# lostinc0de/sparsemat

Measured on AMD Instinct MI355X. Metric: csr_spmv_effective_hbm_GBps, higher is better.
Workload: dtype f32

## Files before the change

include/sparsemat_hip.h:

```cpp
#ifndef SPARSEMAT_HIP_H
#define SPARSEMAT_HIP_H

#include <stddef.h>
#include <stdint.h>

#ifdef __cplusplus
extern "C" {
#endif

#define SMH_ABI_VERSION 3

enum {
    SMH_OK = 0,
    SMH_ERR_DIM_MISMATCH = 1,
    SMH_ERR_NOT_SQUARE = 2,
    SMH_ERR_INDEX_RANGE = 3,
    SMH_ERR_INVALID = 4,
    SMH_ERR_HIP = 5,
    SMH_ERR_OOM = 6,
    SMH_ERR_NO_DEVICE = 7,
    SMH_ERR_CAPACITY = 8,
    SMH_ERR_COMM = 9
};

// ... 22 lines not shown
const char *smh_last_error(void);
const char *smh_status_string(int status);
int smh_device_count(int *count_out);
int smh_set_device(int device);
int smh_device_synchronize(void);

int smh_crs_create(smh_dtype dtype, size_t n_rows, size_t n_cols, size_t nnz,
                   const uint32_t *offset_rows, const uint32_t *columns, const void *values,
                   int validate, smh_crs **out);
int smh_crs_create_dev(smh_dtype dtype, size_t n_rows, size_t n_cols, size_t nnz,
                       const uint32_t *offset_rows_dev, const uint32_t *columns_dev,
                       const void *values_dev, int validate, smh_crs **out);
int smh_crs_assemble(smh_dtype dtype, size_t n_ops, const uint32_t *rows, const uint32_t *cols,
                     const void *values, const uint8_t *ops, smh_crs **out);
int smh_crs_assemble_dev(smh_dtype dtype, size_t n_ops, const uint32_t *rows_dev,
                         const uint32_t *cols_dev, const void *values_dev, const uint8_t *ops_dev,
                         smh_crs **out);
int smh_crs_replay(smh_dtype dtype, size_t n_ops, const uint32_t *rows, const uint32_t *cols,
                   const void *values, const uint8_t *ops, smh_crs **out);
int smh_crs_replay_dev(smh_dtype dtype, size_t n_ops, const uint32_t *rows_dev,
                       const uint32_t *cols_dev, const void *values_dev, const uint8_t *ops_dev,
                       smh_crs **out);
int smh_crs_transpose(const smh_crs *a, smh_crs **out);
int smh_last_transpose_route(void);
int smh_crs_column_info(const smh_crs *m, uint32_t *rows, uint32_t *col_ptr, uint32_t *entries);
int smh_crs_column_info_dev(const smh_crs *m, uint32_t *rows_dev, uint32_t *col_ptr_dev,
                            uint32_t *entries_dev);
int smh_crs_prod(const smh_crs *a, const smh_crs *b, smh_crs **out);
int smh_crs_permute(const smh_crs *a, const uint32_t *row_perm, size_t n_row_perm, const uint32_t *col_perm, size_t n_col_perm, smh_crs **out);
int smh_crs_permute_dev(const smh_crs *a, const uint32_t *row_perm_dev, size_t n_row_perm, const uint32_t *col_perm_dev, size_t n_col_perm,
                        smh_crs **out);
int smh_crs_permute_symmetric(const smh_crs *a, const uint32_t *perm, size_t n_perm, smh_crs **out);
int smh_crs_permute_symmetric_dev(const smh_crs *a, const uint32_t *perm_dev, size_t n_perm, smh_crs **out);
int smh_crs_bandwidth(const smh_crs *m, uint32_t *lower_out, uint32_t *upper_out);
int smh_crs_span_fraction(smh_crs *m, double *out);
int smh_crs_rcm(const smh_crs *m, uint32_t *perm_out, size_t *n_components_out, size_t *n_levels_out);
int smh_crs_rcm_dev(const smh_crs *m, uint32_t *perm_out_dev, size_t *n_components_out, size_t *n_levels_out);
int smh_crs_color(const smh_crs *m, uint32_t seed, uint32_t *colors_out, uint32_t *perm_out, size_t *n_colors_out, size_t *n_rounds_out);
int smh_crs_color_dev(const smh_crs *m, uint32_t seed, uint32_t *colors_out_dev, uint32_t *perm_out_dev, size_t *n_colors_out, size_t *n_rounds_out);
int smh_crs_clone(const smh_crs *a, smh_crs **out);
int smh_crs_add(const smh_crs *a, const smh_crs *b, smh_crs **out);
int smh_crs_sub(const smh_crs *a, const smh_crs *b, smh_crs **out);
int smh_crs_add_assign(smh_crs *a, const smh_crs *b);
int smh_crs_sub_assign(smh_crs *a, const smh_crs *b);
int smh_last_add_route(void);
int smh_crs_get(const smh_crs *m, size_t i, size_t j, void *value_out);
int smh_crs_get_many(const smh_crs *m, size_t n, const uint32_t *rows, const uint32_t *cols, void *values_out);
int smh_crs_get_many_dev(const smh_crs *m, size_t n, const uint32_t *rows_dev, const uint32_t *cols_dev, void *values_out_dev);
int smh_crs_apply(smh_crs *m, size_t n_ops, const uint32_t *rows, const uint32_t *cols, const void *values, const uint8_t *ops);
int smh_crs_apply_dev(smh_crs *m, size_t n_ops, const uint32_t *rows_dev, const uint32_t *cols_dev, const void *values_dev,
                      const uint8_t *ops_dev);
int smh_last_apply_route(void);
typedef struct smh_update_plan smh_update_plan;
int smh_update_plan_create(const smh_crs *m, size_t n_ops, const uint32_t *rows, const uint32_t *cols, const uint8_t *ops,
                           smh_update_plan **out);
int smh_update_plan_create_dev(const smh_crs *m, size_t n_ops, const uint32_t *rows_dev, const uint32_t *cols_dev,
                               const uint8_t *ops_dev, smh_update_plan **out);
int smh_update_plan_execute(smh_update_plan *p, smh_crs *m, const void *values, int from_zero);
int smh_update_plan_execute_dev(smh_update_plan *p, smh_crs *m, const void *values_dev, int from_zero);
int smh_update_plan_stats(const smh_update_plan *p, size_t *n_ops, size_t *n_targets, size_t *n_live_ops, size_t *longest_run,
                          size_t *long_run_threshold, size_t *device_bytes);
int smh_update_plan_destroy(smh_update_plan *p);
int smh_crs_eye(smh_dtype dtype, size_t dim, smh_crs **out);
int smh_crs_is_symmetric(const smh_crs *m, int *out);
int smh_crs_is_sorted(const smh_crs *m, int *out);
int smh_crs_sort_rows(smh_crs *m);
int smh_crs_destroy(smh_crs *m);
int smh_crs_update_values(smh_crs *m, const void *values_host);
int smh_crs_download(const smh_crs *m, uint32_t *offset_rows, uint32_t *columns, void *values);
size_t smh_crs_n_rows(const smh_crs *m);
size_t smh_crs_n_cols(const smh_crs *m);
size_t smh_crs_nnz(const smh_crs *m);
size_t smh_crs_orphans(const smh_crs *m);
int smh_crs_dtype(const smh_crs *m);
int smh_crs_max_row_len(const smh_crs *m, uint32_t *out);
int smh_crs_col_range(const smh_crs *m, uint32_t *min_out, uint32_t *max_out);
int smh_crs_scale(smh_crs *m, double a);
int smh_crs_resolved_variant(const smh_crs *m, int *variant_out, int *lanes_out);
int smh_crs_set_vector_lanes(smh_crs *m, int lanes);
int smh_crs_set_stream_xs(smh_crs *m, int mode);
int smh_crs_stream_layout(smh_crs *m, int *coded_out, int *byte_lengths_out, int *small_tiles_out, int *xs_chunks_out);
int smh_crs_stream_value_dict(smh_crs *m, int *n_values_out, void *values_out);
int smh_crs_set_stream_value_dict(smh_crs *m, int mode);
int smh_crs_set_stream_direct(smh_crs *m, int mode);
int smh_crs_stream_direct(smh_crs *m, int *direct_out);
int smh_crs_set_vector_chunks(smh_crs *m, int chunks);
int smh_crs_set_ring(smh_crs *m, int mode);
int smh_crs_ring_entries(smh_crs *m, uint32_t *out);
int smh_crs_ring_column_form(smh_crs *m, int *form_out);
int smh_crs_ring_bands(smh_crs *m, uint32_t *bands_out, uint32_t *intervals_out);
int smh_crs_ring_plan(smh_crs *m, uint32_t *n_blocks_out, size_t *n_phases_out,
                      double *ring_fraction_out, int *active_out, uint32_t *phase_ptr_out,
                      uint32_t *phases_out);
int smh_crs_ring_regular(smh_crs *m, uint32_t *len_out);

int smh_crs_set_colblock_shift(smh_crs *m, uint32_t shift);
int smh_crs_colblock(smh_crs *m, uint32_t *shift_out, size_t *n_blocks_out, int *rows_per_thread_out,
                     double *span_fraction_out, uint32_t *offsets_out, uint32_t *columns_out,
                     void *values_out);

int smh_crs_colfused(smh_crs *m, int *fits_out, uint32_t *shift_out, size_t *n_blocks_out, uint32_t *rows_per_lane_out,
                     size_t *n_tiles_out, uint32_t *tile_rows_out, uint32_t *segments_out, uint8_t *counts_out,
                     uint32_t *columns_out, void *values_out);

int smh_crs_tiled_layout(smh_crs *m, uint32_t *n_slices_out, uint32_t *slice_columns_out, uint32_t *rows_per_block_out,
                         uint32_t *n_row_blocks_out, size_t *copy_entries_out);
int smh_crs_tiled_products(smh_crs *m, size_t *n_products_out);

int smh_crs_tiled_array(smh_crs *m, int which, void *out, size_t capacity_bytes, size_t *bytes_out);

int smh_crs_colsplit(smh_crs *m, int *split_out, uint32_t *min_long_out, size_t *n_long_out, uint32_t *long_rows_out,
                     smh_crs **long_out, smh_crs **short_out);

int smh_crs_spmv(smh_crs *m, const void *x_host, size_t x_len, void *y_host, int variant);
int smh_crs_prepare(smh_crs *m, int variant);
int smh_crs_prepare_stats(smh_crs *m, int variant, double *prepare_ms_out, size_t *derived_bytes_out);
int smh_crs_spmv_dev(smh_crs *m, const void *x_dev, size_t x_len, void *y_dev, int variant,
                     void *stream);
int smh_crs_inner_prod(smh_crs *m, const void *lhs_host, size_t lhs_len, const void *rhs_host,
                       size_t rhs_len, int variant, double *out);
size_t smh_crs_merge_tiles(const smh_crs *m);
size_t smh_crs_merge_tile_items(const smh_crs *m);
int smh_crs_merge_table(smh_crs *m, uint32_t *row_out, uint32_t *nnz_out);

int smh_vec_create(smh_dtype dtype, size_t n, smh_vec **out);
int smh_vec_from_host(smh_dtype dtype, size_t n, const void *host, smh_vec **out);
int smh_vec_wrap_dev(smh_dtype dtype, size_t n, void *dev_ptr, smh_vec **out);
int smh_vec_destroy(smh_vec *v);
int smh_vec_upload(smh_vec *v, const void *host);
int smh_vec_download(const smh_vec *v, void *host);
size_t smh_vec_dim(const smh_vec *v);
int smh_vec_dtype(const smh_vec *v);
void *smh_vec_data(const smh_vec *v);
int smh_vec_copy(smh_vec *dst, const smh_vec *src);
int smh_vec_permute(smh_vec *dst, const smh_vec *src, const uint32_t *perm, size_t n_perm, int inverse);
int smh_vec_permute_dev(smh_vec *dst, const smh_vec *src, const uint32_t *perm_dev, size_t n_perm, int inverse);
int smh_vec_add(smh_vec *x, const smh_vec *y);
int smh_vec_sub(smh_vec *x, const smh_vec *y);
int smh_vec_scale(smh_vec *x, double a);
int smh_vec_axpy(smh_vec *y, double a, const smh_vec *x);
int smh_vec_xpby(smh_vec *p, double b, const smh_vec *r);
int smh_vec_dot(const smh_vec *x, const smh_vec *y, double *out);
int smh_vec_norm_squared(const smh_vec *x, double *out);
int smh_vec_norm(const smh_vec *x, double *out);
int smh_blas_dot_dev(smh_dtype dtype, const void *x_dev, const void *y_dev, size_t n, void *result_dev,
                     void *scratch_dev, void *stream);
size_t smh_blas_dot_scratch_bytes(void);
int smh_blas_axpy_dev(smh_dtype dtype, void *y_dev, const void *a_dev, const void *x_dev, size_t n, void *stream);
int smh_blas_xpby_dev(smh_dtype dtype, void *p_dev, const void *b_dev, const void *r_dev, size_t n, void *stream);
int smh_crs_spmv_vec(smh_crs *m, const smh_vec *x, smh_vec *y, int variant);
int smh_crs_inner_prod_vec(smh_crs *m, const smh_vec *lhs, const smh_vec *rhs, int variant, double *out);

int smh_mvec_create(smh_dtype dtype, size_t n, size_t k, smh_mvec **out);
int smh_mvec_from_host(smh_dtype dtype, size_t n, size_t k, const void *host, smh_mvec **out);
int smh_mvec_upload(smh_mvec *mv, const void *host);
int smh_mvec_download(const smh_mvec *mv, void *host);
int smh_mvec_destroy(smh_mvec *mv);
size_t smh_mvec_dim(const smh_mvec *mv);
size_t smh_mvec_count(const smh_mvec *mv);
size_t smh_mvec_ld(const smh_mvec *mv);
int smh_mvec_dtype(const smh_mvec *mv);
void *smh_mvec_data(const smh_mvec *mv);
int smh_mvec_set_column(smh_mvec *mv, size_t c, const smh_vec *v);
int smh_mvec_get_column(const smh_mvec *mv, size_t c, smh_vec *v);
int smh_mvec_copy(smh_mvec *dst, const smh_mvec *src);
int smh_mvec_add(smh_mvec *x, const smh_mvec *y);
// ... 153 lines not shown
```

rust/src/ffi.rs:

```rust
#![allow(non_camel_case_types)]
use std::os::raw::{c_char, c_double, c_int, c_void};

#[repr(C)] pub struct smh_crs { _private: [u8; 0] }
#[repr(C)] pub struct smh_vec { _private: [u8; 0] }
#[repr(C)] pub struct smh_update_plan { _private: [u8; 0] }
#[repr(C)] pub struct smh_par { _private: [u8; 0] }
#[repr(C)] pub struct smh_par_vec { _private: [u8; 0] }
#[repr(C)] pub struct smh_comm { _private: [u8; 0] }

pub const SMH_OK: c_int = 0;
pub const SMH_ERR_DIM_MISMATCH: c_int = 1;
pub const SMH_F32: c_int = 0;
pub const SMH_F64: c_int = 1;
pub const SMH_SPMV_AUTO: c_int = 0;
pub const SMH_TRI_LOWER: c_int = 0;
pub const SMH_TRI_UPPER: c_int = 1;
pub const SMH_DIAG_NON_UNIT: c_int = 0;
pub const SMH_DIAG_UNIT: c_int = 1;
pub const SMH_EXCHANGE_NONE: c_int = 0;
pub const SMH_EXCHANGE_ALLGATHER: c_int = 1;
pub const SMH_EXCHANGE_WINDOW: c_int = 2;
pub const SMH_EXCHANGE_AUTO: c_int = 3;
pub const SMH_COMM_ID_BYTES: usize = 128;
pub const SMH_SPLIT_ROWS: c_int = 0;
pub const SMH_SPLIT_NNZ: c_int = 1;

extern "C" {
    pub fn smh_abi_version() -> c_int;
    pub fn smh_last_error() -> *const c_char;
    pub fn smh_device_count(count_out: *mut c_int) -> c_int;
    pub fn smh_pool_trim() -> c_int;
    pub fn smh_pool_stats(kept_bytes_out: *mut usize, live_bytes_out: *mut usize) -> c_int;
    pub fn smh_crs_create(dtype: c_int, n_rows: usize, n_cols: usize, nnz: usize,
                          offset_rows: *const u32, columns: *const u32, values: *const c_void,
                          validate: c_int, out: *mut *mut smh_crs) -> c_int;
    pub fn smh_crs_destroy(m: *mut smh_crs) -> c_int;
    pub fn smh_crs_update_values(m: *mut smh_crs, values_host: *const c_void) -> c_int;
    pub fn smh_crs_spmv(m: *mut smh_crs, x_host: *const c_void, x_len: usize, y_host: *mut c_void,
                        variant: c_int) -> c_int;
    pub fn smh_cg_solve(m: *mut smh_crs, b_host: *const c_void, b_len: usize, x_host_inout: *mut c_void,
                        x_len: usize, tol: c_double, iter_max: usize, variant: c_int,
                        iters_out: *mut usize, rr_out: *mut c_double) -> c_int;
    pub fn smh_pcg_jacobi_solve(m: *mut smh_crs, b_host: *const c_void, b_len: usize, x_host_inout: *mut c_void,
                                x_len: usize, tol: c_double, iter_max: usize, variant: c_int,
                                iters_out: *mut usize, rr_out: *mut c_double) -> c_int;
    pub fn smh_bicgstab_solve(m: *mut smh_crs, b_host: *const c_void, b_len: usize, x_host_inout: *mut c_void,
                              x_len: usize, tol: c_double, iter_max: usize, variant: c_int,
                              iters_out: *mut usize, rr_out: *mut c_double, breakdown_out: *mut c_int) -> c_int;
    pub fn smh_bicgstab_solve_vec(m: *mut smh_crs, b: *const smh_vec, x: *mut smh_vec, tol: c_double, iter_max: usize,
                                  variant: c_int, check_every: usize,
                                  iters_out: *mut usize, rr_out: *mut c_double, breakdown_out: *mut c_int) -> c_int;
    pub fn smh_crs_trisolve_levels(m: *mut smh_crs, uplo: c_int, n_levels_out: *mut usize, level_of_row_out: *mut u32,
                                   n_launches_out: *mut usize, small_level_rows_out: *mut usize) -> c_int;
    pub fn smh_crs_trisolve(m: *mut smh_crs, uplo: c_int, diag: c_int, b_host: *const c_void, b_len: usize, x_host: *mut c_void,
                            x_len: usize) -> c_int;
    pub fn smh_crs_trisolve_vec(m: *mut smh_crs, uplo: c_int, diag: c_int, b: *const smh_vec, x: *mut smh_vec) -> c_int;
    pub fn smh_crs_sgs_apply_vec(m: *mut smh_crs, r: *const smh_vec, z: *mut smh_vec) -> c_int;
    pub fn smh_pcg_sgs_solve(m: *mut smh_crs, b_host: *const c_void, b_len: usize, x_host_inout: *mut c_void,
                             x_len: usize, tol: c_double, iter_max: usize, variant: c_int,
                             iters_out: *mut usize, rr_out: *mut c_double) -> c_int;
    pub fn smh_pcg_sgs_solve_vec(m: *mut smh_crs, b: *const smh_vec, x: *mut smh_vec, tol: c_double, iter_max: usize,
                                 variant: c_int, check_every: usize, iters_out: *mut usize, rr_out: *mut c_double) -> c_int;
    pub fn smh_crs_ilu0(a: *const smh_crs, f_out: *mut *mut smh_crs, zero_pivot_out: *mut usize) -> c_int;
    pub fn smh_crs_ilu0_refactor(f: *mut smh_crs, a: *const smh_crs, zero_pivot_out: *mut usize) -> c_int;
    pub fn smh_crs_ilu_apply_vec(f: *mut smh_crs, r: *const smh_vec, z: *mut smh_vec) -> c_int;
    pub fn smh_pcg_ilu_solve(a: *mut smh_crs, f: *mut smh_crs, b_host: *const c_void, b_len: usize, x_host_inout: *mut c_void,
                             x_len: usize, tol: c_double, iter_max: usize, variant: c_int,
                             iters_out: *mut usize, rr_out: *mut c_double) -> c_int;
    pub fn smh_pcg_ilu_solve_vec(a: *mut smh_crs, f: *mut smh_crs, b: *const smh_vec, x: *mut smh_vec, tol: c_double, iter_max: usize,
                                 variant: c_int, check_every: usize, iters_out: *mut usize, rr_out: *mut c_double) -> c_int;
    pub fn smh_crs_inner_prod(m: *mut smh_crs, lhs_host: *const c_void, lhs_len: usize, rhs_host: *const c_void,
                              rhs_len: usize, variant: c_int, out: *mut c_double) -> c_int;
    pub fn smh_crs_assemble(dtype: c_int, n_ops: usize, rows: *const u32, cols: *const u32, values: *const c_void,
                            ops: *const u8, out: *mut *mut smh_crs) -> c_int;
    pub fn smh_crs_replay(dtype: c_int, n_ops: usize, rows: *const u32, cols: *const u32, values: *const c_void,
                          ops: *const u8, out: *mut *mut smh_crs) -> c_int;
    pub fn smh_crs_transpose(a: *const smh_crs, out: *mut *mut smh_crs) -> c_int;
    pub fn smh_crs_set_stream_xs(m: *mut smh_crs, mode: c_int) -> c_int;
    pub fn smh_crs_set_stream_direct(m: *mut smh_crs, mode: c_int) -> c_int;
    pub fn smh_crs_stream_direct(m: *mut smh_crs, direct_out: *mut c_int) -> c_int;
    pub fn smh_crs_stream_layout(m: *mut smh_crs, coded_out: *mut c_int, byte_lengths_out: *mut c_int, small_tiles_out: *mut c_int, xs_chunks_out: *mut c_int) -> c_int;
    pub fn smh_last_transpose_route() -> c_int;
    pub fn smh_crs_orphans(m: *const smh_crs) -> usize;
    pub fn smh_crs_prod(a: *const smh_crs, b: *const smh_crs, out: *mut *mut smh_crs) -> c_int;
    pub fn smh_crs_clone(a: *const smh_crs, out: *mut *mut smh_crs) -> c_int;
    pub fn smh_crs_permute(a: *const smh_crs, row_perm: *const u32, n_row_perm: usize, col_perm: *const u32, n_col_perm: usize,
                           out: *mut *mut smh_crs) -> c_int;
    pub fn smh_crs_permute_dev(a: *const smh_crs, row_perm_dev: *const u32, n_row_perm: usize, col_perm_dev: *const u32,
                               n_col_perm: usize, out: *mut *mut smh_crs) -> c_int;
    pub fn smh_crs_permute_symmetric(a: *const smh_crs, perm: *const u32, n_perm: usize, out: *mut *mut smh_crs) -> c_int;
    pub fn smh_crs_permute_symmetric_dev(a: *const smh_crs, perm_dev: *const u32, n_perm: usize, out: *mut *mut smh_crs) -> c_int;
    pub fn smh_crs_bandwidth(m: *const smh_crs, lower_out: *mut u32, upper_out: *mut u32) -> c_int;
    pub fn smh_crs_span_fraction(m: *mut smh_crs, out: *mut f64) -> c_int;
    pub fn smh_crs_ring_regular(m: *mut smh_crs, len_out: *mut u32) -> c_int;
    pub fn smh_crs_rcm(m: *const smh_crs, perm_out: *mut u32, n_components_out: *mut usize, n_levels_out: *mut usize) -> c_int;
    pub fn smh_crs_rcm_dev(m: *const smh_crs, perm_out_dev: *mut u32, n_components_out: *mut usize, n_levels_out: *mut usize) -> c_int;
    pub fn smh_crs_color(m: *const smh_crs, seed: u32, colors_out: *mut u32, perm_out: *mut u32, n_colors_out: *mut usize, n_rounds_out: *mut usize) -> c_int;
    pub fn smh_crs_color_dev(m: *const smh_crs, seed: u32, colors_out_dev: *mut u32, perm_out_dev: *mut u32, n_colors_out: *mut usize, n_rounds_out: *mut usize) -> c_int;
    pub fn smh_vec_permute(dst: *mut smh_vec, src: *const smh_vec, perm: *const u32, n_perm: usize, inverse: c_int) -> c_int;
    pub fn smh_vec_permute_dev(dst: *mut smh_vec, src: *const smh_vec, perm_dev: *const u32, n_perm: usize, inverse: c_int) -> c_int;
    pub fn smh_crs_add(a: *const smh_crs, b: *const smh_crs, out: *mut *mut smh_crs) -> c_int;
    pub fn smh_crs_sub(a: *const smh_crs, b: *const smh_crs, out: *mut *mut smh_crs) -> c_int;
    pub fn smh_crs_add_assign(a: *mut smh_crs, b: *const smh_crs) -> c_int;
    pub fn smh_crs_sub_assign(a: *mut smh_crs, b: *const smh_crs) -> c_int;
    pub fn smh_last_add_route() -> c_int;
    pub fn smh_crs_get(m: *const smh_crs, i: usize, j: usize, value_out: *mut c_void) -> c_int;
    pub fn smh_crs_get_many(m: *const smh_crs, n: usize, rows: *const u32, cols: *const u32, values_out: *mut c_void) -> c_int;
    pub fn smh_crs_get_many_dev(m: *const smh_crs, n: usize, rows_dev: *const u32, cols_dev: *const u32,
                                values_out_dev: *mut c_void) -> c_int;
    pub fn smh_crs_apply(m: *mut smh_crs, n_ops: usize, rows: *const u32, cols: *const u32, values: *const c_void,
                         ops: *const u8) -> c_int;
    pub fn smh_crs_apply_dev(m: *mut smh_crs, n_ops: usize, rows_dev: *const u32, cols_dev: *const u32,
                             values_dev: *const c_void, ops_dev: *const u8) -> c_int;
    pub fn smh_last_apply_route() -> c_int;
    pub fn smh_update_plan_create(m: *const smh_crs, n_ops: usize, rows: *const u32, cols: *const u32, ops: *const u8,
                                  out: *mut *mut smh_update_plan) -> c_int;
    pub fn smh_update_plan_create_dev(m: *const smh_crs, n_ops: usize, rows_dev: *const u32, cols_dev: *const u32,
                                      ops_dev: *const u8, out: *mut *mut smh_update_plan) -> c_int;
    pub fn smh_update_plan_execute(p: *mut smh_update_plan, m: *mut smh_crs, values: *const c_void, from_zero: c_int) -> c_int;
    pub fn smh_update_plan_execute_dev(p: *mut smh_update_plan, m: *mut smh_crs, values_dev: *const c_void, from_zero: c_int) -> c_int;
    pub fn smh_update_plan_stats(p: *const smh_update_plan, n_ops: *mut usize, n_targets: *mut usize, n_live_ops: *mut usize,
                                 longest_run: *mut usize, long_run_threshold: *mut usize, device_bytes: *mut usize) -> c_int;
    pub fn smh_update_plan_destroy(p: *mut smh_update_plan) -> c_int;
    pub fn smh_crs_eye(dtype: c_int, dim: usize, out: *mut *mut smh_crs) -> c_int;
    pub fn smh_crs_is_symmetric(m: *const smh_crs, out: *mut c_int) -> c_int;
    pub fn smh_crs_is_sorted(m: *const smh_crs, out: *mut c_int) -> c_int;
    pub fn smh_crs_column_info(m: *const smh_crs, rows: *mut u32, col_ptr: *mut u32, entries: *mut u32) -> c_int;
    pub fn smh_crs_sort_rows(m: *mut smh_crs) -> c_int;
    pub fn smh_par_create(dtype: c_int, n_blocks: usize, device_ids: *const c_int, n_rows: usize, n_cols: usize,
                          offset_rows: *const u32, columns: *const u32, values: *const c_void, validate: c_int,
                          out: *mut *mut smh_par) -> c_int;
    pub fn smh_par_create_split(dtype: c_int, n_blocks: usize, device_ids: *const c_int, n_rows: usize, n_cols: usize,
                                offset_rows: *const u32, columns: *const u32, values: *const c_void, validate: c_int,
                                split_mode: c_int, out: *mut *mut smh_par) -> c_int;
    pub fn smh_par_split(p: *const smh_par, rows_out: *mut usize) -> c_int;
    pub fn smh_par_set_overlap(p: *mut smh_par, on: c_int) -> c_int;
    pub fn smh_par_interior(p: *const smh_par, local_block: usize, variant: c_int, row_begin: *mut usize, row_end: *mut usize) -> c_int;
    pub fn smh_par_destroy(p: *mut smh_par) -> c_int;
    pub fn smh_par_spmv(p: *mut smh_par, x_host: *const c_void, x_len: usize, y_host: *mut c_void, variant: c_int) -> c_int;
    pub fn smh_par_cg_solve(p: *mut smh_par, b_host: *const c_void, b_len: usize, x_host_inout: *mut c_void, x_len: usize,
                            tol: c_double, iter_max: usize, variant: c_int, iters_out: *mut usize,
                            rr_out: *mut c_double) -> c_int;
    pub fn smh_par_vec_create(p: *mut smh_par, n: usize, out: *mut *mut smh_par_vec) -> c_int;
    pub fn smh_par_vec_destroy(v: *mut smh_par_vec) -> c_int;
    pub fn smh_par_vec_upload(v: *mut smh_par_vec, host: *const c_void) -> c_int;
    pub fn smh_par_vec_download(v: *const smh_par_vec, host: *mut c_void) -> c_int;
    pub fn smh_par_spmv_dev(p: *mut smh_par, x: *const smh_par_vec, y: *mut smh_par_vec, variant: c_int, exchange: c_int) -> c_int;
    pub fn smh_par_exchange(p: *mut smh_par, v: *mut smh_par_vec, mode: c_int) -> c_int;
    pub fn smh_par_synchronize(p: *mut smh_par) -> c_int;
    pub fn smh_par_cg_solve_vec(p: *mut smh_par, b: *const smh_par_vec, x: *mut smh_par_vec, tol: c_double, iter_max: usize,
                                variant: c_int, check_every: usize, iters_out: *mut usize, rr_out: *mut c_double) -> c_int;
    pub fn smh_comm_unique_id(id_out: *mut c_void) -> c_int;
    pub fn smh_comm_create(id: *const c_void, n_ranks: c_int, rank: c_int, out: *mut *mut smh_comm) -> c_int;
    pub fn smh_comm_destroy(c: *mut smh_comm) -> c_int;
    pub fn smh_par_create_rank(comm: *mut smh_comm, n_rows: usize, block: *mut smh_crs, out: *mut *mut smh_par) -> c_int;
    pub fn smh_par_create_rank_split(comm: *mut smh_comm, n_rows: usize, block: *mut smh_crs, row_begin: usize, out: *mut *mut smh_par) -> c_int;
    pub fn smh_crs_n_rows(m: *const smh_crs) -> usize;
    pub fn smh_crs_n_cols(m: *const smh_crs) -> usize;
    pub fn smh_crs_dtype(m: *const smh_crs) -> c_int;
    pub fn smh_crs_nnz(m: *const smh_crs) -> usize;
    pub fn smh_crs_download(m: *const smh_crs, offset_rows: *mut u32, columns: *mut u32, values: *mut c_void) -> c_int;
}
```

sparsemat_amd/_lib.py:

```python
import ctypes as C
import os

_HERE = os.path.dirname(os.path.abspath(__file__))
LIB_PATH = os.environ.get("SPARSEMAT_HIP_LIB") or os.path.join(_HERE, "libsparsemat_hip.so")

SMH_OK = 0
SMH_ERR_DIM_MISMATCH, SMH_ERR_NOT_SQUARE, SMH_ERR_INDEX_RANGE, SMH_ERR_INVALID = 1, 2, 3, 4
SMH_ERR_HIP, SMH_ERR_OOM, SMH_ERR_NO_DEVICE, SMH_ERR_CAPACITY, SMH_ERR_COMM = 5, 6, 7, 8, 9
SMH_F32, SMH_F64 = 0, 1
SMH_TRI_LOWER, SMH_TRI_UPPER = 0, 1
SMH_DIAG_NON_UNIT, SMH_DIAG_UNIT = 0, 1
UPLO = {"lower": SMH_TRI_LOWER, "upper": SMH_TRI_UPPER}
EXCHANGE_NONE, EXCHANGE_ALLGATHER, EXCHANGE_WINDOW, EXCHANGE_AUTO = 0, 1, 2, 3
EXCHANGES = {"none": EXCHANGE_NONE, "allgather": EXCHANGE_ALLGATHER, "window": EXCHANGE_WINDOW, "halo": EXCHANGE_WINDOW, "auto": EXCHANGE_AUTO}
EXCHANGE_NAMES = {EXCHANGE_NONE: "none", EXCHANGE_ALLGATHER: "allgather", EXCHANGE_WINDOW: "window", EXCHANGE_AUTO: "auto"}
PAR_BACKEND_AUTO, PAR_BACKEND_PEER, PAR_BACKEND_RCCL = 0, 1, 2
PAR_BACKENDS = {"auto": PAR_BACKEND_AUTO, "peer": PAR_BACKEND_PEER, "rccl": PAR_BACKEND_RCCL}
COMM_ID_BYTES = 128
SPMV_AUTO, SPMV_VECTOR, SPMV_MERGE, SPMV_SEQ, SPMV_STREAM, SPMV_COLBLOCK, SPMV_COLFUSED, SPMV_COLSPLIT, SPMV_TILED = 0, 1, 2, 3, 4, 5, 6, 7, 8
VARIANTS = {"auto": SPMV_AUTO, "vector": SPMV_VECTOR, "merge": SPMV_MERGE, "seq": SPMV_SEQ, "stream": SPMV_STREAM,
            "colblock": SPMV_COLBLOCK, "colfused": SPMV_COLFUSED, "colsplit": SPMV_COLSPLIT, "tiled": SPMV_TILED}

_sz = C.c_size_t
_vp = C.c_void_p
# ... 139 lines not shown
    "smh_cg_solve_many_host": (_int, [_vp, _vp, _sz, _sz, _vp, C.c_double, _sz, C.POINTER(_sz), C.POINTER(C.c_double)]),
    "smh_pcg_jacobi_solve": (_int, [_vp, _vp, _sz, _vp, _sz, C.c_double, _sz, _int, C.POINTER(_sz),
                                    C.POINTER(C.c_double)]),
    "smh_crs_trisolve_levels": (_int, [_vp, _int, C.POINTER(_sz), _vp, C.POINTER(_sz), C.POINTER(_sz)]),
    "smh_crs_trisolve": (_int, [_vp, _int, _int, _vp, _sz, _vp, _sz]),
    "smh_crs_trisolve_vec": (_int, [_vp, _int, _int, _vp, _vp]),
    "smh_crs_sgs_apply_vec": (_int, [_vp, _vp, _vp]),
    "smh_pcg_sgs_solve": (_int, [_vp, _vp, _sz, _vp, _sz, C.c_double, _sz, _int, C.POINTER(_sz),
                                 C.POINTER(C.c_double)]),
    "smh_pcg_sgs_solve_vec": (_int, [_vp, _vp, _vp, C.c_double, _sz, _int, _sz, C.POINTER(_sz),
                                     C.POINTER(C.c_double)]),
    "smh_crs_ilu0": (_int, [_vp, C.POINTER(_vp), C.POINTER(_sz)]),
    "smh_crs_ilu0_refactor": (_int, [_vp, _vp, C.POINTER(_sz)]),
    "smh_crs_ilu_apply_vec": (_int, [_vp, _vp, _vp]),
    "smh_pcg_ilu_solve": (_int, [_vp, _vp, _vp, _sz, _vp, _sz, C.c_double, _sz, _int, C.POINTER(_sz),
                                 C.POINTER(C.c_double)]),
    "smh_pcg_ilu_solve_vec": (_int, [_vp, _vp, _vp, _vp, C.c_double, _sz, _int, _sz, C.POINTER(_sz),
                                     C.POINTER(C.c_double)]),
    "smh_bicgstab_solve": (_int, [_vp, _vp, _sz, _vp, _sz, C.c_double, _sz, _int, C.POINTER(_sz),
                                  C.POINTER(C.c_double), C.POINTER(_int)]),
    "smh_bicgstab_solve_vec": (_int, [_vp, _vp, _vp, C.c_double, _sz, _int, _sz, C.POINTER(_sz),
                                      C.POINTER(C.c_double), C.POINTER(_int)]),
    "smh_comm_unique_id": (_int, [_vp]),
    "smh_comm_create": (_int, [_vp, _int, _int, C.POINTER(_vp)]),
    "smh_comm_destroy": (_int, [_vp]),
    "smh_comm_size": (_int, [_vp]),
    "smh_comm_rank": (_int, [_vp]),
    "smh_comm_ranks_seen": (_int, [_vp, C.POINTER(C.c_int), C.POINTER(C.c_int)]),
    "smh_rccl_version": (_int, [C.POINTER(C.c_int)]),
    "smh_comm_barrier": (_int, [_vp]),
    "smh_comm_max_f64": (_int, [_vp, C.POINTER(C.c_double)]),
    "smh_par_create": (_int, [_int, _sz, _vp, _sz, _sz, _vp, _vp, _vp, _int, C.POINTER(_vp)]),
    "smh_par_create_split": (_int, [_int, _sz, _vp, _sz, _sz, _vp, _vp, _vp, _int, _int, C.POINTER(_vp)]),
    "smh_par_adopt_split": (_int, [_sz, C.POINTER(_vp), _sz, _vp, C.POINTER(_vp)]),
    "smh_par_create_rank_split": (_int, [_vp, _sz, _vp, _sz, C.POINTER(_vp)]),
    "smh_par_split": (_int, [_vp, _vp]),
    "smh_par_plan_split": (_int, [_sz, _sz, _vp, _vp, _vp, _vp, _sz, _vp, _vp, _vp, _vp, C.POINTER(_int), C.POINTER(_sz)]),
    "smh_par_adopt": (_int, [_sz, C.POINTER(_vp), _sz, C.POINTER(_vp)]),
    "smh_par_create_rank": (_int, [_vp, _sz, _vp, C.POINTER(_vp)]),
    "smh_par_n_local_blocks": (_sz, [_vp]),
    "smh_par_set_backend": (_int, [_vp, _int]),
    "smh_par_backend": (_int, [_vp]),
    "smh_par_set_overlap": (_int, [_vp, _int]),
    "smh_par_set_threads": (_int, [_vp, _int]),
    "smh_par_interior": (_int, [_vp, _sz, _int, C.POINTER(_sz), C.POINTER(_sz)]),
    "smh_par_exchange_mode": (_int, [_vp, _int, C.POINTER(_int), C.POINTER(_sz)]),
    "smh_par_plan": (_int, [_sz, _sz, _vp, _vp, _vp, _sz, _vp, _vp, _vp, _vp, C.POINTER(_int), C.POINTER(_sz)]),
    "smh_par_vec_create": (_int, [_vp, _sz, C.POINTER(_vp)]),
    "smh_par_vec_destroy": (_int, [_vp]),
    "smh_par_vec_dim": (_sz, [_vp]),
    "smh_par_vec_upload": (_int, [_vp, _vp]),
    "smh_par_vec_download": (_int, [_vp, _vp]),
    "smh_par_vec_download_block": (_int, [_vp, _sz, _vp]),
    "smh_par_vec_ptr": (_int, [_vp, _sz, C.POINTER(_vp)]),
    "smh_par_spmv_dev": (_int, [_vp, _vp, _vp, _int, _int]),
    "smh_par_exchange": (_int, [_vp, _vp, _int]),
    "smh_par_synchronize": (_int, [_vp]),
    "smh_par_cg_solve_vec": (_int, [_vp, _vp, _vp, C.c_double, _sz, _int, _sz, C.POINTER(_sz), C.POINTER(C.c_double)]),
    "smh_par_destroy": (_int, [_vp]),
    "smh_par_n_blocks": (_sz, [_vp]),
    "smh_par_n_rows": (_sz, [_vp]),
    "smh_par_n_cols": (_sz, [_vp]),
    "smh_par_nnz": (_sz, [_vp]),
    "smh_par_rows_per_block": (_sz, [_vp]),
    "smh_par_block": (_int, [_vp, _sz, C.POINTER(_vp), C.POINTER(_sz), C.POINTER(_sz), C.POINTER(_int)]),
    "smh_par_block_stream": (_int, [_vp, _sz, C.POINTER(_vp)]),
    "smh_par_get_block_and_row_id": (_int, [_vp, _sz, C.POINTER(_sz), C.POINTER(_sz)]),
    "smh_par_scale": (_int, [_vp, C.c_double]),
    "smh_par_spmv": (_int, [_vp, _vp, _sz, _vp, _int]),
    "smh_par_cg_solve": (_int, [_vp, _vp, _sz, _vp, _sz, C.c_double, _sz, _int, C.POINTER(_sz),
                                C.POINTER(C.c_double)]),
    "smh_synth_x": (_int, [_int, C.c_uint64, _sz, _sz, _vp, _vp]),
    "smh_synth_fixed": (_int, [_int, C.c_uint64, _int, _sz, C.c_uint32, _sz, _sz, _vp, _vp, _vp, _vp]),
    "smh_synth_powerlaw_cdf": (_int, [C.c_uint32, C.c_double, _vp]),
    "smh_synth_powerlaw_lengths": (_int, [C.c_uint64, _sz, _sz, C.c_uint32, _vp, _vp]),
    "smh_synth_fill": (_int, [_int, C.c_uint64, _sz, _sz, _sz, _vp, _vp, _vp, _vp]),
    "smh_synth_laplace3d": (_int, [_int, _sz, _sz, _sz, _sz, _sz, _vp, _vp, _vp, C.POINTER(_sz), _vp]),
    "smh_crs_set_stream_xs": (_int, [_vp, _int]),
    "smh_crs_set_stream_direct": (_int, [_vp, _int]),
    "smh_crs_stream_direct": (_int, [_vp, C.POINTER(_int)]),
    "smh_crs_stream_layout": (_int, [_vp, C.POINTER(_int), C.POINTER(_int), C.POINTER(_int), C.POINTER(_int)]),
    "smh_crs_stream_value_dict": (_int, [_vp, C.POINTER(C.c_int), _vp]),
    "smh_crs_set_stream_value_dict": (_int, [_vp, _int]),
    "smh_last_transpose_route": (_int, []),
    "smh_pool_trim": (_int, []),
    "smh_pool_stats": (_int, [C.POINTER(_sz), C.POINTER(_sz)]),
    "smh_dev_alloc": (_int, [_sz, C.POINTER(_vp)]),
    "smh_dev_free": (_int, [_vp]),
    "smh_dev_upload": (_int, [_vp, _vp, _sz]),
    "smh_dev_download": (_int, [_vp, _vp, _sz]),
    "smh_dev_memset": (_int, [_vp, _int, _sz, _vp]),
    "smh_stream_create": (_int, [C.POINTER(_vp)]),
    "smh_stream_destroy": (_int, [_vp]),
    "smh_stream_synchronize": (_int, [_vp]),
    "smh_event_create": (_int, [C.POINTER(_vp)]),
    "smh_event_destroy": (_int, [_vp]),
    "smh_event_record": (_int, [_vp, _vp]),
    "smh_event_elapsed_ms": (_int, [_vp, _vp, C.POINTER(C.c_float)]),
}

_LIB = None


class SparseMatPanic(RuntimeError):

    def __init__(self, status, message):
        super().__init__(message)
        self.status = status


def lib():
    global _LIB
    if _LIB is None:
        if not os.path.exists(LIB_PATH):
            raise ImportError(
                "%s is missing: build it with `python -m sparsemat_amd.build` (hipcc, gfx950). "
                "sparsemat_amd has no CPU fallback." % LIB_PATH)
        import sys
        if "torch" in sys.modules:
            try:
                if sys.modules["torch"].cuda.is_available():
                    sys.modules["torch"].cuda.init()
            except Exception:
                pass
        os.environ.setdefault("HSA_ENABLE_IPC_MODE_LEGACY", "0")
        L = C.CDLL(LIB_PATH)
        for name, (res, args) in SIGNATURES.items():
            fn = getattr(L, name)
            fn.restype = res
            fn.argtypes = args
        _LIB = L
    return _LIB


def check(status):
    if status != SMH_OK:
        L = lib()
        msg = L.smh_last_error().decode(errors="replace") or L.smh_status_string(status).decode()
        raise SparseMatPanic(status, msg)


def dtype_code(np_dtype):
    import numpy as np
    dt = np.dtype(np_dtype)
    if dt == np.float32:
        return SMH_F32
    if dt == np.float64:
        return SMH_F64
    raise TypeError("the HIP path handles f32/f64 values only (got %s)" % dt)


def np_dtype(code):
    import numpy as np
    return np.float64 if code == SMH_F64 else np.float32
```

sparsemat_amd/csrc/capi.hip:

```cpp
#include <atomic>
#include <chrono>
#include <cmath>
#include <cstdarg>
#include <cstdlib>
#include <cstring>
#include <new>
#include <vector>

#include "crs_forms.hpp"

namespace smh {

static thread_local char g_err[512] = "";

void set_error(const char *fmt, ...) {
    va_list ap;
    va_start(ap, fmt);
    vsnprintf(g_err, sizeof g_err, fmt, ap);
    va_end(ap);
}

void clear_error() { g_err[0] = 0; }

int fail(int status, const char *fmt, ...) {
// ... 933 lines not shown
    SMH_TRY(build_eye(dtype, dim, arrays.off, arrays.col, arrays.val, nullptr));
    return wrap_arrays(dtype, nullptr, dim, dim, dim, arrays, 0, out);
}

int smh_crs_is_symmetric(const smh_crs *m, int *out) {
    if (!m || !out) return fail(SMH_ERR_INVALID, "NULL argument");
    return crs_is_symmetric(m->dtype, m->d_off, m->d_col, m->d_val, m->n_rows, out, m->stream);
}

int smh_crs_is_sorted(const smh_crs *m, int *out) {
    if (!m || !out) return fail(SMH_ERR_INVALID, "NULL argument");
    return crs_is_sorted(m->d_off, m->d_col, m->n_rows, out, m->stream);
}

int smh_crs_sort_rows(smh_crs *m) {
    if (!m) return fail(SMH_ERR_INVALID, "NULL handle");
    SMH_TRY(sort_rows(m->dtype, m->d_off, m->d_col, m->d_val, m->n_rows, m->nnz, m->max_col, m->stream));
    invalidate(m, Changed::Order);
    ++m->epoch;
    return SMH_OK;
}

int smh_crs_destroy(smh_crs *m) {
    if (!m) return SMH_OK;
    if (m->stream) { (void)hipStreamSynchronize(m->stream); (void)hipStreamDestroy(m->stream); }
    if (m->owns) { (void)hipFree(m->d_off); (void)hipFree(m->d_col); (void)hipFree(m->d_val); }
    (void)hipGetLastError();
    delete m;
    return SMH_OK;
}

int smh_crs_update_values(smh_crs *m, const void *values_host) {
    if (!m) return fail(SMH_ERR_INVALID, "NULL argument");
    if (m->nnz && values_host) SMH_HIP(hipMemcpy(m->d_val, values_host, m->nnz * dtype_size(m->dtype), hipMemcpyHostToDevice));
    invalidate(m, Changed::Values);
    if (m->codes.state != Form::NotTried && m->codes.direct) {
        StreamCfg c;
        SMH_TRY(stream_cfg(m, &c, true));
    }
    return SMH_OK;
}

int smh_crs_download(const smh_crs *m, uint32_t *offset_rows, uint32_t *columns, void *values) {
    if (!m) return fail(SMH_ERR_INVALID, "NULL handle");
    SMH_HIP(hipStreamSynchronize(m->stream));
    if (offset_rows) SMH_HIP(hipMemcpy(offset_rows, m->d_off, (m->n_rows + 1) * sizeof(uint32_t), hipMemcpyDeviceToHost));
    if (columns && m->nnz) SMH_HIP(hipMemcpy(columns, m->d_col, m->nnz * sizeof(uint32_t), hipMemcpyDeviceToHost));
    if (values && m->nnz) SMH_HIP(hipMemcpy(values, m->d_val, m->nnz * dtype_size(m->dtype), hipMemcpyDeviceToHost));
    return SMH_OK;
}

size_t smh_crs_n_rows(const smh_crs *m) { return m ? m->n_rows : 0; }
size_t smh_crs_n_cols(const smh_crs *m) { return m ? m->n_cols : 0; }
size_t smh_crs_nnz(const smh_crs *m) { return m ? m->nnz : 0; }
size_t smh_crs_orphans(const smh_crs *m) { return m ? m->orphans : 0; }
int smh_crs_dtype(const smh_crs *m) { return m ? m->dtype : -1; }

int smh_crs_max_row_len(const smh_crs *m, uint32_t *out) {
    if (!m || !out) return fail(SMH_ERR_INVALID, "NULL argument");
    *out = m->max_row_len;
    return SMH_OK;
}

int smh_crs_col_range(const smh_crs *m, uint32_t *min_out, uint32_t *max_out) {
    if (!m) return fail(SMH_ERR_INVALID, "NULL handle");
    if (min_out) *min_out = m->min_col;
    if (max_out) *max_out = m->max_col;
    return SMH_OK;
}

int smh_crs_scale(smh_crs *m, double a) {
    if (!m) return fail(SMH_ERR_INVALID, "NULL handle");
    SMH_TRY(launch_scale_values(m->dtype, m->d_val, m->nnz, a, m->stream));
    if (m->has_first_op) {
        Scratch scr;
        char *d = nullptr;
        SMH_TRY(scr.alloc(&d, 16));
        SMH_HIP(hipMemcpyAsync(d, &m->first_val_bits, 8, hipMemcpyHostToDevice, m->stream));
        SMH_TRY(launch_scale_values(m->dtype, d, 1, a, m->stream));
        SMH_HIP(hipMemcpyAsync(&m->first_val_bits, d, 8, hipMemcpyDeviceToHost, m->stream));
        SMH_HIP(hipStreamSynchronize(m->stream));
    }
    if (m->dict.state == Form::Ready) SMH_TRY(launch_scale_values(m->dtype, m->dict.values.get(), 32, a, m->stream));
    if (m->cb.state == Form::Ready) SMH_TRY(launch_scale_values(m->dtype, m->cb.val.get(), m->nnz, a, m->stream));
    if (m->cf.state == Form::Ready) SMH_TRY(launch_scale_values(m->dtype, m->cf.val.get(), m->nnz, a, m->stream));
    if (m->tiled.state == Form::Ready) SMH_TRY(launch_scale_values(m->dtype, m->tiled.val.get(), (size_t)m->tiled.tot, a, m->stream));
    if (m->split.state == Form::Ready) {
        SMH_TRY(smh_crs_scale(m->split.long_part, a));
        SMH_TRY(smh_crs_scale(m->split.short_part, a));
    }
    SMH_HIP(hipStreamSynchronize(m->stream));
    return SMH_OK;
}

int smh_crs_tiled_layout(smh_crs *m, uint32_t *n_slices_out, uint32_t *slice_columns_out, uint32_t *rows_per_block_out, uint32_t *n_row_blocks_out,
                         size_t *copy_entries_out) {
    if (!m) return fail(SMH_ERR_INVALID, "NULL handle");
    SMH_TRY(tiled_build(m));
    if (n_slices_out) *n_slices_out = m->tiled.n_cb;
    if (slice_columns_out) *slice_columns_out = tiled_slice_columns(m->dtype);
    if (rows_per_block_out) *rows_per_block_out = m->tiled.R;
    if (n_row_blocks_out) *n_row_blocks_out = m->tiled.n_rb;
    if (copy_entries_out) *copy_entries_out = (size_t)m->tiled.tot;
    return SMH_OK;
}

int smh_crs_tiled_products(smh_crs *m, size_t *n_products_out) {
    if (!m) return fail(SMH_ERR_INVALID, "NULL handle");
    SMH_TRY(tiled_build(m));
    if (n_products_out) *n_products_out = (size_t)m->tiled.n_prod;
    return SMH_OK;
}

int smh_crs_tiled_array(smh_crs *m, int which, void *out, size_t capacity_bytes, size_t *bytes_out) {
    if (!m) return fail(SMH_ERR_INVALID, "NULL handle");
    SMH_TRY(tiled_build(m));
    return tiled_array(m, which, out, capacity_bytes, bytes_out);
}

int smh_crs_set_colblock_shift(smh_crs *m, uint32_t shift) {
    if (!m) return fail(SMH_ERR_INVALID, "NULL handle");
    if (shift > 31) return fail(SMH_ERR_INVALID, "column block shift must be 0 (automatic) or 1..31");
    if (shift != m->knobs.cb_forced_shift) invalidate(m, Changed::BlockWidth);
    m->knobs.cb_forced_shift = shift;
    return SMH_OK;
}

int smh_crs_colblock(smh_crs *m, uint32_t *shift_out, size_t *n_blocks_out, int *rows_per_thread_out,
                     double *span_fraction_out, uint32_t *offsets_out, uint32_t *columns_out, void *values_out) {
    if (!m) return fail(SMH_ERR_INVALID, "NULL handle");
    SMH_TRY(ensure_ring_plan(m, false));
    SMH_TRY(ensure_colblock(m));
    if (shift_out) *shift_out = m->cb.shift;
    if (n_blocks_out) *n_blocks_out = m->cb.blocks;
    if (rows_per_thread_out) *rows_per_thread_out = m->cb.rpt;
    if (span_fraction_out) *span_fraction_out = m->span_fraction;
    if (offsets_out)
        SMH_HIP(hipMemcpy(offsets_out, m->cb.off.get(), m->cb.blocks * (m->n_rows + 1) * sizeof(uint32_t), hipMemcpyDeviceToHost));
    if (columns_out && m->nnz) SMH_HIP(hipMemcpy(columns_out, m->cb.col.get(), m->nnz * sizeof(uint32_t), hipMemcpyDeviceToHost));
    if (values_out && m->nnz) SMH_HIP(hipMemcpy(values_out, m->cb.val.get(), m->nnz * dtype_size(m->dtype), hipMemcpyDeviceToHost));
    return SMH_OK;
}

int smh_crs_colfused(smh_crs *m, int *fits_out, uint32_t *shift_out, size_t *n_blocks_out, uint32_t *rows_per_lane_out,
                     size_t *n_tiles_out, uint32_t *tile_rows_out, uint32_t *segments_out, uint8_t *counts_out, uint32_t *columns_out,
                     void *values_out) {
    if (!m) return fail(SMH_ERR_INVALID, "NULL handle");
    SMH_TRY(ensure_colfused(m));
    const size_t tile_rows = (size_t)64 * m->cf.rt, n_tiles = (m->cf.state == Form::Ready) ? m->cf.tiles : 0;
    if (fits_out) *fits_out = (m->cf.state == Form::Ready) ? 1 : 0;
    if (shift_out) *shift_out = m->cf.shift;
    if (n_blocks_out) *n_blocks_out = m->cf.blocks;
    if (rows_per_lane_out) *rows_per_lane_out = m->cf.rt;
    if (n_tiles_out) *n_tiles_out = n_tiles;
    if (m->cf.state != Form::Ready) return SMH_OK;
    SMH_HIP(hipStreamSynchronize(m->stream));
    if (tile_rows_out) SMH_HIP(hipMemcpy(tile_rows_out, m->cf.tile_row.get(), (n_tiles + 1) * sizeof(uint32_t), hipMemcpyDeviceToHost));
    if (segments_out) SMH_HIP(hipMemcpy(segments_out, m->cf.seg.get(), (n_tiles * m->cf.blocks + 1) * sizeof(uint32_t), hipMemcpyDeviceToHost));
    if (counts_out && n_tiles) SMH_HIP(hipMemcpy(counts_out, m->cf.cnt.get(), n_tiles * m->cf.blocks * tile_rows, hipMemcpyDeviceToHost));
    if (columns_out && m->nnz) SMH_HIP(hipMemcpy(columns_out, m->cf.col.get(), m->nnz * sizeof(uint32_t), hipMemcpyDeviceToHost));
    if (values_out && m->nnz) SMH_HIP(hipMemcpy(values_out, m->cf.val.get(), m->nnz * dtype_size(m->dtype), hipMemcpyDeviceToHost));
    return SMH_OK;
}

int smh_crs_colsplit(smh_crs *m, int *split_out, uint32_t *min_long_out, size_t *n_long_out, uint32_t *long_rows_out, smh_crs **long_out,
                     smh_crs **short_out) {
    if (!m) return fail(SMH_ERR_INVALID, "NULL handle");
    SMH_TRY(ensure_split(m));
    const bool split = m->split.state == Form::Ready;
    if (split_out) *split_out = split ? 1 : 0;
    if (min_long_out) *min_long_out = kSplitMinLong;
    if (n_long_out) *n_long_out = split ? m->split.n_long : 0;
    if (long_out) *long_out = split ? m->split.long_part : nullptr;
    if (short_out) *short_out = split ? m->split.short_part : nullptr;
    if (long_rows_out && split && m->split.n_long)
        SMH_HIP(hipMemcpy(long_rows_out, m->split.rows.get(), m->split.n_long * sizeof(uint32_t), hipMemcpyDeviceToHost));
    return SMH_OK;
}

int smh_crs_resolved_variant(const smh_crs *m, int *variant_out, int *lanes_out) {
    if (!m) return fail(SMH_ERR_INVALID, "NULL handle");
    if (variant_out) *variant_out = resolve_variant(m, SMH_SPMV_AUTO);
    if (lanes_out) *lanes_out = auto_lanes(m);
    return SMH_OK;
}

int smh_crs_set_stream_xs(smh_crs *m, int mode) {
    if (!m) return fail(SMH_ERR_INVALID, "NULL handle");
    if (mode < -1 || mode > 1) return fail(SMH_ERR_INVALID, "mode must be -1 (automatic), 0 (never) or 1 (whenever the tiles allow)");
    m->knobs.use_stream_xs = mode;
    return recode_stream(m);
}

int smh_crs_set_stream_direct(smh_crs *m, int mode) {
    if (!m) return fail(SMH_ERR_INVALID, "NULL handle");
    if (mode < -1 || mode > 1) return fail(SMH_ERR_INVALID, "mode must be -1 (automatic), 0 (never) or 1 (whenever x is staged)");
    m->knobs.use_stream_direct = mode;
    return recode_stream(m);
}

int smh_crs_stream_direct(smh_crs *m, int *direct_out) {
    if (!m || !direct_out) return fail(SMH_ERR_INVALID, "NULL argument");
    StreamCfg c;
    SMH_TRY(stream_cfg(m, &c));
    *direct_out = c.direct && c.xs != 0;
    return SMH_OK;
}

int smh_crs_stream_value_dict(smh_crs *m, int *n_values_out, void *values_out) {
    if (!m || !n_values_out) return fail(SMH_ERR_INVALID, "NULL argument");
    StreamCfg c;
    SMH_TRY(stream_cfg(m, &c));
    *n_values_out = c.dict ? (int)m->dict.n : 0;
    if (c.dict && values_out) {
        SMH_HIP(hipMemcpyAsync(values_out, m->dict.values.get(), (size_t)m->dict.n * dtype_size(m->dtype), hipMemcpyDeviceToHost, m->stream));
        SMH_HIP(hipStreamSynchronize(m->stream));
    }
    return SMH_OK;
}

int smh_crs_set_stream_value_dict(smh_crs *m, int mode) {
    if (!m) return fail(SMH_ERR_INVALID, "NULL handle");
    if (mode < -1 || mode > 0) return fail(SMH_ERR_INVALID, "mode must be -1 (automatic: whenever the values allow) or 0 (never)");
    m->knobs.use_stream_vdict = mode;
    return recode_stream(m);
}

int smh_crs_stream_layout(smh_crs *m, int *coded_out, int *byte_lengths_out, int *small_tiles_out, int *xs_chunks_out) {
    if (!m) return fail(SMH_ERR_INVALID, "NULL handle");
    StreamCfg c;
    SMH_TRY(stream_cfg(m, &c));
    if (coded_out) *coded_out = c.code && c.cwin;
    if (byte_lengths_out) *byte_lengths_out = c.len8 && c.tbase;
    if (small_tiles_out) *small_tiles_out = c.small;
    if (xs_chunks_out) *xs_chunks_out = c.xs;
    return SMH_OK;
}

int smh_crs_set_vector_chunks(smh_crs *m, int chunks) {
    if (!m) return fail(SMH_ERR_INVALID, "NULL handle");
    if (chunks < 0 || chunks > 3) return fail(SMH_ERR_INVALID, "chunks per lane must be 0 (automatic), 1, 2 or 3");
    m->knobs.forced_chunks = chunks;
    return SMH_OK;
}

int smh_crs_set_ring(smh_crs *m, int mode) {
    if (!m) return fail(SMH_ERR_INVALID, "NULL handle");
    if (mode < -1 || mode > 1) return fail(SMH_ERR_INVALID, "ring mode must be -1 (auto), 0 (plain K1) or 1 (K1r)");
    m->knobs.use_ring = mode;
    return SMH_OK;
}

int smh_crs_ring_plan(smh_crs *m, uint32_t *n_blocks_out, size_t *n_phases_out, double *ring_fraction_out,
                      int *active_out, uint32_t *phase_ptr_out, uint32_t *phases_out) {
    if (!m) return fail(SMH_ERR_INVALID, "NULL handle");
    SMH_TRY(ensure_ring_plan(m));
    bool ring = false;
    SMH_TRY(vector_uses_ring(m, &ring));
    if (n_blocks_out) *n_blocks_out = m->ring.blocks;
    if (n_phases_out) *n_phases_out = m->ring.n_phases;
    if (ring_fraction_out) *ring_fraction_out = m->ring.fraction;
    if (active_out) *active_out = ring ? 1 : 0;
    if (phase_ptr_out)
        SMH_HIP(hipMemcpy(phase_ptr_out, m->ring.phase_ptr.get(), (m->ring.blocks + 1) * sizeof(uint32_t), hipMemcpyDeviceToHost));
    if (phases_out && m->ring.n_phases)
        SMH_HIP(hipMemcpy(phases_out, m->ring.phases.get(), m->ring.n_phases * sizeof(RingPhase), hipMemcpyDeviceToHost));
    return SMH_OK;
}

int smh_crs_ring_regular(smh_crs *m, uint32_t *len_out) {
    if (!m || !len_out) return fail(SMH_ERR_INVALID, "NULL argument");
    SMH_TRY(ensure_ring_plan(m));
    if (m->ring.n_phases)
        SMH_HIP(hipMemcpy(len_out, m->ring.reg_len.get(), m->ring.n_phases * sizeof(uint32_t), hipMemcpyDeviceToHost));
    return SMH_OK;
}

int smh_crs_ring_column_form(smh_crs *m, int *form_out) {
    if (!m || !form_out) return fail(SMH_ERR_INVALID, "NULL argument");
    bool ring = false;
    SMH_TRY(vector_uses_ring(m, &ring));
    *form_out = !ring ? 0 : m->ring.lo8.get() ? 2 : m->ring.col16.get() ? 1 : 0;
    return SMH_OK;
}

int smh_crs_ring_entries(smh_crs *m, uint32_t *out) {
    if (!m || !out) return fail(SMH_ERR_INVALID, "NULL argument");
    SMH_TRY(ensure_ring_plan(m));
    *out = m->ring.entries;
    return SMH_OK;
}

int smh_crs_ring_bands(smh_crs *m, uint32_t *bands_out, uint32_t *intervals_out) {
    if (!m || !bands_out) return fail(SMH_ERR_INVALID, "NULL argument");
    SMH_TRY(ensure_ring_plan(m));
    *bands_out = m->ring.bands;
    if (intervals_out && m->ring.bands == 4 && m->ring.win.get())
        SMH_HIP(hipMemcpy(intervals_out, m->ring.win.get(), ((m->n_rows + 63) / 64) * 8 * sizeof(uint32_t), hipMemcpyDeviceToHost));
    return SMH_OK;
}

int smh_crs_set_vector_lanes(smh_crs *m, int lanes) {
    if (!m) return fail(SMH_ERR_INVALID, "NULL handle");
    if (lanes != 0 && (lanes < 1 || lanes > 64 || (lanes & (lanes - 1))))
        return fail(SMH_ERR_INVALID, "lanes per row must be 0 or a power of two in 1..64");
    m->knobs.forced_lanes = lanes;
    return SMH_OK;
// ... 433 lines not shown
```

sparsemat_amd/csrc/crs_forms.hip:

```cpp
#include <cstdlib>
#include <cstring>
#include <vector>

#include "crs_forms.hpp"

namespace smh {

void build_ring_plan(size_t n_rows, size_t ring_entries, const uint32_t *cmin, const uint32_t *cmax, size_t n_blocks,
                     uint32_t noring_mode, std::vector<uint32_t> &phase_ptr, std::vector<RingPhase> &phases,
                     double *ring_row_fraction);
void build_ring_plan_banded(size_t n_rows, size_t ring_entries, const uint32_t *win, size_t n_blocks, uint32_t noring_mode,
                            std::vector<uint32_t> &phase_ptr, std::vector<RingPhase> &phases, double *ring_row_fraction);

int ensure_merge_ws(smh_crs *m) {
    if (m->merge.state == Form::Ready) return SMH_OK;
    MergeTable t;
    const uint64_t items = (uint64_t)m->n_rows + (uint64_t)m->nnz;
    t.n_tiles = (size_t)((items + kMergeTile - 1) / kMergeTile);
    if (t.n_tiles) {
        SMH_TRY(t.tile_row.alloc(t.n_tiles + 1));
        SMH_TRY(t.tile_nz.alloc(t.n_tiles + 1));
        SMH_TRY(t.carry_row.alloc(t.n_tiles));
        SMH_TRY(t.carry_val.alloc(t.n_tiles * dtype_size(m->dtype)));
        SMH_TRY(launch_merge_table(m->d_off, m->n_rows, m->nnz, t.n_tiles, t.tile_row.get(), t.tile_nz.get(), m->stream));
// ... 153 lines not shown
                return launch_stream_max_tile(c.off.get() + b * (m->n_rows + 1), m->n_rows, (size_t)kStreamRows * rpt, d, m->stream);
            }));
            worst = h > worst ? h : worst;
        }
        if (worst <= (uint32_t)kStreamCap || rpt == 1) break;
    }
    c.rpt = rpt < 1 ? 1 : rpt;
    c.single_pass = worst <= (uint32_t)kStreamCap;
    c.state = Form::Ready;
    m->cb = std::move(c);
    return SMH_OK;
}

int ensure_colfused(smh_crs *m) {
    if (m->cf.state != Form::NotTried) return SMH_OK;
    SMH_TRY(columns_within_n_cols(m, "fused column-blocked variant"));
    const size_t blocks = blocks_for(m->n_cols, cf_shift_for(m));
    if (blocks > 255) return fail(SMH_ERR_INVALID, "fused column-blocked variant: %zu column blocks (supported: 1..255)", blocks);
    uint32_t rt = 16;
    if (const char *e = getenv("SMH_COLFUSED_RT")) {
        if (atoi(e) == 8) rt = 8;
    }
    ColFused c;
    bool fits = false;
    uint32_t *tile_row = nullptr, *seg = nullptr, *col2 = nullptr;
    uint8_t *cnt = nullptr;
    void *val2 = nullptr;
    SMH_TRY(build_colfused(m->dtype, m->d_off, m->d_col, m->d_val, m->n_rows, m->nnz, cf_shift_for(m), blocks, rt, &c.tiles,
                           &tile_row, &seg, &cnt, &col2, &val2, &fits, m->stream));
    c.tile_row.reset(tile_row);
    c.seg.reset(seg);
    c.cnt.reset(cnt);
    c.col.reset(col2);
    c.val.reset((char *)val2);
    c.shift = cf_shift_for(m);
    c.blocks = blocks;
    c.rt = rt;
    c.state = fits ? Form::Ready : Form::Refused;
    m->cf = std::move(c);
    return SMH_OK;
}

const uint32_t kSplitMinLong = 64;
int ensure_split(smh_crs *m) {
    if (m->split.state != Form::NotTried) return SMH_OK;
    SMH_TRY(columns_within_n_cols(m, "row-length split"));
    m->split.state = Form::Refused;
    if (m->no_split || m->n_rows == 0 || m->nnz == 0) return SMH_OK;
    RowSplit sp;
    size_t nnz_long = 0;
    uint32_t *rows = nullptr;
    CrsArrays long_part, short_part;
    SMH_TRY(build_colsplit(m->dtype, m->d_off, m->d_col, m->d_val, m->n_rows, m->nnz, kSplitMinLong, &sp.n_long, &nnz_long, &rows, &long_part.off,
                           &long_part.col, &long_part.val, &short_part.off, &short_part.col, &short_part.val, m->stream));
    sp.rows.reset(rows);
    const bool worth = sp.n_long > 0 && sp.n_long * 4 <= m->n_rows && nnz_long * 4 >= m->nnz;
    if (!worth) return SMH_OK;
    auto part = [&](size_t n_rows, size_t nnz, CrsArrays &arrays, uint32_t shift, smh_crs **out) -> int {
        SMH_TRY(wrap_arrays(m->dtype, nullptr, n_rows, m->n_cols, nnz, arrays, 0, out));
        (*out)->no_split = true;
        (*out)->knobs.cb_forced_shift = shift;
        return SMH_OK;
    };
    SMH_TRY(part(sp.n_long, nnz_long, long_part, 18u, &sp.long_part));
    SMH_TRY(part(m->n_rows, m->nnz - nnz_long, short_part, 19u, &sp.short_part));
    SMH_TRY(sp.y.alloc(sp.n_long * dtype_size(m->dtype)));
    SMH_HIP(hipStreamCreateWithFlags(&sp.side, hipStreamNonBlocking));
    SMH_HIP(hipEventCreateWithFlags(&sp.fork, hipEventDisableTiming));
    SMH_HIP(hipEventCreateWithFlags(&sp.join, hipEventDisableTiming));
    sp.state = Form::Ready;
    m->split = std::move(sp);
    return SMH_OK;
}
RowSplit::~RowSplit() {
    (void)smh_crs_destroy(long_part);
    (void)smh_crs_destroy(short_part);
    rows.reset();
    y.reset();
    if (side) { (void)hipStreamSynchronize(side); (void)hipStreamDestroy(side); }
    if (fork) (void)hipEventDestroy(fork);
    if (join) (void)hipEventDestroy(join);
}

static int ensure_stream_codes(smh_crs *m) {
    if (m->codes.state != Form::NotTried) return SMH_OK;
    StreamCodes c;
    c.state = Form::Refused;
    const size_t n_tiles = (m->n_rows + kStreamRows - 1) / kStreamRows;
    if (n_tiles && m->nnz) {
        uint32_t h_count = 0;
        SMH_TRY(c.cwin.alloc(n_tiles * 8));
        SMH_TRY(read_back(&h_count, 1, m->stream, [&](uint32_t *d_count) {
            return launch_stream_windows(m->d_off, m->d_col, m->n_rows, c.cwin.get(), d_count, m->stream);
        }));
        if ((size_t)h_count == n_tiles) c.state = Form::Ready;
        else c.cwin.reset();
    }
    if (c.state == Form::Ready) {
        const size_t n_out = ((m->nnz + 3) & ~size_t(3)) + 4;
        SMH_TRY(c.code.alloc(n_out));
        SMH_HIP(hipMemsetAsync(c.code.get(), 0, n_out * sizeof(uint16_t), m->stream));
        SMH_TRY(launch_stream_codes(m->d_off, m->d_col, c.cwin.get(), m->n_rows, c.code.get(), m->stream));
        if (m->max_row_len <= 255u) {
            SMH_TRY(c.len8.alloc(n_tiles * kStreamRows));
            SMH_TRY(c.tbase.alloc(n_tiles + 1));
            SMH_TRY(launch_stream_len8(m->d_off, m->n_rows, c.len8.get(), c.tbase.get(), m->stream));
            uint32_t h_xs[2] = {0xFFFFFFFFu, 0};
            SMH_TRY(read_back(h_xs, 2, m->stream, [&](uint32_t *d_xs) { return launch_stream_xs_stats(c.cwin.get(), n_tiles, d_xs, m->stream); }));
            c.xs_chunks = h_xs[0];
            c.xs_end = h_xs[1];
            unsigned long long h_odd = 0;
            SMH_TRY(read_back(&h_odd, 1, m->stream, [&](unsigned long long *d_odd) {
                return launch_stream_odd_rows(c.len8.get(), n_tiles * kStreamRows, d_odd, m->stream);
            }));
            c.odd_rows = (uint64_t)h_odd;
        }
        SMH_HIP(hipStreamSynchronize(m->stream));
    }
    m->codes = std::move(c);
    return SMH_OK;
}

static void drop_ring_col12(smh_crs *m) {
    m->ring.lo8.reset();
    m->ring.hdr.reset();
    m->ring.escapes.reset();
}
static int ensure_ring_col12(smh_crs *m, bool forced, bool *use) {
    RingPlan &r = m->ring;
    *use = forced || r.c12 == Form::Ready;
    if (r.c12 != Form::NotTried && (!*use || r.lo8.get())) return SMH_OK;
    Scratch scr;
    uint32_t *jobs = nullptr;
    unsigned long long *d_counts = nullptr, h_counts[2] = {0, 0};
    SMH_TRY(scr.alloc(&jobs, 2 * r.n_phases));
    SMH_TRY(scr.alloc(&d_counts, 2));
    SMH_TRY(read_back(d_counts, h_counts, 2, m->stream, [&](unsigned long long *d) {
        return launch_col12_count(m->d_off, m->d_col, m->nnz, r.phases.get(), r.n_phases, jobs, d, m->stream);
    }));
    r.c12_chunks = h_counts[0];
    r.c12_escapes = h_counts[1];
    r.c12 = r.c12_escapes * 1024ull <= r.c12_chunks ? Form::Ready : Form::Refused;
    *use = forced || r.c12 == Form::Ready;
    if (!*use) return SMH_OK;
    const size_t n_chunks_out = ((m->nnz + 3) >> 2) + 1;
    DevArray<uint8_t> lo8;
    DevArray<uint16_t> hdr;
    DevArray<uint32_t> escapes;
    SMH_TRY(lo8.alloc(n_chunks_out * 4));
    SMH_TRY(hdr.alloc(n_chunks_out));
    SMH_TRY(escapes.alloc(2 * (size_t)(r.c12_escapes ? r.c12_escapes : 1)));
    SMH_TRY(launch_col12_encode(m->d_col, m->nnz, jobs, r.n_phases, n_chunks_out, lo8.get(), hdr.get(), escapes.get(), d_counts, m->stream));
    SMH_HIP(hipStreamSynchronize(m->stream));
    r.lo8 = std::move(lo8);
    r.hdr = std::move(hdr);
    r.escapes = std::move(escapes);
    return SMH_OK;
}

int vector_uses_ring(smh_crs *m, bool *out) {
    *out = false;
    if (m->knobs.use_ring == 0 || m->n_rows == 0) return SMH_OK;
    SMH_TRY(ensure_ring_plan(m));
    *out = true;
    int want = m->knobs.use_col16;
    if (const char *e = getenv("SMH_RING_COL16")) want = atoi(e) ? 1 : 0;
    int want12 = m->knobs.use_col12;
    if (const char *e = getenv("SMH_RING_COL12")) want12 = strcmp(e, "auto") == 0 ? -1 : (atoi(e) ? 1 : 0);
    const bool can12 = m->dtype == SMH_F32 && m->ring.bands == 1 && m->ring.entries == (unsigned)kRingEntries && m->nnz > 0;
    bool use12 = can12 && (want12 == 1 || (want12 < 0 && want < 0 && m->ring.fraction >= 0.25));
    if (use12) SMH_TRY(ensure_ring_col12(m, want12 == 1, &use12));
    if (!use12) drop_ring_col12(m);
    const bool use16 = m->ring.bands == 4 || want == 1 || (want < 0 && m->ring.fraction >= 0.25);
    if (use16 && !m->ring.col16.get() && m->nnz) {
        const size_t n_out = ((m->nnz + 3) & ~size_t(3)) + 4;
        DevArray<uint16_t> col16;
        SMH_TRY(col16.alloc(n_out));
        if (m->ring.bands == 4) {
            SMH_HIP(hipMemsetAsync(col16.get(), 0, n_out * sizeof(uint16_t), m->stream));
            SMH_TRY(launch_ring_band_codes(m->d_off, m->d_col, m->ring.win.get(), m->n_rows, m->ring.entries / 4, col16.get(), m->stream));
        } else {
            SMH_TRY(launch_narrow_columns(m->d_col, m->nnz, col16.get(), n_out, m->stream));
        }
        SMH_HIP(hipStreamSynchronize(m->stream));
        m->ring.col16 = std::move(col16);
    } else if (!use16) {
        m->ring.col16.reset();
    }
    return SMH_OK;
}

void invalidate(smh_crs *m, Changed what) {
    m->cb = ColBlock();
    m->cf = ColFused();
    m->split = RowSplit();
    m->tiled = Tiled();
    if (what == Changed::Values) m->dict.state = Form::NotTried;
    if (what == Changed::Order) {
        m->codes = StreamCodes();
        m->ring.col16.reset();
        drop_ring_col12(m);
        m->ring.c12 = Form::NotTried;
        m->tri[0] = TriSchedule();
        m->tri[1] = TriSchedule();
    }
}

static int stream_rpt(const smh_crs *m) {
    int want = m->knobs.stream_rows_per_thread;
    if (const char *e = getenv("SMH_STREAM_RPT")) want = atoi(e);
    return want == 2 && m->max_tile512_entries <= (uint32_t)kStreamCap ? 2 : 1;
}

int stream_cfg(smh_crs *m, StreamCfg *c, bool recode) {
    *c = StreamCfg();
    c->rpt = stream_rpt(m);
    c->single_pass = m->have_stats && (c->rpt == 2 || m->max_tile_entries <= (uint32_t)kStreamCap);
    const char *c16_env = getenv("SMH_STREAM_C16");
    if (!(c16_env && atoi(c16_env) == 0) && c->rpt == 1 && c->single_pass) {
        const bool first = m->codes.state == Form::NotTried;
        SMH_TRY(ensure_stream_codes(m));
        if (first) recode = true;
        c->code = m->codes.code.get();
        c->cwin = m->codes.code.get() ? m->codes.cwin.get() : nullptr;
        static const bool l8_off = getenv("SMH_STREAM_L8") && atoi(getenv("SMH_STREAM_L8")) == 0;
        if (c->cwin && !l8_off) { c->len8 = m->codes.len8.get(); c->tbase = m->codes.tbase.get(); }
        static const bool small_off = getenv("SMH_STREAM_SMALL") && atoi(getenv("SMH_STREAM_SMALL")) == 0;
        c->small = !small_off && m->have_stats && m->max_tile_entries <= (uint32_t)kStreamCapSmall;
        static const bool xs_off = getenv("SMH_STREAM_XS") && atoi(getenv("SMH_STREAM_XS")) == 0;
        const bool forced = m->knobs.use_stream_xs == 1;
        const size_t x_bytes = m->n_cols * dtype_size(m->dtype);
        const bool on2 = forced || x_bytes >= ((size_t)1 << 20), on4 = forced || (x_bytes >= ((size_t)8 << 20) && m->dtype == SMH_F32);
        c->xs = (xs_off || m->knobs.use_stream_xs == 0 || !c->small || !c->len8) ? 0
                : (m->codes.xs_chunks <= 2u * kBlock && on2) ? 2
                : (m->codes.xs_chunks <= 4u * kBlock && on4) ? 4 : 0;
        static const bool xd_off = getenv("SMH_STREAM_XD") && atoi(getenv("SMH_STREAM_XD")) == 0;
        const bool want_direct = c->code && c->xs != 0 && !xd_off && m->knobs.use_stream_direct != 0 &&
                                 (m->knobs.use_stream_direct == 1 || 2 * m->codes.odd_rows >= (uint64_t)m->n_rows);
        static const bool vd_off = getenv("SMH_STREAM_VDICT") && atoi(getenv("SMH_STREAM_VDICT")) == 0;
        bool want_vdict = want_direct && !vd_off && m->knobs.use_stream_vdict != 0 && m->dict.state != Form::Refused;
        bool dict_rebuilt = false;
        if (recode && want_vdict && m->dict.state == Form::NotTried) {
            if (!m->dict.values.get()) SMH_TRY(m->dict.values.alloc(32 * dtype_size(m->dtype)));
            SMH_HIP(hipDeviceSynchronize());
            uint32_t n_vals = 0;
            SMH_TRY(stream_value_dict(m->dtype, m->d_val, m->nnz, m->dict.values.get(), &n_vals, m->stream));
            m->dict.n = n_vals;
            m->dict.state = n_vals ? Form::Ready : Form::Refused;
            dict_rebuilt = true;
        }
        want_vdict = want_vdict && m->dict.state == Form::Ready && m->dict.n <= stream_value_dict_capacity(c->xs);
        const bool form_ok = want_direct == m->codes.direct && want_vdict == m->codes.vdict && (!want_vdict || m->codes.vdict_xs == c->xs) &&
                             !(dict_rebuilt && (want_vdict || m->codes.vdict));
        if (recode && c->code && !form_ok) {
            SMH_HIP(hipDeviceSynchronize());
            if (want_direct)
                SMH_TRY(launch_stream_stage_codes(m->d_off, m->d_col, m->codes.cwin.get(), m->n_rows, (uint32_t)dtype_size(m->dtype), m->codes.code.get(), m->stream));
            else
                SMH_TRY(launch_stream_codes(m->d_off, m->d_col, m->codes.cwin.get(), m->n_rows, m->codes.code.get(), m->stream));
            if (want_vdict)
                SMH_TRY(launch_stream_value_codes(m->dtype, m->d_val, m->nnz, m->dict.values.get(), m->dict.n, c->xs, m->codes.code.get(), m->stream));
            SMH_HIP(hipStreamSynchronize(m->stream));
            m->codes.direct = want_direct;
            m->codes.vdict = want_vdict;
            m->codes.vdict_xs = want_vdict ? c->xs : 0;
        }
        c->direct = c->code && m->codes.direct;
        c->dict = c->direct && m->codes.vdict ? m->dict.values.get() : nullptr;
        c->dict_high = c->dict && stream_value_dict_high(m->dtype, m->dict.n, m->codes.vdict_xs);
    }
    return SMH_OK;
}

int recode_stream(smh_crs *m) {
    if (m->codes.state == Form::NotTried) return SMH_OK;
    StreamCfg c;
    return stream_cfg(m, &c, true);
}

}
```

sparsemat_amd/csrc/crs_forms.hpp:

```cpp
#pragma once
#include "internal.hpp"

namespace smh {

void clear_error();
int wrap_arrays(int dtype, const ::smh_crs *like, size_t n_rows, size_t n_cols, size_t nnz, CrsArrays &arrays, int validate, ::smh_crs **out);

template <typename U, typename F> int read_back(U *d, U *host, size_t count, hipStream_t s, F &&launch) {
    SMH_TRY(launch(d));
    SMH_HIP(hipMemcpyAsync(host, d, count * sizeof(U), hipMemcpyDeviceToHost, s));
    SMH_HIP(hipStreamSynchronize(s));
    return SMH_OK;
}
template <typename U, typename F> int read_back(U *host, size_t count, hipStream_t s, F &&launch) {
    Scratch scr;
    U *d = nullptr;
    SMH_TRY(scr.alloc(&d, count));
    return read_back(d, host, count, s, launch);
}

extern const uint32_t kSplitMinLong;
int ensure_merge_ws(::smh_crs *m);
int ensure_ring_plan(::smh_crs *m, bool with_bands = true);
int ensure_colblock(::smh_crs *m);
int ensure_colfused(::smh_crs *m);
int ensure_split(::smh_crs *m);
int vector_uses_ring(::smh_crs *m, bool *out);
enum class Changed { Values, Order, BlockWidth };
void invalidate(::smh_crs *m, Changed what);
struct StreamCfg {
    int rpt = 1;
    bool single_pass = false;
    const uint16_t *code = nullptr;
    const uint32_t *cwin = nullptr;
    const uint8_t *len8 = nullptr;
    const uint32_t *tbase = nullptr;
    bool small = false;
    int xs = 0;
    bool direct = false;
    const void *dict = nullptr;
    bool dict_high = false;
};
int stream_cfg(::smh_crs *m, StreamCfg *c, bool recode = false);
int recode_stream(::smh_crs *m);

extern const size_t kColblockMinXBytes;
uint32_t cb_shift_for(const ::smh_crs *m);
uint32_t cf_shift_for(const ::smh_crs *m);
size_t blocks_for(size_t n_cols, uint32_t shift);
int auto_lanes(const ::smh_crs *m);
int resolve_variant(const ::smh_crs *m, int variant);
int prepare_forms(::smh_crs *m, int variant);
int spmv_inner_prod(::smh_crs *m, const void *d_lhs, const void *d_rhs, size_t rhs_len, int variant, void *scratch, void *res);

}
```

sparsemat_amd/csrc/internal.hpp:

```cpp
#pragma once
#include <hip/hip_runtime.h>

#include <cstddef>
#include <cstdint>
#include <cstdio>
#include <cstring>
#include <string>
#include <utility>
#include <vector>

#include "../../include/sparsemat_hip.h"

namespace smh {

void set_error(const char *fmt, ...);
int fail(int status, const char *fmt, ...);
int hip_fail(hipError_t e, const char *what, const char *file, int line);

#define SMH_HIP(call)                                                     \
    do {                                                                  \
        hipError_t e__ = (call);                                          \
        if (e__ != hipSuccess) return ::smh::hip_fail(e__, #call, __FILE__, __LINE__); \
    } while (0)

// ... 230 lines not shown
    return v + __int_as_float(__builtin_amdgcn_update_dpp(0, __float_as_int(v), CTRL, ROWS, 0xF, false));
}
template <int CTRL, int ROWS> __device__ __forceinline__ double wave_dpp_add(double v) {
    const long long b = __double_as_longlong(v);
    const uint32_t lo = (uint32_t)__builtin_amdgcn_update_dpp(0, (int)(uint32_t)b, CTRL, ROWS, 0xF, false);
    const uint32_t hi = (uint32_t)__builtin_amdgcn_update_dpp(0, (int)(uint32_t)((unsigned long long)b >> 32), CTRL, ROWS, 0xF, false);
    return v + __longlong_as_double((long long)(((unsigned long long)hi << 32) | lo));
}
template <typename T> __device__ __forceinline__ T wave_sum_to_lane63(T v) {
    v = wave_dpp_add<0x111, 0xF>(v);
    v = wave_dpp_add<0x112, 0xF>(v);
    v = wave_dpp_add<0x114, 0xF>(v);
    v = wave_dpp_add<0x118, 0xF>(v);
    v = wave_dpp_add<0x142, 0xA>(v);
    v = wave_dpp_add<0x143, 0xC>(v);
    return v;
}
__device__ __forceinline__ uint32_t wave_max_u32(uint32_t v) {
#pragma unroll
    for (int o = 32; o > 0; o >>= 1) {
        const uint32_t w = (uint32_t)__shfl_xor((int)v, o, kWave);
        v = w > v ? w : v;
    }
    return v;
}
constexpr uint64_t kBuildGrid = 16384;
inline unsigned grid_for(uint64_t n, uint64_t cap) {
    const uint64_t b = (n + kBlock - 1) / kBlock;
    return (unsigned)(b == 0 ? 1 : b > cap ? cap : b);
}
inline unsigned bits_for(uint64_t v) {
    unsigned b = 1;
    while (b < 64 && (v >> b)) ++b;
    return b;
}
constexpr int kMergeItemsPerThread = 8;
constexpr int kMergeTile = kBlock * kMergeItemsPerThread;
constexpr int kReducePartials = 1024;
constexpr int kRingEntries = 16384;
constexpr int kRingEntriesWide = 32768;
constexpr int kStreamRows = kBlock;
constexpr int kStreamCap = 4096;
constexpr int kStreamCapSmall = 2045;
constexpr int kStreamCodeWidth = 16384;
constexpr int kManyCap = 2048;

int device_exclusive_scan_u32(uint32_t *data, uint64_t n, hipStream_t s, uint64_t *total_out);
int launch_spmv_vector(int dtype, int lanes, const uint32_t *off, const uint32_t *col, const void *val,
                       const void *x, void *y, size_t n_rows, size_t nnz, hipStream_t s);
int launch_spmv_seq(int dtype, const uint32_t *off, const uint32_t *col, const void *val, const void *x,
                    void *y, size_t n_rows, hipStream_t s);
int launch_merge_table(const uint32_t *off, size_t n_rows, size_t nnz, size_t n_tiles, uint32_t *tile_row,
                       uint32_t *tile_nz, hipStream_t s);
int launch_spmv_merge(int dtype, const uint32_t *off, const uint32_t *col, const void *val, const void *x,
                      void *y, size_t n_rows, size_t nnz, size_t n_tiles, const uint32_t *tile_row,
                      const uint32_t *tile_nz, uint32_t *carry_row, void *carry_val, hipStream_t s);
int launch_spmv_stream(int dtype, const uint32_t *off, const uint32_t *col, const void *val, const void *x, void *y,
                       size_t n_rows, size_t nnz, bool padded, int rows_per_thread,
                       bool single_pass ,
                       void *dot_partials ,
                       const uint16_t *code, const uint32_t *cwin ,
                       const uint8_t *len8, const uint32_t *tbase ,
                       const void *dot_lhs ,
                       hipStream_t s, bool small_tiles = false ,
                       int xs = 0 ,
                       uint64_t tile_begin = 0, uint64_t tile_end = ~uint64_t(0) );
int launch_stream_xs_stats(const uint32_t *win, size_t n_tiles, uint32_t *d_out2, hipStream_t s);
int launch_stream_len8(const uint32_t *off, size_t n_rows, uint8_t *len8, uint32_t *tbase, hipStream_t s);
size_t stream_tiles(size_t n_rows, int rows_per_thread);
int launch_stream_windows(const uint32_t *off, const uint32_t *col, size_t n_rows, uint32_t *win,
                          uint32_t *d_count, hipStream_t s);
int launch_stream_codes(const uint32_t *off, const uint32_t *col, const uint32_t *win, size_t n_rows, uint16_t *code,
                        hipStream_t s);
int launch_spmv_many(int dtype, const uint32_t *off, const uint32_t *col, const void *val, const void *x, void *y, size_t n_rows, size_t nnz,
                     bool padded, size_t k, size_t ld, hipStream_t s);
int launch_spmv_stream_xd(int dtype, const void *val, const void *x, void *y, size_t n_rows, void *dot_partials, const uint16_t *scode,
                          const uint32_t *cwin, const uint8_t *len8, const uint32_t *tbase, const void *dot_lhs, hipStream_t s, int xs,
                          uint64_t tile_begin = 0, uint64_t tile_end = ~uint64_t(0), const void *dict = nullptr ,
                          bool dict_high = false );
bool stream_value_dict_high(int dtype, uint32_t n, int xs);
int stream_value_dict(int dtype, const void *val, size_t nnz, void *dict_out, uint32_t *count_out, hipStream_t s);
int launch_stream_value_codes(int dtype, const void *val, size_t nnz, const void *dict, uint32_t n, int xs, uint16_t *code, hipStream_t s);
uint32_t stream_value_dict_capacity(int xs);
int launch_stream_stage_codes(const uint32_t *off, const uint32_t *col, const uint32_t *win, size_t n_rows, uint32_t elem_bytes,
                              uint16_t *code, hipStream_t s);
int launch_stream_odd_rows(const uint8_t *len8, size_t n_padded, unsigned long long *d_out, hipStream_t s);
int launch_stream_max_tile(const uint32_t *off, size_t n_rows, size_t tile_rows, uint32_t *d_out, hipStream_t s);
int launch_spmv_stream_block(int dtype, const uint32_t *off, const uint32_t *col, const void *val, const void *x, void *y,
                             size_t n_rows, size_t nnz_total, int rows_per_thread, bool single_pass, bool accumulate,
                             hipStream_t s);
int build_colblock(int dtype, const uint32_t *off, const uint32_t *col, const void *val, size_t n_rows, size_t nnz,
                   uint32_t shift, size_t n_blocks, uint32_t **off2_out, uint32_t **col2_out, void **val2_out,
                   hipStream_t s);
int build_colfused(int dtype, const uint32_t *off, const uint32_t *col, const void *val, size_t n_rows, size_t nnz, uint32_t shift,
                   size_t n_blocks, uint32_t rt, size_t *n_tiles_out, uint32_t **tile_row_out, uint32_t **seg_out, uint8_t **cnt_out,
                   uint32_t **col2_out, void **val2_out, bool *fits_out, hipStream_t s);
int launch_spmv_colfused(int dtype, uint32_t rt, const uint32_t *tile_row, size_t n_tiles, const uint32_t *seg, const uint8_t *cnt,
                         const uint32_t *col, const void *val, const void *x, void *y, size_t n_rows, size_t nnz, uint32_t n_blocks,
                         int device, hipStream_t s);
int build_colsplit(int dtype, const uint32_t *off, const uint32_t *col, const void *val, size_t n_rows, size_t nnz, uint32_t min_long,
                   size_t *n_long_out, size_t *nnz_long_out, uint32_t **long_rows_out, uint32_t **off_l_out, uint32_t **col_l_out, void **val_l_out,
                   uint32_t **off_s_out, uint32_t **col_s_out, void **val_s_out, hipStream_t s);
int launch_split_scatter(int dtype, const uint32_t *long_rows, const void *y_long, size_t n_long, void *y, hipStream_t s);
int assemble_triplets(int dtype, size_t n, const uint32_t *rows, const uint32_t *cols, const void *vals, const uint8_t *ops,
                      bool reverse_rows, bool all_set, bool repeats_adjacent, size_t *n_rows_out, size_t *n_cols_out, size_t *nnz_out,
                      uint32_t **off_out, uint32_t **col_out, void **val_out, hipStream_t s);
int expand_rows(const uint32_t *off, size_t n_rows, uint32_t *rows_out, hipStream_t s);
int column_lists_bucketed(const uint32_t *off, const uint32_t *col, size_t n_rows, size_t n_cols, size_t nnz, uint32_t max_col, uint32_t *col_ptr,
                          uint32_t *entries, bool *done, hipStream_t s);
int transpose_bucketed(int dtype, const uint32_t *off, const uint32_t *col, const void *val, size_t n_rows, size_t nnz, uint32_t max_col,
                       uint32_t **off_out, uint32_t **col_out, void **val_out, size_t *n_rows_out, size_t *n_cols_out, bool *done, hipStream_t s);
int append_to_row(int dtype, uint32_t *off, uint32_t **col, void **val, size_t n_rows, size_t *nnz, size_t row, uint32_t column,
                  const void *value_host, hipStream_t s);
int column_info(const uint32_t *off, const uint32_t *col, size_t n_rows, size_t n_cols, size_t nnz, uint32_t max_col, uint32_t *rows,
                uint32_t *col_ptr, uint32_t *entries, hipStream_t s);
int sort_rows(int dtype, const uint32_t *off, uint32_t *col, void *val, size_t n_rows, size_t nnz, uint32_t max_col,
              hipStream_t s);
int crs_is_sorted(const uint32_t *off, const uint32_t *col, size_t n_rows, int *out, hipStream_t s);
int crs_is_symmetric(int dtype, const uint32_t *off, const uint32_t *col, const void *val, size_t n_rows, int *out, hipStream_t s);
int prod_crs(int dtype, const uint32_t *a_off, const uint32_t *a_col, const void *a_val, size_t a_rows, size_t a_nnz, uint32_t a_max_col,
             const uint32_t *b_off, const uint32_t *b_col, const void *b_val, size_t b_rows, size_t *n_rows_out, size_t *n_cols_out,
             size_t *nnz_out, uint32_t **off_out, uint32_t **col_out, void **val_out, hipStream_t s);
struct AddOperand {
    const uint32_t *off = nullptr, *col = nullptr;
    const void *val = nullptr;
    size_t n_rows = 0, n_cols = 0, nnz = 0, orphans = 0;
    uint32_t max_row_len = 0, max_col = 0;
};
struct AddResult {
    size_t n_rows = 0, n_cols = 0, nnz = 0;
    CrsArrays arrays;
    int route = 0;
    bool values_only = false;
};
int add_crs(int dtype, bool subtract, const AddOperand &a, const AddOperand &b, bool in_place, bool alias, bool force_general, AddResult *res,
            hipStream_t s);
struct UpdMatrix {
    const uint32_t *off = nullptr, *col = nullptr;
    void *val = nullptr;
    size_t n_rows = 0, n_cols = 0, nnz = 0, orphans = 0;
    uint32_t max_row_len = 0;
};
struct UpdResult {
    size_t n_rows = 0, n_cols = 0, nnz = 0;
    CrsArrays arrays;
    int route = 0;
    bool values_only = false;
};
int crs_get_many(int dtype, const UpdMatrix &m, size_t n, const uint32_t *rows, const uint32_t *cols, void *values_out, hipStream_t s);
int crs_apply(int dtype, const UpdMatrix &m, size_t n, const uint32_t *rows, const uint32_t *cols, const void *vals, const uint8_t *ops,
              bool force_general, UpdResult *res, hipStream_t s);
int build_eye(int dtype, size_t dim, uint32_t *off, uint32_t *col, void *val, hipStream_t s);
int validate_permutation(const uint32_t *perm, size_t n, uint32_t *first, const char *what, hipStream_t s);
int permute_crs(int dtype, const uint32_t *a_off, const uint32_t *a_col, const void *a_val, size_t n_rows, size_t nnz, const uint32_t *row_perm,
                const uint32_t *col_inv, CrsArrays *out, hipStream_t s);
int launch_vec_permute(int dtype, void *dst, const void *src, const uint32_t *perm, size_t n, bool inverse, hipStream_t s);
int launch_bandwidth(const uint32_t *off, const uint32_t *col, size_t n_rows, uint32_t *d_out2, hipStream_t s);
int rcm_order(const uint32_t *off, const uint32_t *col, size_t n, size_t nnz, uint32_t *perm_out, size_t *n_components, size_t *n_levels, hipStream_t s);
int symmetrised_pattern(const uint32_t *off, const uint32_t *col, size_t n, size_t nnz, Scratch &scr, uint32_t **adj_off_out, uint32_t **adj_col_out,
                        hipStream_t s);
int color_order(const uint32_t *off, const uint32_t *col, size_t n, size_t nnz, uint32_t seed, uint32_t *colors_out, uint32_t *perm_out, size_t *n_colors,
                size_t *n_rounds, hipStream_t s);
constexpr uint32_t kPlanLongRun = 64;
struct UpdPlan {
    size_t n_ops = 0, n_targets = 0, n_live = 0, longest_run = 0, n_short = 0, device_bytes = 0;
    DevArray<uint32_t> pos;
// ... 92 lines not shown
        if (crc != SMH_OK || ce != hipSuccess || !graph.get() || exec.instantiate(graph.get()) != hipSuccess)
            (void)hipGetLastError();
    } else {
        (void)hipGetLastError();
    }
    auto poll = [&]() -> int {
        SMH_HIP(hipMemcpyAsync(h_sc, d_sc, cg_scalars_bytes(dtype), hipMemcpyDeviceToHost, s));
        SMH_HIP(hipStreamSynchronize(s));
        uint64_t it64 = 0;
        cg_read_scalars(dtype, h_sc, converged, &it64, rr);
        *iters = (size_t)it64;
        return SMH_OK;
    };
    auto run = [&]() -> int {
        size_t launched = 0;
        while (launched < iter_max) {
            size_t batch = iter_max - launched < check_every ? iter_max - launched : check_every;
            if (exec.get()) {
                SMH_HIP(hipGraphLaunch(exec.get(), s));
                batch = check_every;
            } else {
                for (size_t i = 0; i < batch; ++i) SMH_TRY(body());
            }
            launched += batch;
            SMH_TRY(poll());
            if (*converged) break;
        }
        if (iter_max == 0) SMH_TRY(poll());
        return SMH_OK;
    };
    const int rc = run();
    if (rc != SMH_OK) (void)hipStreamSynchronize(s);
    return rc;
}

enum class Form {
    NotTried,
    Ready,
    Refused,
};
struct MergeTable {
    Form state = Form::NotTried;
    size_t n_tiles = 0;
    DevArray<uint32_t> tile_row, tile_nz, carry_row;
    DevArray<char> carry_val;
};
struct RingPlan {
    Form state = Form::NotTried;
    bool bands_tried = false;
    unsigned blocks = 0;
    double fraction = 0.0;
    unsigned entries = kRingEntries;
    unsigned bands = 1;
    size_t n_phases = 0;
    DevArray<uint32_t> phase_ptr;
    DevArray<RingPhase> phases;
    DevArray<uint32_t> reg_len;
    bool reg_applies = false;
    DevArray<uint32_t> win;
    DevArray<uint16_t> col16;
    Form c12 = Form::NotTried;
    uint64_t c12_chunks = 0, c12_escapes = 0;
    DevArray<uint8_t> lo8;
    DevArray<uint16_t> hdr;
    DevArray<uint32_t> escapes;
};
struct StreamCodes {
    Form state = Form::NotTried;
    DevArray<uint32_t> cwin;
    DevArray<uint16_t> code;
    DevArray<uint8_t> len8;
    DevArray<uint32_t> tbase;
    uint32_t xs_chunks = 0xFFFFFFFFu, xs_end = 0;
    uint64_t odd_rows = 0;
    bool direct = false;
    bool vdict = false;
    int vdict_xs = 0;
};
struct StreamDict {
    Form state = Form::NotTried;
    uint32_t n = 0;
    DevArray<char> values;
};
struct ColBlock {
    Form state = Form::NotTried;
    uint32_t shift = 0;
    size_t blocks = 0;
    int rpt = 1;
    bool single_pass = false;
    DevArray<uint32_t> off, col;
    DevArray<char> val;
};
struct ColFused {
    Form state = Form::NotTried;
    uint32_t shift = 0, rt = 0;
    size_t blocks = 0, tiles = 0;
    DevArray<uint32_t> seg, col, tile_row;
    DevArray<uint8_t> cnt;
    DevArray<char> val;
};
struct RowSplit {
    Form state = Form::NotTried;
    ::smh_crs *long_part = nullptr, *short_part = nullptr;
    DevArray<uint32_t> rows;
    DevArray<char> y;
    size_t n_long = 0;
    hipStream_t side = nullptr;
    hipEvent_t fork = nullptr, join = nullptr;
    RowSplit() = default;
    RowSplit(RowSplit &&o) noexcept { swap(o); }
    RowSplit &operator=(RowSplit &&o) noexcept {
        RowSplit old(std::move(*this));
        swap(o);
        return *this;
    }
    ~RowSplit();
    void swap(RowSplit &o) noexcept {
        std::swap(state, o.state); std::swap(long_part, o.long_part); std::swap(short_part, o.short_part);
        std::swap(rows, o.rows); std::swap(y, o.y); std::swap(n_long, o.n_long);
        std::swap(side, o.side); std::swap(fork, o.fork); std::swap(join, o.join);
    }
};
struct Tiled {
    Form state = Form::NotTried;
    uint32_t n_cb = 0, n_rb = 0, R = 0;
    uint64_t tot = 0;
    DevArray<char> val, prod;
    DevArray<uint16_t> code, row;
    DevArray<uint32_t> tstart;
    DevArray<uint32_t> rbstart;
    DevArray<uint32_t> cptr;
    DevArray<char> chunk;
    uint32_t n_chunks = 0, max_slice_chunks = 0;
    bool dups = false;
    uint64_t n_prod = 0;
};
struct TriSchedule {
    Form state = Form::NotTried;
    size_t n_levels = 0;
    uint64_t first_no_diag = ~0ull;
    DevArray<uint32_t> rows;
    DevArray<uint32_t> level_ptr;
    DevArray<uint32_t> level;
    DevArray<uint32_t> diagpos;
    struct Launch { uint32_t level_begin, level_end, row_begin, row_end; bool small; };
    std::vector<Launch> launches;
};
constexpr uint32_t kTriSmallRows = 128;
constexpr uint32_t kTriSmallBlock = 1024;
struct StageBuf {
    DevArray<char> d;
    size_t cap = 0;
    int ensure_cap(size_t bytes) {
        if (cap >= bytes && d.get()) return SMH_OK;
        cap = 0;
        const size_t want = bytes < 256 ? 256 : bytes;
        SMH_TRY(d.alloc(want));
        cap = want;
        return SMH_OK;
    }
};
struct Knobs {
    int forced_lanes = 0;
    int forced_chunks = 0;
    int stream_rows_per_thread = 0;
    uint32_t cb_forced_shift = 0;
    int use_ring = -1;
    int use_stream_xs = -1;
    int use_stream_direct = -1;
    int use_stream_vdict = -1;
    int use_col16 = -1;
    int use_col12 = -1;
};

}

namespace smh {
uint64_t next_crs_id();
}
struct smh_crs {
    uint64_t id = smh::next_crs_id();
    uint64_t epoch = 0;
    int dtype = SMH_F32;
    int device = 0;
    size_t n_rows = 0, n_cols = 0, nnz = 0;
    size_t orphans = 0;
    bool has_first_op = false;
    uint32_t first_row = 0, first_col = 0;
    uint64_t first_val_bits = 0;
    uint32_t *d_off = nullptr;
    uint32_t *d_col = nullptr;
    void *d_val = nullptr;
    bool owns = true;
    bool no_split = false;
    hipStream_t stream = nullptr;
    uint32_t max_row_len = 0;
    uint32_t max_col = 0;
    uint32_t min_col = 0;
    uint32_t max_tile_entries = 0;
    uint32_t max_tile512_entries = 0;
    bool have_stats = false;
    double span_fraction = 0.0;
    smh::Knobs knobs;
    smh::MergeTable merge;
    smh::RingPlan ring;
    smh::StreamCodes codes;
    smh::StreamDict dict;
    smh::ColBlock cb;
    smh::ColFused cf;
    smh::RowSplit split;
    smh::Tiled tiled;
    smh::TriSchedule tri[2];
    smh::StageBuf stage_x, stage_y;
    double create_ms = 0.0, prepare_ms = 0.0;
    long long create_bytes = 0, prepare_bytes = 0;
};

struct smh_vec {
    int dtype = SMH_F32;
    int device = 0;
    size_t n = 0;
    void *d = nullptr;
    bool owns = true;
};

struct smh_mvec {
    int dtype = SMH_F32;
    int device = 0;
    size_t n = 0, k = 0, ld = 0;
    smh::DevArray<char> d;
};

namespace smh {
int cg_solve_many(::smh_crs *m, const ::smh_mvec *b, ::smh_mvec *x, double tol, size_t iter_max, size_t check_every, size_t *iters_out,
                  double *rr_out);
}

#ifndef SMH_POOL_IMPL
#define hipMalloc(p, n) ::smh::pool_malloc((void **)(p), (n))
#define hipFree(p) ::smh::pool_free((void *)(p))
#endif
```

sparsemat_amd/csrc/spmv_dispatch.hip:

```cpp
#include <cstdlib>
#include <cstring>

#include "crs_forms.hpp"

namespace smh {

static double mean_row(const smh_crs *m) { return m->n_rows ? (double)m->nnz / (double)m->n_rows : 0.0; }

static int mean_lanes(const smh_crs *m) {
    const double mean = mean_row(m);
    const double need = mean < 16.0 ? mean + 3.0 : mean;
    int lanes = 1;
    while (lanes < 64 && 4.0 * lanes < need) lanes <<= 1;
    return lanes;
}

int auto_lanes(const smh_crs *m) {
    if (m->knobs.forced_lanes) return m->knobs.forced_lanes;
    const double mean = mean_row(m);
    int lanes = mean_lanes(m);
    if (m->knobs.use_ring != 0) {
        if (mean >= 128.0) lanes = 16;
        else if (lanes > 32) lanes = 32;
        if (mean > 32.0 && m->ring.state == Form::Ready && m->ring.fraction < 0.5) lanes = 8;
    }
    return lanes;
}

static int auto_chunks(const smh_crs *m) {
    const int lanes = auto_lanes(m);
    if (m->knobs.forced_chunks) {
        if (lanes == 1) return m->knobs.forced_chunks;
        if (lanes == 2) return m->knobs.forced_chunks > 2 ? 2 : m->knobs.forced_chunks;
        return 1;
    }
    return 1;
}

uint32_t cb_shift_for(const smh_crs *m) { return m->knobs.cb_forced_shift ? m->knobs.cb_forced_shift : 19u; }
uint32_t cf_shift_for(const smh_crs *m) { return m->knobs.cb_forced_shift ? m->knobs.cb_forced_shift : 18u; }
size_t blocks_for(size_t n_cols, uint32_t shift) {
    const uint64_t w = 1ull << shift;
    const uint64_t b = ((uint64_t)n_cols + w - 1) / w;
    return (size_t)(b ? b : 1);
}
const size_t kColblockMinXBytes = 4u << 20;
static bool wants_colblock(const smh_crs *m) {
    const size_t b = blocks_for(m->n_cols, cb_shift_for(m));
    return m->n_cols * dtype_size(m->dtype) >= kColblockMinXBytes && m->span_fraction > 0.25 && b >= 2 && b <= 128;
}

static bool tiled_fits(const smh_crs *m, double min_tile = 32.0) {
    static const bool tiled_off = getenv("SMH_TILED") && atoi(getenv("SMH_TILED")) == 0;
    if (tiled_off || m->tiled.state == Form::Refused) return false;
    uint32_t n_cb = 0, R = 0, n_rb = 0;
    tiled_geometry(m->n_rows, m->n_cols, m->nnz, m->dtype, &n_cb, &R, &n_rb);
    const double tile = (double)m->nnz / (double)n_cb / (double)n_rb;
    return tile >= min_tile && (double)(n_rb + 1) * (double)n_cb * 4.0 <= (double)(1u << 30);
}

int resolve_variant(const smh_crs *m, int variant) {
    if (variant != SMH_SPMV_AUTO) return variant;
    if (wants_colblock(m)) {
        static const bool fused_off = getenv("SMH_COLBLOCK_FUSED") && atoi(getenv("SMH_COLBLOCK_FUSED")) == 0;
        if (fused_off || m->cf.state == Form::Refused || blocks_for(m->n_cols, cf_shift_for(m)) > 255) return SMH_SPMV_COLBLOCK;
        const double mean = mean_row(m);
        const double similar = 2.0 * mean + 8.0 > 128.0 ? 2.0 * mean + 8.0 : 128.0;
        if ((double)m->max_row_len <= similar) {
            const size_t blocks = blocks_for(m->n_cols, cf_shift_for(m));
            const bool pays = m->dtype == SMH_F32 ? tiled_fits(m)
                              : m->no_split       ? false
                                                  : tiled_fits(m, blocks >= 24 ? 12.0 : 32.0);
            if (pays) return SMH_SPMV_TILED;
            return SMH_SPMV_COLFUSED;
        }
        if (!m->no_split && tiled_fits(m, m->dtype == SMH_F64 && blocks_for(m->n_cols, cf_shift_for(m)) >= 24 ? 12.0 : 32.0)) return SMH_SPMV_TILED;
        static const bool split_off = getenv("SMH_COLBLOCK_SPLIT") && atoi(getenv("SMH_COLBLOCK_SPLIT")) == 0;
        const double vs = (double)dtype_size(m->dtype);
        const double sweeps = (double)blocks_for(m->n_cols, cb_shift_for(m)) * (double)m->n_rows * (4.0 + 2.0 * vs), entries = (double)m->nnz * (4.0 + vs);
        if (!split_off && !m->no_split && m->split.state != Form::Refused && sweeps >= 0.6 * entries) return SMH_SPMV_COLSPLIT;
        return SMH_SPMV_COLBLOCK;
    }
    const int lanes = mean_lanes(m);
    const double mean = mean_row(m);
    const bool short_ring_rows = mean > 8.0 && m->ring.state == Form::Ready && m->ring.fraction >= 0.5 && m->knobs.use_ring != 0;
    if (mean <= 12.0 && m->max_row_len <= 64 && !short_ring_rows) return SMH_SPMV_STREAM;
    if ((uint64_t)m->max_row_len >= 8ull * 4ull * (uint64_t)lanes && m->max_row_len > 64) return SMH_SPMV_MERGE;
    if (mean > 32.0 && mean <= 128.0 && m->ring.state == Form::Ready && m->ring.fraction < 0.5) return SMH_SPMV_STREAM;
    return SMH_SPMV_VECTOR;
}

static int launch_colblock(const smh_crs *m, const void *x, void *y, hipStream_t s) {
    for (size_t b = 0; b < m->cb.blocks; ++b)
        SMH_TRY(launch_spmv_stream_block(m->dtype, m->cb.off.get() + b * (m->n_rows + 1), m->cb.col.get(), m->cb.val.get(), x, y,
                                         m->n_rows, m->nnz, m->cb.rpt, m->cb.single_pass, b > 0, s));
    return SMH_OK;
}

static int stream_launch(smh_crs *m, const StreamCfg &c, const void *x, size_t x_len, void *y, hipStream_t s, void *dot_partials,
                         const void *dot_lhs, uint64_t t0, uint64_t t1) {
    const bool xs_ok = ((m->dtype == SMH_F64 ? x_len + 1 : ((x_len + 3) & ~(size_t)3)) >= (size_t)m->codes.xs_end) &&
                       (reinterpret_cast<uintptr_t>(x) & 15u) == 0;
    if (c.direct) {
        if (xs_ok && c.xs)
            return launch_spmv_stream_xd(m->dtype, m->d_val, x, y, m->n_rows, dot_partials, c.code, c.cwin, c.len8, c.tbase, dot_lhs, s,
                                         c.xs, t0, t1, c.dict, c.dict_high);
        return launch_spmv_stream(m->dtype, m->d_off, m->d_col, m->d_val, x, y, m->n_rows, m->nnz, m->owns, c.rpt, c.single_pass,
                                  dot_partials, nullptr, nullptr, nullptr, nullptr, dot_lhs, s, false, 0, t0, t1);
    }
    return launch_spmv_stream(m->dtype, m->d_off, m->d_col, m->d_val, x, y, m->n_rows, m->nnz, m->owns, c.rpt, c.single_pass,
                              dot_partials, c.code, c.cwin, c.len8, c.tbase, dot_lhs, s, c.small, xs_ok ? c.xs : 0, t0, t1);
}

static int launch_ring(smh_crs *m, const void *x, void *y, hipStream_t s, void *dot_partials = nullptr, unsigned b0 = 0, unsigned b1 = ~0u) {
    const char *reg_env = getenv("SMH_RING_REGULAR");
    const bool reg_off = reg_env && strcmp(reg_env, "auto") != 0 && atoi(reg_env) == 0;
    const uint32_t *reg_len = m->ring.reg_applies && !reg_off && (m->ring.lo8.get() || m->ring.col16.get()) ? m->ring.reg_len.get() : nullptr;
    return launch_spmv_ring2(m->dtype, auto_lanes(m), auto_chunks(m), m->d_off, m->d_col, m->ring.col16.get(),
                             RingCol12{m->ring.lo8.get(), m->ring.hdr.get(), m->ring.escapes.get()}, m->d_val, x, y, m->n_rows, m->nnz,
                             m->owns || m->nnz % 4 == 0, m->ring.blocks, m->ring.phase_ptr.get(), m->ring.phases.get(), m->ring.entries,
                             m->ring.bands, s, dot_partials, b0, b1, reg_len);
}

size_t spmv_fused_dot_partials(smh_crs *m, size_t x_len, int variant, bool any_lhs) {
    if (const char *e = getenv("SMH_CG_FUSED_DOT")) {
        if (atoi(e) == 0) return 0;
    }
    if (resolve_variant(m, variant) != SMH_SPMV_STREAM) return 0;
    if (!any_lhs && (m->n_rows != m->n_cols || x_len < m->n_rows)) return 0;
    StreamCfg c;
    if (stream_cfg(m, &c) != SMH_OK) return 0;
    return stream_tiles(m->n_rows, c.rpt);
}

static int x_covers_columns(const smh_crs *m, size_t x_len) {
    if (m->nnz > 0 && (size_t)m->max_col >= x_len)
        return fail(SMH_ERR_INDEX_RANGE, "index out of bounds: the len is %zu but the index is %u", x_len, m->max_col);
    return SMH_OK;
}

struct Resolved {
    int v = SMH_SPMV_AUTO;
    bool ring = false;
    StreamCfg stream;
};

static int build_forms(smh_crs *m, Resolved *r, bool eager) {
    switch (r->v) {
        case SMH_SPMV_VECTOR: return vector_uses_ring(m, &r->ring);
        case SMH_SPMV_SEQ: return SMH_OK;
        case SMH_SPMV_STREAM: return stream_cfg(m, &r->stream, eager);
        case SMH_SPMV_COLSPLIT:
            SMH_TRY(ensure_split(m));
            if (m->split.state != Form::Ready) return ensure_colblock(m);
            if (eager) {
                SMH_TRY(smh_crs_prepare(m->split.short_part, SMH_SPMV_AUTO));
                return smh_crs_prepare(m->split.long_part, SMH_SPMV_AUTO);
            }
            return SMH_OK;
        case SMH_SPMV_COLFUSED:
            SMH_TRY(ensure_colfused(m));
            return (m->cf.state == Form::Ready) ? SMH_OK : ensure_colblock(m);
        case SMH_SPMV_COLBLOCK: return ensure_colblock(m);
        case SMH_SPMV_TILED: return tiled_build(m);
        case SMH_SPMV_MERGE: return ensure_merge_ws(m);
        default: return fail(SMH_ERR_INVALID, "unknown SpMV variant %d", r->v);
    }
}

static int resolve_and_build(smh_crs *m, int variant, bool eager, Resolved *r) {
    for (;;) {
        r->v = resolve_variant(m, variant);
        const int rc = build_forms(m, r, eager);
        if (rc == SMH_OK || variant != SMH_SPMV_AUTO || rc == SMH_ERR_INDEX_RANGE || resolve_variant(m, variant) == r->v) return rc;
        clear_error();
    }
}

int prepare_forms(smh_crs *m, int variant) {
    Resolved r;
    return resolve_and_build(m, variant, true, &r);
}

int spmv_enqueue(smh_crs *m, const void *x, size_t x_len, void *y, int variant, hipStream_t s, void *dot_partials, const void *dot_lhs) {
    SMH_TRY(x_covers_columns(m, x_len));
    Resolved r;
// ... 118 lines not shown
```

sparsemat_amd/csrc/spmv_stream_xd.hip:

```cpp
#include "internal.hpp"

namespace smh {

namespace {

typedef uint32_t xd_u4 __attribute__((ext_vector_type(4)));
typedef uint32_t xd_u2 __attribute__((ext_vector_type(2)));
typedef float xd_f4 __attribute__((ext_vector_type(4)));
typedef double xd_d2 __attribute__((ext_vector_type(2)));
constexpr int kXdRsrc = 0x00020000;

__device__ __forceinline__ float xd_mul(float a, float b) { return __fmul_rn(a, b); }
__device__ __forceinline__ double xd_mul(double a, double b) { return __dmul_rn(a, b); }
__device__ __forceinline__ float xd_add(float a, float b) { return __fadd_rn(a, b); }
__device__ __forceinline__ double xd_add(double a, double b) { return __dadd_rn(a, b); }

template <int CTRL, int ROWS> __device__ __forceinline__ uint32_t xd_dpp(uint32_t v) {
    return (uint32_t)__builtin_amdgcn_update_dpp(0, (int)v, CTRL, ROWS, 0xF, false);
}
__device__ __forceinline__ uint32_t xd_wave_scan(uint32_t v) {
    v += xd_dpp<0x111, 0xF>(v);
    v += xd_dpp<0x112, 0xF>(v);
    v += xd_dpp<0x114, 0xF>(v);
    v += xd_dpp<0x118, 0xF>(v);
    v += xd_dpp<0x142, 0xA>(v);
    v += xd_dpp<0x143, 0xC>(v);
    return v;
}

constexpr int kXdSlots = 2 * 4 * kBlock;
static_assert(kStreamCapSmall + 3 <= kXdSlots, "a tile's entries from an aligned start fit two chunks per thread");

template <typename T, int XS> struct XdBits {
    static constexpr uint32_t kLow = sizeof(T) == 8 ? 3u : 2u;
    static constexpr uint32_t kIdx = XS == 4 ? 12u : 11u;
    static constexpr uint32_t kOfsMask = ((1u << (kLow + kIdx)) - 1u) & ~((1u << kLow) - 1u);
    static constexpr uint32_t kValues = 1u << (16u - kIdx);
    static constexpr uint32_t kHigh = 16u - (kLow + kIdx);
    __device__ static __forceinline__ uint32_t ofs(uint32_t c) { return c & kOfsMask; }
    __device__ static __forceinline__ uint32_t vidx(uint32_t c) { return (c & ((1u << kLow) - 1u)) | ((c >> (kLow + kIdx)) << kLow); }
    __device__ static __forceinline__ uint32_t vidx_high(uint32_t c) { return c >> (kLow + kIdx); }
};

template <typename T, bool DOT, int XS, int VD = 0>
__global__ void __launch_bounds__(kBlock)
k_spmv_stream_xd(const T *__restrict__ val, const T *__restrict__ x, T *__restrict__ y, uint64_t n_rows, uint64_t n_tiles,
                 T *__restrict__ dot_partials, const uint16_t *__restrict__ scode, const uint32_t *__restrict__ cwin,
                 const uint8_t *__restrict__ len8, const uint32_t *__restrict__ tbase, const T *__restrict__ dot_lhs, uint64_t tile0,
                 const T *__restrict__ dict = nullptr) {
    constexpr int kXsCap = XS * kBlock * 4;
    __shared__ T s_dict[VD ? 32 : 1];
    T dict_v = T(0);
    if constexpr (VD) dict_v = dict[threadIdx.x & 31u];
    __shared__ __attribute__((aligned(16))) T s_xs[kXsCap];
    __shared__ __attribute__((aligned(16))) T s_prod[kXdSlots + 8];
    __shared__ uint32_t s_wtot[kBlock / kWave];
    const uint64_t q8 = n_tiles >> 3, rm = n_tiles & 7, xcd = blockIdx.x & 7, idx = blockIdx.x >> 3;
    const uint64_t tile = tile0 + (xcd < rm ? xcd * (q8 + 1) : rm * (q8 + 1) + (xcd - rm) * q8) + idx;
    const uint64_t r0 = tile * (uint64_t)kStreamRows;
    const uint32_t tid = threadIdx.x, lane = tid & (kWave - 1);
    const uint32_t wave = (uint32_t)__builtin_amdgcn_readfirstlane((int)(tid / kWave));
    const uint32_t k0 = tbase[tile], k1 = tbase[tile + 1];
    const uint32_t my_len = len8[r0 + tid];
    T dl = T(0);
    if constexpr (DOT) dl = r0 + tid < n_rows ? dot_lhs[r0 + tid] : T(0);
    const uint32_t *w = cwin + 8 * tile;
    const uint32_t cb0 = w[0], e0 = w[1], cb1 = w[2], e1 = w[3], cb2 = w[4], e2 = w[5], cb3 = w[6], e3 = w[7];
    const uint32_t al0 = cb0 & ~3u, al1 = cb1 & ~3u, al2 = cb2 & ~3u, al3 = cb3 & ~3u;
    const uint32_t n0 = e0 > cb0 ? (e0 - al0 + 3u) >> 2 : 0u, n1 = e1 > cb1 ? (e1 - al1 + 3u) >> 2 : 0u;
    const uint32_t n2 = e2 > cb2 ? (e2 - al2 + 3u) >> 2 : 0u, n3 = e3 > cb3 ? (e3 - al3 + 3u) >> 2 : 0u;
    const uint32_t p1 = n0, p2 = p1 + n1, p3 = p2 + n2, xs_tot = p3 + n3;
    const uint32_t d0 = al0 >> 2, d1 = (al1 >> 2) - p1, d2 = (al2 >> 2) - p2, d3 = (al3 >> 2) - p3;
    const uint32_t wbase = tid & ~(uint32_t)(kWave - 1);
    T xr[XS][4];
    uint32_t xpiece[XS][2];
#pragma unroll
    for (int u = 0; u < XS; ++u) {
        xr[u][0] = xr[u][1] = xr[u][2] = xr[u][3] = T(0);
        if constexpr (sizeof(T) == 4) {
            const uint32_t j = tid + (uint32_t)u * kBlock;
            xpiece[u][0] = xpiece[u][1] = 0;
            if (j < xs_tot) {
                uint32_t d = d0;
                d = j >= p1 ? d1 : d;
                d = j >= p2 ? d2 : d;
                d = j >= p3 ? d3 : d;
                const T *g = x + 4ull * (uint64_t)(j + d);
                const xd_f4 a = *reinterpret_cast<const xd_f4 *>(g);
                xr[u][0] = a.x; xr[u][1] = a.y; xr[u][2] = a.z; xr[u][3] = a.w;
            }
        } else {
#pragma unroll
            for (int h = 0; h < 2; ++h) {
                const uint32_t pi = 2u * ((uint32_t)u * kBlock + wbase) + (uint32_t)h * kWave + lane;
                const uint32_t j = pi >> 1;
                xpiece[u][h] = pi;
                if (j < xs_tot) {
                    uint32_t d = d0;
                    d = j >= p1 ? d1 : d;
                    d = j >= p2 ? d2 : d;
                    d = j >= p3 ? d3 : d;
                    const xd_d2 a = *reinterpret_cast<const xd_d2 *>(x + 4ull * (uint64_t)(j + d) + 2u * (pi & 1u));
                    xr[u][2 * h] = a.x; xr[u][2 * h + 1] = a.y;
                }
            }
        }
    }
    const uint32_t pa = k0 & ~3u, hi = k1 - pa;
    const __amdgpu_buffer_rsrc_t rc = __builtin_amdgcn_make_buffer_rsrc((void *)(scode + pa), 0, (int)(((hi + 3u) & ~3u) * 2u), kXdRsrc);
    const __amdgpu_buffer_rsrc_t rv = __builtin_amdgcn_make_buffer_rsrc((void *)(val + pa), 0, (int)(hi * (uint32_t)sizeof(T)), kXdRsrc);
    xd_u2 cw[2];
    T v[2][4];
    uint32_t epos[2][2];
#pragma unroll
    for (int it = 0; it < 2; ++it) {
        v[it][0] = v[it][1] = v[it][2] = v[it][3] = T(0);
        if constexpr (sizeof(T) == 4) {
            const uint32_t j = 4u * tid + (uint32_t)it * (4u * kBlock);
            epos[it][0] = epos[it][1] = 0;
            cw[it] = __builtin_bit_cast(xd_u2, __builtin_amdgcn_raw_buffer_load_b64(rc, (int)(j * 2u), 0, 2 ));
            if constexpr (!VD) {
                const xd_f4 a = __builtin_bit_cast(xd_f4, __builtin_amdgcn_raw_buffer_load_b128(rv, (int)(j * 4u), 0, 2));
                v[it][0] = a.x; v[it][1] = a.y; v[it][2] = a.z; v[it][3] = a.w;
            }
        } else {
            const uint32_t e0p = 4u * ((uint32_t)it * kBlock + wbase) + 2u * lane, e1p = e0p + 2u * kWave;
            epos[it][0] = e0p; epos[it][1] = e1p;
            cw[it].x = __builtin_amdgcn_raw_buffer_load_b32(rc, (int)(e0p * 2u), 0, 2 );
            cw[it].y = __builtin_amdgcn_raw_buffer_load_b32(rc, (int)(e1p * 2u), 0, 2);
            if constexpr (!VD) {
                const xd_d2 a = __builtin_bit_cast(xd_d2, __builtin_amdgcn_raw_buffer_load_b128(rv, (int)(e0p * 8u), 0, 2));
                const xd_d2 b = __builtin_bit_cast(xd_d2, __builtin_amdgcn_raw_buffer_load_b128(rv, (int)(e1p * 8u), 0, 2));
                v[it][0] = a.x; v[it][1] = a.y; v[it][2] = b.x; v[it][3] = b.y;
            }
        }
    }
    const uint32_t incl = xd_wave_scan(my_len);
    if (lane == kWave - 1) s_wtot[wave] = incl;
#pragma unroll
    for (int u = 0; u < XS; ++u) {
        if constexpr (sizeof(T) == 4) {
            const uint32_t j = tid + (uint32_t)u * kBlock;
            if (j < xs_tot) {
                xd_f4 a; a.x = xr[u][0]; a.y = xr[u][1]; a.z = xr[u][2]; a.w = xr[u][3];
                *reinterpret_cast<xd_f4 *>(&s_xs[4u * j]) = a;
            }
        } else {
#pragma unroll
            for (int h = 0; h < 2; ++h)
                if ((xpiece[u][h] >> 1) < xs_tot) {
                    xd_d2 a; a.x = xr[u][2 * h]; a.y = xr[u][2 * h + 1];
                    *reinterpret_cast<xd_d2 *>(&s_xs[2u * xpiece[u][h]]) = a;
                }
        }
    }
    if constexpr (VD) {
        if (tid < 32u) s_dict[tid] = dict_v;
    }
    __syncthreads();
    const char *xs_bytes = reinterpret_cast<const char *>(s_xs);
#pragma unroll
    for (int it = 0; it < 2; ++it) {
        T p[4];
#pragma unroll
        for (int e = 0; e < 4; ++e) {
            const uint32_t cword = (e >> 1) ? cw[it].y : cw[it].x;
            const uint32_t code = (e & 1) ? (cword >> 16) : (cword & 0xFFFFu);
            if constexpr (VD) {
                const uint32_t vi = VD == 2 ? XdBits<T, XS>::vidx_high(code) : XdBits<T, XS>::vidx(code);
                p[e] = xd_mul(*reinterpret_cast<const T *>(xs_bytes + XdBits<T, XS>::ofs(code)), s_dict[vi]);
            } else {
                p[e] = xd_mul(*reinterpret_cast<const T *>(xs_bytes + code), v[it][e]);
            }
        }
        if constexpr (sizeof(T) == 4) {
            const uint32_t j = 4u * tid + (uint32_t)it * (4u * kBlock);
            xd_f4 a; a.x = p[0]; a.y = p[1]; a.z = p[2]; a.w = p[3];
            *reinterpret_cast<xd_f4 *>(&s_prod[j]) = a;
        } else {
            xd_d2 a, b; a.x = p[0]; a.y = p[1]; b.x = p[2]; b.y = p[3];
            *reinterpret_cast<xd_d2 *>(&s_prod[epos[it][0]]) = a;
            *reinterpret_cast<xd_d2 *>(&s_prod[epos[it][1]]) = b;
        }
    }
    __syncthreads();
    uint32_t before = 0;
#pragma unroll
    for (int ww = 0; ww < kBlock / kWave - 1; ++ww) before += (uint32_t)ww < wave ? s_wtot[ww] : 0u;
    const T *pp = s_prod + ((k0 - pa) + before + (incl - my_len));
    T q[8];
#pragma unroll
    for (int i = 0; i < 8; ++i) q[i] = pp[i];
    T acc = T(0);
#pragma unroll
    for (int i = 0; i < 8; ++i)
        if ((uint32_t)i < my_len) acc = xd_add(acc, q[i]);
    for (uint32_t i = 8; i < my_len; ++i) acc = xd_add(acc, pp[i]);
    const uint64_t r = r0 + tid;
    if (r < n_rows && (!DOT || y)) __builtin_nontemporal_store(acc, &y[r]);
    if constexpr (DOT) {
        __shared__ T s_red[kBlock / kWave];
        T d = T(0);
        if (r < n_rows) d += dl * acc;
        d = wave_sum_to_lane63(d);
        if (lane == kWave - 1) s_red[wave] = d;
        __syncthreads();
        if (tid == 0) {
            T t = T(0);
#pragma unroll
            for (int ww = 0; ww < kBlock / kWave; ++ww) t += s_red[ww];
            dot_partials[tile] = t;
        }
    }
}

template <typename T, int XS>
struct XdTileRegs {
    uint32_t k0, pa, my_len, xs_tot;
    uint64_t r0, tile;
    T dl;
    T xr[XS][4];
    uint32_t xpiece[XS][2];
    xd_u2 cw[2];
    uint32_t epos[2][2];
};

template <typename T, bool DOT, int XS, int VD>
__global__ void __launch_bounds__(kBlock)
k_spmv_stream_xdp(const T *__restrict__ x, T *__restrict__ y, uint64_t n_rows, uint64_t n_tiles, T *__restrict__ dot_partials,
                  const uint16_t *__restrict__ scode, const uint32_t *__restrict__ cwin, const uint8_t *__restrict__ len8,
                  const uint32_t *__restrict__ tbase, const T *__restrict__ dot_lhs, uint64_t tile0, const T *__restrict__ dict) {
    static_assert(VD == 1 || VD == 2, "the persistent form exists for the value-dictionary kernels");
    constexpr int kXsCap = XS * kBlock * 4;
    __shared__ T s_dict[32];
    __shared__ __attribute__((aligned(16))) T s_xs[kXsCap];
    __shared__ __attribute__((aligned(16))) T s_prod[kXdSlots + 8];
    __shared__ uint32_t s_wtot[2][kBlock / kWave];
    __shared__ T s_red[2][kBlock / kWave];
    const uint32_t tid = threadIdx.x, lane = tid & (kWave - 1);
    const uint32_t wave = (uint32_t)__builtin_amdgcn_readfirstlane((int)(tid / kWave));
    const uint32_t wbase = tid & ~(uint32_t)(kWave - 1);
    if (tid < 32u) s_dict[tid] = dict[tid];
    const uint64_t q8 = n_tiles >> 3, rm = n_tiles & 7, xcd = blockIdx.x & 7, wgx = gridDim.x >> 3, j_wg = blockIdx.x >> 3;
    const uint64_t xcd_first = xcd < rm ? xcd * (q8 + 1) : rm * (q8 + 1) + (xcd - rm) * q8, xcd_count = q8 + (xcd < rm ? 1u : 0u);
    const uint64_t per = (xcd_count + wgx - 1) / wgx;
    const uint64_t t_begin = xcd_first + j_wg * per;
    const uint64_t t_end = t_begin + per < xcd_first + xcd_count ? t_begin + per : xcd_first + xcd_count;
    if (t_begin >= t_end) return;

    auto load = [&](XdTileRegs<T, XS> &R, uint64_t t) {
        R.tile = tile0 + t;
        R.r0 = R.tile * (uint64_t)kStreamRows;
        const uint32_t k0 = tbase[R.tile], k1 = tbase[R.tile + 1];
        R.k0 = k0;
        R.my_len = len8[R.r0 + tid];
        R.dl = T(0);
        if constexpr (DOT) R.dl = R.r0 + tid < n_rows ? dot_lhs[R.r0 + tid] : T(0);
        const uint32_t *w = cwin + 8 * R.tile;
        const uint32_t cb0 = w[0], e0 = w[1], cb1 = w[2], e1 = w[3], cb2 = w[4], e2 = w[5], cb3 = w[6], e3 = w[7];
        const uint32_t al0 = cb0 & ~3u, al1 = cb1 & ~3u, al2 = cb2 & ~3u, al3 = cb3 & ~3u;
        const uint32_t n0 = e0 > cb0 ? (e0 - al0 + 3u) >> 2 : 0u, n1 = e1 > cb1 ? (e1 - al1 + 3u) >> 2 : 0u;
        const uint32_t n2 = e2 > cb2 ? (e2 - al2 + 3u) >> 2 : 0u, n3 = e3 > cb3 ? (e3 - al3 + 3u) >> 2 : 0u;
        const uint32_t p1 = n0, p2 = p1 + n1, p3 = p2 + n2;
        R.xs_tot = p3 + n3;
        const uint32_t d0 = al0 >> 2, d1 = (al1 >> 2) - p1, d2 = (al2 >> 2) - p2, d3 = (al3 >> 2) - p3;
#pragma unroll
        for (int u = 0; u < XS; ++u) {
            R.xr[u][0] = R.xr[u][1] = R.xr[u][2] = R.xr[u][3] = T(0);
            if constexpr (sizeof(T) == 4) {
                const uint32_t j = tid + (uint32_t)u * kBlock;
                R.xpiece[u][0] = R.xpiece[u][1] = 0;
                if (j < R.xs_tot) {
                    uint32_t d = d0;
                    d = j >= p1 ? d1 : d;
                    d = j >= p2 ? d2 : d;
                    d = j >= p3 ? d3 : d;
                    const xd_f4 a = *reinterpret_cast<const xd_f4 *>(x + 4ull * (uint64_t)(j + d));
                    R.xr[u][0] = a.x; R.xr[u][1] = a.y; R.xr[u][2] = a.z; R.xr[u][3] = a.w;
                }
            } else {
#pragma unroll
                for (int h = 0; h < 2; ++h) {
                    const uint32_t pi = 2u * ((uint32_t)u * kBlock + wbase) + (uint32_t)h * kWave + lane;
                    const uint32_t j = pi >> 1;
                    R.xpiece[u][h] = pi;
                    if (j < R.xs_tot) {
                        uint32_t d = d0;
                        d = j >= p1 ? d1 : d;
                        d = j >= p2 ? d2 : d;
                        d = j >= p3 ? d3 : d;
                        const xd_d2 a = *reinterpret_cast<const xd_d2 *>(x + 4ull * (uint64_t)(j + d) + 2u * (pi & 1u));
                        R.xr[u][2 * h] = a.x; R.xr[u][2 * h + 1] = a.y;
                    }
                }
            }
        }
        const uint32_t pa = k0 & ~3u, hi = k1 - pa;
        R.pa = pa;
        const __amdgpu_buffer_rsrc_t rc = __builtin_amdgcn_make_buffer_rsrc((void *)(scode + pa), 0, (int)(((hi + 3u) & ~3u) * 2u), kXdRsrc);
#pragma unroll
        for (int it = 0; it < 2; ++it) {
            if constexpr (sizeof(T) == 4) {
                const uint32_t j = 4u * tid + (uint32_t)it * (4u * kBlock);
                R.epos[it][0] = j; R.epos[it][1] = j;
                R.cw[it] = __builtin_bit_cast(xd_u2, __builtin_amdgcn_raw_buffer_load_b64(rc, (int)(j * 2u), 0, 2 ));
            } else {
                const uint32_t e0p = 4u * ((uint32_t)it * kBlock + wbase) + 2u * lane, e1p = e0p + 2u * kWave;
                R.epos[it][0] = e0p; R.epos[it][1] = e1p;
                R.cw[it].x = __builtin_amdgcn_raw_buffer_load_b32(rc, (int)(e0p * 2u), 0, 2);
                R.cw[it].y = __builtin_amdgcn_raw_buffer_load_b32(rc, (int)(e1p * 2u), 0, 2);
            }
        }
    };
    auto fold_dot = [&](uint32_t par, uint64_t tile) {
        if (tid == 0) {
            T t = T(0);
#pragma unroll
            for (int ww = 0; ww < kBlock / kWave; ++ww) t += s_red[par][ww];
            dot_partials[tile] = t;
        }
    };
    auto tile_body = [&](XdTileRegs<T, XS> &R, XdTileRegs<T, XS> &N, uint64_t t_next, uint32_t par, bool first) {
        const uint32_t incl = xd_wave_scan(R.my_len);
        if (lane == kWave - 1) s_wtot[par][wave] = incl;
#pragma unroll
        for (int u = 0; u < XS; ++u) {
            if constexpr (sizeof(T) == 4) {
                const uint32_t j = tid + (uint32_t)u * kBlock;
                if (j < R.xs_tot) {
                    xd_f4 a; a.x = R.xr[u][0]; a.y = R.xr[u][1]; a.z = R.xr[u][2]; a.w = R.xr[u][3];
                    *reinterpret_cast<xd_f4 *>(&s_xs[4u * j]) = a;
                }
            } else {
#pragma unroll
                for (int h = 0; h < 2; ++h)
                    if ((R.xpiece[u][h] >> 1) < R.xs_tot) {
                        xd_d2 a; a.x = R.xr[u][2 * h]; a.y = R.xr[u][2 * h + 1];
                        *reinterpret_cast<xd_d2 *>(&s_xs[2u * R.xpiece[u][h]]) = a;
                    }
            }
        }
        __syncthreads();
        if constexpr (DOT) {
            if (!first) fold_dot(par ^ 1u, R.tile - 1);
        }
        load(N, t_next);
        const char *xs_bytes = reinterpret_cast<const char *>(s_xs);
#pragma unroll
        for (int it = 0; it < 2; ++it) {
            T p[4];
#pragma unroll
            for (int e = 0; e < 4; ++e) {
                const uint32_t cword = (e >> 1) ? R.cw[it].y : R.cw[it].x;
                const uint32_t code = (e & 1) ? (cword >> 16) : (cword & 0xFFFFu);
                const uint32_t vi = VD == 2 ? XdBits<T, XS>::vidx_high(code) : XdBits<T, XS>::vidx(code);
                p[e] = xd_mul(*reinterpret_cast<const T *>(xs_bytes + XdBits<T, XS>::ofs(code)), s_dict[vi]);
            }
            if constexpr (sizeof(T) == 4) {
                xd_f4 a; a.x = p[0]; a.y = p[1]; a.z = p[2]; a.w = p[3];
                *reinterpret_cast<xd_f4 *>(&s_prod[R.epos[it][0]]) = a;
            } else {
                xd_d2 a, b; a.x = p[0]; a.y = p[1]; b.x = p[2]; b.y = p[3];
                *reinterpret_cast<xd_d2 *>(&s_prod[R.epos[it][0]]) = a;
                *reinterpret_cast<xd_d2 *>(&s_prod[R.epos[it][1]]) = b;
            }
        }
        __syncthreads();
        uint32_t before = 0;
#pragma unroll
        for (int ww = 0; ww < kBlock / kWave - 1; ++ww) before += (uint32_t)ww < wave ? s_wtot[par][ww] : 0u;
        const T *pp = s_prod + ((R.k0 - R.pa) + before + (incl - R.my_len));
        T q[8];
#pragma unroll
        for (int i = 0; i < 8; ++i) q[i] = pp[i];
        T acc = T(0);
#pragma unroll
        for (int i = 0; i < 8; ++i)
            if ((uint32_t)i < R.my_len) acc = xd_add(acc, q[i]);
        for (uint32_t i = 8; i < R.my_len; ++i) acc = xd_add(acc, pp[i]);
        const uint64_t r = R.r0 + tid;
        if (r < n_rows && (!DOT || y)) __builtin_nontemporal_store(acc, &y[r]);
        if constexpr (DOT) {
            T d = T(0);
            if (r < n_rows) d += R.dl * acc;
            d = wave_sum_to_lane63(d);
            if (lane == kWave - 1) s_red[par][wave] = d;
        }
    };
    XdTileRegs<T, XS> A, B;
    const uint64_t t_last = t_end - 1;
    load(A, t_begin);
    uint32_t last_par = 0;
    for (uint64_t t = t_begin;;) {
        tile_body(A, B, t + 1 < t_end ? t + 1 : t_last, 0u, t == t_begin);
        last_par = 0;
        if (++t >= t_end) break;
        tile_body(B, A, t + 1 < t_end ? t + 1 : t_last, 1u, false);
        last_par = 1;
        if (++t >= t_end) break;
    }
    if constexpr (DOT) {
        __syncthreads();
        fold_dot(last_par, tile0 + t_last);
    }
}

__global__ void __launch_bounds__(kBlock)
k_stream_stage_codes(const uint32_t *__restrict__ off, const uint32_t *__restrict__ col, const uint32_t *__restrict__ win,
                     uint64_t n_rows, uint64_t n_tiles, uint32_t elem_bytes, uint16_t *__restrict__ code) {
    for (uint64_t t = blockIdx.x; t < n_tiles; t += gridDim.x) {
        const uint32_t *w = win + 8 * t;
        const uint32_t a0 = w[0], e0 = w[1], a1 = w[2], e1 = w[3], a2 = w[4], e2 = w[5], a3 = w[6], e3 = w[7];
        const uint32_t al0 = a0 & ~3u, al1 = a1 & ~3u, al2 = a2 & ~3u, al3 = a3 & ~3u;
        const uint32_t n0 = e0 > a0 ? (e0 - al0 + 3u) >> 2 : 0u, n1 = e1 > a1 ? (e1 - al1 + 3u) >> 2 : 0u;
        const uint32_t n2 = e2 > a2 ? (e2 - al2 + 3u) >> 2 : 0u;
        const uint32_t p1 = n0, p2 = p1 + n1, p3 = p2 + n2;
        const uint64_t r0 = t * kStreamRows, r1 = r0 + kStreamRows < n_rows ? r0 + kStreamRows : n_rows;
        const uint64_t k0 = off[r0], k1 = off[r1];
        for (uint64_t k = k0 + threadIdx.x; k < k1; k += kBlock) {
            const uint32_t c = col[k];
            const uint32_t q = (uint32_t)(e1 > a1 && c >= a1) + (uint32_t)(e2 > a2 && c >= a2) + (uint32_t)(e3 > a3 && c >= a3);
            const uint32_t al = q == 3u ? al3 : q == 2u ? al2 : q == 1u ? al1 : al0;
            const uint32_t pq = q == 3u ? p3 : q == 2u ? p2 : q == 1u ? p1 : 0u;
            code[k] = (uint16_t)((4u * pq + (c - al)) * elem_bytes);
// ... 16 lines not shown
            if (old == empty || old == pat) return true;
        }
    }
    return false;
}

template <typename T>
__global__ void __launch_bounds__(kBlock)
k_value_dict_collect(const T *__restrict__ val, uint64_t nnz, typename XdPat<T>::U *__restrict__ wg_tables, uint32_t *__restrict__ overflow) {
    typedef typename XdPat<T>::U U;
    __shared__ U tab[kXdDictCap];
    if (threadIdx.x < kXdDictCap) tab[threadIdx.x] = XdPat<T>::kEmpty;
    __syncthreads();
    const U *bits = reinterpret_cast<const U *>(val);
    for (uint64_t i = (uint64_t)blockIdx.x * kBlock + threadIdx.x; i < nnz; i += (uint64_t)gridDim.x * kBlock) {
        if (*(volatile uint32_t *)overflow) break;
        const U pat = bits[i];
        if (pat == XdPat<T>::kEmpty || !xd_dict_insert<U>(tab, pat, XdPat<T>::kEmpty)) { atomicOr(overflow, 1u); break; }
    }
    __syncthreads();
    if (threadIdx.x < kXdDictCap) wg_tables[(uint64_t)blockIdx.x * kXdDictCap + threadIdx.x] = tab[threadIdx.x];
}

template <typename T>
__global__ void __launch_bounds__(kBlock)
k_value_dict_merge(const typename XdPat<T>::U *__restrict__ wg_tables, uint32_t n_tables, T *__restrict__ dict, uint32_t *__restrict__ count,
                   uint32_t *__restrict__ overflow) {
    typedef typename XdPat<T>::U U;
    __shared__ U tab[kXdDictCap];
    __shared__ uint32_t s_over;
    if (threadIdx.x < kXdDictCap) tab[threadIdx.x] = XdPat<T>::kEmpty;
    if (threadIdx.x == 0) s_over = *overflow;
    __syncthreads();
    if (!s_over) {
        for (uint32_t i = threadIdx.x; i < n_tables * kXdDictCap; i += kBlock) {
            const U pat = wg_tables[i];
            if (pat != XdPat<T>::kEmpty && !xd_dict_insert<U>(tab, pat, XdPat<T>::kEmpty)) s_over = 1u;
        }
    }
    __syncthreads();
    if (threadIdx.x == 0) {
        uint32_t n = 0;
        U sorted[kXdDictCap];
        for (uint32_t i = 0; i < kXdDictCap; ++i)
            if (tab[i] != XdPat<T>::kEmpty) sorted[n++] = tab[i];
        for (uint32_t i = 1; i < n; ++i) {
            const U v = sorted[i];
            uint32_t j = i;
            while (j > 0 && sorted[j - 1] > v) { sorted[j] = sorted[j - 1]; --j; }
            sorted[j] = v;
        }
        U *out = reinterpret_cast<U *>(dict);
        for (uint32_t i = 0; i < kXdDictCap; ++i) out[i] = i < n ? sorted[i] : (U)0;
        *count = s_over ? 0u : n;
        *overflow = s_over;
    }
}

template <typename T>
__global__ void __launch_bounds__(kBlock)
k_value_dict_encode(const T *__restrict__ val, uint64_t nnz, const T *__restrict__ dict, uint32_t n, uint32_t low, uint32_t high_shift,
                    uint16_t *__restrict__ code) {
    typedef typename XdPat<T>::U U;
    __shared__ U tab[kXdDictCap];
    if (threadIdx.x < kXdDictCap) tab[threadIdx.x] = reinterpret_cast<const U *>(dict)[threadIdx.x];
    __syncthreads();
    const U *bits = reinterpret_cast<const U *>(val);
    for (uint64_t k = (uint64_t)blockIdx.x * kBlock + threadIdx.x; k < nnz; k += (uint64_t)gridDim.x * kBlock) {
        const U pat = bits[k];
        uint32_t idx = 0;
        for (uint32_t i = 0; i < n; ++i) idx = tab[i] == pat ? i : idx;
        const uint32_t lowmask = (1u << low) - 1u;
        code[k] = (uint16_t)(code[k] | (idx & lowmask) | ((idx >> low) << high_shift));
    }
}

__global__ void __launch_bounds__(kBlock)
k_stream_odd_rows(const uint8_t *__restrict__ len8, uint64_t n, unsigned long long *__restrict__ out) {
    uint32_t c = 0;
    for (uint64_t i = (uint64_t)blockIdx.x * blockDim.x + threadIdx.x; i < n; i += (uint64_t)gridDim.x * blockDim.x) c += len8[i] & 1u;
#pragma unroll
    for (int o = kWave / 2; o > 0; o >>= 1) c += (uint32_t)__shfl_down((int)c, o, kWave);
    if ((threadIdx.x & (kWave - 1)) == 0 && c) atomicAdd(out, (unsigned long long)c);
}

template <typename T, int XS, int VD> int xdp_resident(bool dot) {
    static int res[2] = {0, 0};
    if (res[0] == 0 || res[1] == 0) {
        int a = 0, b = 0;
        if (hipOccupancyMaxActiveBlocksPerMultiprocessor(&a, k_spmv_stream_xdp<T, false, XS, VD>, kBlock, 0) == hipSuccess && a > 0) res[0] = a;
        if (hipOccupancyMaxActiveBlocksPerMultiprocessor(&b, k_spmv_stream_xdp<T, true, XS, VD>, kBlock, 0) == hipSuccess && b > 0) res[1] = b;
        (void)hipGetLastError();
    }
    const int r = res[dot ? 1 : 0];
    return r > 0 ? r : (sizeof(T) == 8 ? 4 : 8);
}

template <typename T>
int launch_xd_t(const T *val, const T *x, T *y, size_t n_rows, T *dot_partials, const uint16_t *scode, const uint32_t *cwin,
                const uint8_t *len8, const uint32_t *tbase, const T *dot_lhs, hipStream_t s, int xs, uint64_t tile_begin, uint64_t tile_end,
                const T *dict, bool dict_high) {
    const uint64_t all_tiles = stream_tiles(n_rows, 1);
    const uint64_t tile0 = tile_begin < all_tiles ? tile_begin : all_tiles, tile1 = tile_end < all_tiles ? tile_end : all_tiles;
    if (tile1 <= tile0) return SMH_OK;
    const uint64_t n_tiles = tile1 - tile0;
    const dim3 grid((unsigned)n_tiles), block(kBlock);
    static const int persist_env = getenv("SMH_STREAM_PERSIST") ? atoi(getenv("SMH_STREAM_PERSIST")) : -1;
    const bool persist = persist_env < 0 ? sizeof(T) == 8 : persist_env != 0;
    if (dict && persist && (xs == 2 || xs == 4)) {
        static int cus_cache[64] = {};
        int dev = 0;
        (void)hipGetDevice(&dev);
        int &cus = cus_cache[dev & 63];
        if (cus == 0) {
            hipDeviceProp_t prop;
            cus = hipGetDeviceProperties(&prop, dev) == hipSuccess && prop.multiProcessorCount > 0 ? prop.multiProcessorCount : 256;
        }
        static const int per_cu_env = getenv("SMH_STREAM_PERSIST_WGS") ? atoi(getenv("SMH_STREAM_PERSIST_WGS")) : 0;
#define SMH_XDP(D, P, V)                                                                                                           \
    do {                                                                                                                           \
        const int resident = xdp_resident<T, P, V>(D);                          \
        uint64_t wgx = (uint64_t)(cus / 8 > 0 ? cus / 8 : 1) * (uint64_t)(per_cu_env > 0 ? per_cu_env : resident);    \
        if (wgx > (n_tiles + 7) / 8) wgx = (n_tiles + 7) / 8;                                                                      \
        if (wgx < 1) wgx = 1;                                                                                                      \
        hipLaunchKernelGGL((k_spmv_stream_xdp<T, D, P, V>), dim3((unsigned)(8 * wgx)), block, 0, s, x, y, (uint64_t)n_rows, n_tiles, \
                           dot_partials, scode, cwin, len8, tbase, dot_lhs, tile0, dict);                                          \
    } while (0)
#define SMH_XDP2(P)                                                                              \
    do {                                                                                         \
        if (dict_high) { if (dot_partials) SMH_XDP(true, P, 2); else SMH_XDP(false, P, 2); }    \
        else { if (dot_partials) SMH_XDP(true, P, 1); else SMH_XDP(false, P, 1); }              \
    } while (0)
        if (xs == 2) SMH_XDP2(2); else SMH_XDP2(4);
#undef SMH_XDP2
#undef SMH_XDP
        SMH_HIP(hipGetLastError());
        return SMH_OK;
    }
#define SMH_XD(D, P, V)                                                                                                              \
    hipLaunchKernelGGL((k_spmv_stream_xd<T, D, P, V>), grid, block, 0, s, val, x, y, (uint64_t)n_rows, n_tiles, dot_partials, scode, \
                       cwin, len8, tbase, dot_lhs, tile0, dict)
#define SMH_XD2(P)                                                                                  \
    do {                                                                                            \
        if (dict && dict_high) { if (dot_partials) SMH_XD(true, P, 2); else SMH_XD(false, P, 2); } \
        else if (dict) { if (dot_partials) SMH_XD(true, P, 1); else SMH_XD(false, P, 1); }         \
        else { if (dot_partials) SMH_XD(true, P, 0); else SMH_XD(false, P, 0); }                   \
    } while (0)
    if (xs == 2) SMH_XD2(2);
    else if (xs == 4) SMH_XD2(4);
    else return fail(SMH_ERR_INVALID, "K1s XD: the stage of x holds 2 or 4 chunks per thread");
#undef SMH_XD2
#undef SMH_XD
    SMH_HIP(hipGetLastError());
    return SMH_OK;
}

}

int launch_spmv_stream_xd(int dtype, const void *val, const void *x, void *y, size_t n_rows, void *dot_partials, const uint16_t *scode,
                          const uint32_t *cwin, const uint8_t *len8, const uint32_t *tbase, const void *dot_lhs, hipStream_t s, int xs,
                          uint64_t tile_begin, uint64_t tile_end, const void *dict, bool dict_high) {
    if (n_rows == 0) return SMH_OK;
    if (dot_partials && !dot_lhs) dot_lhs = x;
    if (!dot_partials && !y) return fail(SMH_ERR_INVALID, "K1s: no output");
    if (dtype == SMH_F64)
        return launch_xd_t<double>((const double *)val, (const double *)x, (double *)y, n_rows, (double *)dot_partials, scode, cwin, len8,
                                   tbase, (const double *)dot_lhs, s, xs, tile_begin, tile_end, (const double *)dict, dict_high);
    return launch_xd_t<float>((const float *)val, (const float *)x, (float *)y, n_rows, (float *)dot_partials, scode, cwin, len8, tbase,
                              (const float *)dot_lhs, s, xs, tile_begin, tile_end, (const float *)dict, dict_high);
}

template <typename T>
static int value_dict_t(const T *val, size_t nnz, T *dict_out, uint32_t *count_out, hipStream_t s) {
    typedef typename XdPat<T>::U U;
    *count_out = 0;
    if (nnz == 0) return SMH_OK;
    uint64_t blocks = (nnz + (uint64_t)kBlock * 64 - 1) / ((uint64_t)kBlock * 64);
    blocks = blocks < 1 ? 1 : (blocks > 1024 ? 1024 : blocks);
    U *tables = nullptr;
    uint32_t *flags = nullptr;
    SMH_HIP(hipMalloc((void **)&tables, blocks * kXdDictCap * sizeof(U)));
    hipError_t e = hipMalloc((void **)&flags, 2 * sizeof(uint32_t));
    uint32_t h[2] = {1u, 0u};
    auto go = [&]() -> int {
        SMH_HIP(e);
        SMH_HIP(hipMemsetAsync(flags, 0, 2 * sizeof(uint32_t), s));
        hipLaunchKernelGGL(k_value_dict_collect<T>, dim3((unsigned)blocks), dim3(kBlock), 0, s, val, (uint64_t)nnz, tables, flags);
        SMH_HIP(hipGetLastError());
        hipLaunchKernelGGL(k_value_dict_merge<T>, dim3(1), dim3(kBlock), 0, s, (const U *)tables, (uint32_t)blocks, dict_out, flags + 1, flags);
        SMH_HIP(hipGetLastError());
        SMH_HIP(hipMemcpyAsync(h, flags, sizeof h, hipMemcpyDeviceToHost, s));
        SMH_HIP(hipStreamSynchronize(s));
        return SMH_OK;
    };
    const int rc = go();
    (void)hipFree(tables);
    (void)hipFree(flags);
    SMH_TRY(rc);
    *count_out = h[0] ? 0u : h[1];
    return SMH_OK;
}

int stream_value_dict(int dtype, const void *val, size_t nnz, void *dict_out, uint32_t *count_out, hipStream_t s) {
    return dtype == SMH_F64 ? value_dict_t<double>((const double *)val, nnz, (double *)dict_out, count_out, s)
                            : value_dict_t<float>((const float *)val, nnz, (float *)dict_out, count_out, s);
}

bool stream_value_dict_high(int dtype, uint32_t n, int xs) {
    const uint32_t low = dtype == SMH_F64 ? 3u : 2u, high_shift = low + (xs == 4 ? 12u : 11u);
    return n <= (1u << (16u - high_shift));
}

int launch_stream_value_codes(int dtype, const void *val, size_t nnz, const void *dict, uint32_t n, int xs, uint16_t *code, hipStream_t s) {
    if (nnz == 0) return SMH_OK;
    const uint32_t high_shift = (dtype == SMH_F64 ? 3u : 2u) + (xs == 4 ? 12u : 11u);
    const uint32_t low = stream_value_dict_high(dtype, n, xs) ? 0u : (dtype == SMH_F64 ? 3u : 2u);
    uint64_t blocks = (nnz + kBlock - 1) / kBlock;
    if (blocks > 16384) blocks = 16384;
    if (dtype == SMH_F64)
        hipLaunchKernelGGL(k_value_dict_encode<double>, dim3((unsigned)blocks), dim3(kBlock), 0, s, (const double *)val, (uint64_t)nnz, (const double *)dict, n, low, high_shift, code);
    else
        hipLaunchKernelGGL(k_value_dict_encode<float>, dim3((unsigned)blocks), dim3(kBlock), 0, s, (const float *)val, (uint64_t)nnz, (const float *)dict, n, low, high_shift, code);
    SMH_HIP(hipGetLastError());
    return SMH_OK;
}

uint32_t stream_value_dict_capacity(int xs) { return xs == 4 ? 16u : 32u; }

int launch_stream_stage_codes(const uint32_t *off, const uint32_t *col, const uint32_t *win, size_t n_rows, uint32_t elem_bytes,
                              uint16_t *code, hipStream_t s) {
    const uint64_t n_tiles = (n_rows + kStreamRows - 1) / kStreamRows;
    if (n_tiles == 0) return SMH_OK;
    const uint64_t blocks = n_tiles < 16384 ? n_tiles : 16384;
    hipLaunchKernelGGL(k_stream_stage_codes, dim3((unsigned)blocks), dim3(kBlock), 0, s, off, col, win, (uint64_t)n_rows, n_tiles, elem_bytes, code);
    SMH_HIP(hipGetLastError());
    return SMH_OK;
}

int launch_stream_odd_rows(const uint8_t *len8, size_t n_padded, unsigned long long *d_out, hipStream_t s) {
// ... 11 lines not shown
```

sparsemat_amd/sparsemat_crs.py:

```python
import ctypes as C
import numbers

import numpy as np

from . import _lib
from ._lib import check, lib
from .densevec import DenseVec
from .multivec import MultiVec, pack_host


def _index(i):
    i = int(i)
    if not 0 <= i <= 0xFFFFFFFF:
        raise _lib.SparseMatPanic(_lib.SMH_ERR_INVALID, "index %d does not fit the u32 index type" % i)
    return i


class SparseMatCRS:
    def __init__(self, handle, dtype, keep=None):
        self._h = handle
        self._dtype = np.dtype(dtype)
        self._keep = keep

    @classmethod
# ... 393 lines not shown
                out[name] = buf
            out["chunks"] = out["chunks"].reshape(-1, 2)
            out["tile_start"] = out["tile_start"].reshape(d.value + 1, a.value)
        return out

    def colsplit_flag(self):
        flag = C.c_int()
        check(lib().smh_crs_colsplit(self._h, C.byref(flag), None, None, None, None, None))
        return bool(flag.value)

    def colsplit(self):
        flag, ml, nl = C.c_int(), C.c_uint32(), C.c_size_t()
        check(lib().smh_crs_colsplit(self._h, C.byref(flag), C.byref(ml), C.byref(nl), None, None, None))
        out = {"split": bool(flag.value), "min_long": ml.value, "n_long": nl.value}
        if out["split"]:
            rows = np.zeros(nl.value, np.uint32)
            hl, hs = C.c_void_p(), C.c_void_p()
            check(lib().smh_crs_colsplit(self._h, None, None, None, rows.ctypes.data, C.byref(hl), C.byref(hs)))
            out["long_rows"] = rows
            for name, h in (("long", hl), ("short", hs)):
                nr, nnz = lib().smh_crs_n_rows(h), lib().smh_crs_nnz(h)
                off, col, val = np.zeros(nr + 1, np.uint32), np.zeros(nnz, np.uint32), np.zeros(nnz, self._dtype)
                check(lib().smh_crs_download(h, off.ctypes.data, col.ctypes.data if nnz else None, val.ctypes.data if nnz else None))
                var, lanes = C.c_int(), C.c_int()
                check(lib().smh_crs_resolved_variant(h, C.byref(var), C.byref(lanes)))
                out[name] = (nr, off, col, val)
                out[name + "_variant"] = {1: "vector", 2: "merge", 3: "seq", 4: "stream", 5: "colblock", 6: "colfused", 7: "colsplit", 8: "tiled"}[var.value]
        return out

    def colfused(self, arrays=True):
        fits, sh, nb, rt, nt = C.c_int(), C.c_uint32(), C.c_size_t(), C.c_uint32(), C.c_size_t()
        check(lib().smh_crs_colfused(self._h, C.byref(fits), C.byref(sh), C.byref(nb), C.byref(rt), C.byref(nt), None, None, None, None, None))
        out = {"fits": bool(fits.value), "shift": sh.value, "n_blocks": nb.value, "rows_per_lane": rt.value, "n_tiles": nt.value}
        if arrays and out["fits"]:
            nnz = self.n_non_zero_entries()
            tiles = np.zeros(nt.value + 1, np.uint32)
            seg = np.zeros(nt.value * nb.value + 1, np.uint32)
            cnt = np.zeros(nt.value * nb.value * 64 * rt.value, np.uint8)
            col = np.zeros(nnz, np.uint32)
            val = np.zeros(nnz, self._dtype)
            check(lib().smh_crs_colfused(self._h, None, None, None, None, None, tiles.ctypes.data, seg.ctypes.data,
                                         cnt.ctypes.data if len(cnt) else None, col.ctypes.data if nnz else None,
                                         val.ctypes.data if nnz else None))
            out.update(tile_rows=tiles, segments=seg, counts=cnt, columns=col, values=val)
        return out

    def colblock(self, arrays=True):
        sh, nb, rpt, span = C.c_uint32(), C.c_size_t(), C.c_int(), C.c_double()
        check(lib().smh_crs_colblock(self._h, C.byref(sh), C.byref(nb), C.byref(rpt), C.byref(span), None, None, None))
        out = dict(shift=sh.value, n_blocks=nb.value, rows_per_thread=rpt.value, span_fraction=span.value)
        if arrays:
            nnz = self.n_non_zero_entries()
            off = np.zeros((nb.value, self.n_rows() + 1), dtype=np.uint32)
            col = np.zeros(nnz, dtype=np.uint32)
            val = np.zeros(nnz, dtype=self._dtype)
            check(lib().smh_crs_colblock(self._h, None, None, None, None, off.ctypes.data,
                                         col.ctypes.data if nnz else None, val.ctypes.data if nnz else None))
            out.update(offsets=off, columns=col, values=val)
        return out

    def set_vector_lanes(self, lanes):
        check(lib().smh_crs_set_vector_lanes(self._h, lanes))

    def set_stream_xs(self, mode):
        check(lib().smh_crs_set_stream_xs(self._h, mode))

    def set_stream_direct(self, mode):
        check(lib().smh_crs_set_stream_direct(self._h, mode))

    def stream_direct(self):
        a = C.c_int()
        check(lib().smh_crs_stream_direct(self._h, C.byref(a)))
        return bool(a.value)

    def stream_value_dict(self):
        n = C.c_int()
        buf = np.zeros(32, dtype=self.dtype)
        check(lib().smh_crs_stream_value_dict(self._h, C.byref(n), buf.ctypes.data))
        return buf[:n.value].copy()

    def set_stream_value_dict(self, mode):
        check(lib().smh_crs_set_stream_value_dict(self._h, int(mode)))

    def stream_layout(self):
        a, b, c, d = C.c_int(), C.c_int(), C.c_int(), C.c_int()
        check(lib().smh_crs_stream_layout(self._h, C.byref(a), C.byref(b), C.byref(c), C.byref(d)))
        return {"coded": bool(a.value), "byte_lengths": bool(b.value), "small_tiles": bool(c.value), "xs_chunks": d.value}

    def set_vector_chunks(self, chunks):
        check(lib().smh_crs_set_vector_chunks(self._h, chunks))

    def set_ring(self, mode):
        check(lib().smh_crs_set_ring(self._h, mode))

    def ring_entries(self):
        out = C.c_uint32()
        check(lib().smh_crs_ring_entries(self._h, C.byref(out)))
        return out.value

    def ring_column_form(self):
        out = C.c_int()
        check(lib().smh_crs_ring_column_form(self._h, C.byref(out)))
        return ("u32", "col16", "col12")[out.value]

    def ring_bands(self, intervals=False):
        bands = C.c_uint32()
        check(lib().smh_crs_ring_bands(self._h, C.byref(bands), None))
        if not intervals:
            return bands.value
        if bands.value != 4:
            return bands.value, None
        table = np.zeros(((self.n_rows() + 63) // 64, 4, 2), dtype=np.uint32)
        check(lib().smh_crs_ring_bands(self._h, C.byref(bands), table.ctypes.data))
        return bands.value, table

    def ring_plan(self):
        nb, nph, frac, act = C.c_uint32(), C.c_size_t(), C.c_double(), C.c_int()
        check(lib().smh_crs_ring_plan(self._h, C.byref(nb), C.byref(nph), C.byref(frac), C.byref(act), None, None))
        ptr = np.zeros(nb.value + 1, dtype=np.uint32)
        ph = np.zeros((nph.value, 11), dtype=np.uint32)
        check(lib().smh_crs_ring_plan(self._h, None, None, None, None, ptr.ctypes.data,
                                      ph.ctypes.data if nph.value else None))
        return nb.value, frac.value, bool(act.value), ptr, ph

    def ring_regular(self):
        nph = C.c_size_t()
        check(lib().smh_crs_ring_plan(self._h, None, C.byref(nph), None, None, None, None))
        out = np.zeros(nph.value, dtype=np.uint32)
        if nph.value:
            check(lib().smh_crs_ring_regular(self._h, out.ctypes.data))
        return out

    def max_row_len(self):
        out = C.c_uint32()
        check(lib().smh_crs_max_row_len(self._h, C.byref(out)))
        return out.value

    def col_range(self):
        lo, hi = C.c_uint32(), C.c_uint32()
        check(lib().smh_crs_col_range(self._h, C.byref(lo), C.byref(hi)))
        return lo.value, hi.value

    def merge_table(self):
        n = lib().smh_crs_merge_tiles(self._h)
        rows = np.zeros(n + 1, dtype=np.uint32)
        nz = np.zeros(n + 1, dtype=np.uint32)
        check(lib().smh_crs_merge_table(self._h, rows.ctypes.data, nz.ctypes.data))
        return rows, nz, lib().smh_crs_merge_tile_items(self._h)

    def mvp(self, rhs, variant="auto"):
        var = _lib.VARIANTS[variant]
        if isinstance(rhs, DenseVec):
            ret = DenseVec.zeros(self.n_rows(), self._dtype)
            check(lib().smh_crs_spmv_vec(self._h, rhs._h, ret._h, var))
            return ret
        x = np.ascontiguousarray(rhs, dtype=self._dtype)
        y = np.zeros(self.n_rows(), dtype=self._dtype)
        check(lib().smh_crs_spmv(self._h, x.ctypes.data if x.size else None, x.size,
                                 y.ctypes.data if y.size else None, var))
        return y

    def mvp_many(self, rhs):
        if isinstance(rhs, MultiVec):
            ret = MultiVec.zeros(self.n_rows(), rhs.count(), self._dtype)
            check(lib().smh_crs_spmv_many(self._h, rhs._h, ret._h))
            return ret
# ... 81 lines not shown
```

Baseline: 8273.

## Add diagonal-structure stream SpMV kernel that encodes entries by per-row diagonal masks

Adds a new stream form that detects matrices whose nonzeros lie on at most eight diagonal offsets with at most eight distinct values. Each row is encoded as an 8-bit mask plus a per-tile x-stage offset, replacing the per-entry codes and value reads with a tiny value table. A new kernel, with an optional persistent-grid variant, consumes this form, and it is enabled automatically when the value-dictionary path applies. This cuts matrix bytes streamed per nonzero substantially, at the cost of a host-synchronising build pass and a narrow eligibility check.

```diff
diff --git a/include/sparsemat_hip.h b/include/sparsemat_hip.h
--- a/include/sparsemat_hip.h
+++ b/include/sparsemat_hip.h
@@ -128,6 +128,8 @@
 int smh_crs_stream_layout(smh_crs *m, int *coded_out, int *byte_lengths_out, int *small_tiles_out, int *xs_chunks_out);
 int smh_crs_stream_value_dict(smh_crs *m, int *n_values_out, void *values_out);
 int smh_crs_set_stream_value_dict(smh_crs *m, int mode);
+int smh_crs_stream_diag(smh_crs *m, int *k_out, int64_t *offsets_out, void *values_out);
+int smh_crs_set_stream_diag(smh_crs *m, int mode);
 int smh_crs_set_stream_direct(smh_crs *m, int mode);
 int smh_crs_stream_direct(smh_crs *m, int *direct_out);
 int smh_crs_set_vector_chunks(smh_crs *m, int chunks);
diff --git a/rust/src/ffi.rs b/rust/src/ffi.rs
--- a/rust/src/ffi.rs
+++ b/rust/src/ffi.rs
@@ -93,6 +93,8 @@
     pub fn smh_crs_bandwidth(m: *const smh_crs, lower_out: *mut u32, upper_out: *mut u32) -> c_int;
     pub fn smh_crs_span_fraction(m: *mut smh_crs, out: *mut f64) -> c_int;
     pub fn smh_crs_ring_regular(m: *mut smh_crs, len_out: *mut u32) -> c_int;
+    pub fn smh_crs_stream_diag(m: *mut smh_crs, k_out: *mut c_int, offsets_out: *mut i64, values_out: *mut c_void) -> c_int;
+    pub fn smh_crs_set_stream_diag(m: *mut smh_crs, mode: c_int) -> c_int;
     pub fn smh_crs_rcm(m: *const smh_crs, perm_out: *mut u32, n_components_out: *mut usize, n_levels_out: *mut usize) -> c_int;
     pub fn smh_crs_rcm_dev(m: *const smh_crs, perm_out_dev: *mut u32, n_components_out: *mut usize, n_levels_out: *mut usize) -> c_int;
     pub fn smh_crs_color(m: *const smh_crs, seed: u32, colors_out: *mut u32, perm_out: *mut u32, n_colors_out: *mut usize, n_rounds_out: *mut usize) -> c_int;
diff --git a/sparsemat_amd/_lib.py b/sparsemat_amd/_lib.py
--- a/sparsemat_amd/_lib.py
+++ b/sparsemat_amd/_lib.py
@@ -245,6 +245,8 @@
     "smh_crs_stream_layout": (_int, [_vp, C.POINTER(_int), C.POINTER(_int), C.POINTER(_int), C.POINTER(_int)]),
     "smh_crs_stream_value_dict": (_int, [_vp, C.POINTER(C.c_int), _vp]),
     "smh_crs_set_stream_value_dict": (_int, [_vp, _int]),
+    "smh_crs_stream_diag": (_int, [_vp, C.POINTER(C.c_int), _vp, _vp]),
+    "smh_crs_set_stream_diag": (_int, [_vp, _int]),
     "smh_last_transpose_route": (_int, []),
     "smh_pool_trim": (_int, []),
     "smh_pool_stats": (_int, [C.POINTER(_sz), C.POINTER(_sz)]),
diff --git a/sparsemat_amd/csrc/capi.hip b/sparsemat_amd/csrc/capi.hip
--- a/sparsemat_amd/csrc/capi.hip
+++ b/sparsemat_amd/csrc/capi.hip
@@ -1039,6 +1039,7 @@
         SMH_HIP(hipStreamSynchronize(m->stream));
     }
     if (m->dict.state == Form::Ready) SMH_TRY(launch_scale_values(m->dtype, m->dict.values.get(), 32, a, m->stream));
+    if (m->diag.state == Form::Ready) SMH_TRY(launch_scale_values(m->dtype, m->diag.values.get(), 8, a, m->stream));
     if (m->cb.state == Form::Ready) SMH_TRY(launch_scale_values(m->dtype, m->cb.val.get(), m->nnz, a, m->stream));
     if (m->cf.state == Form::Ready) SMH_TRY(launch_scale_values(m->dtype, m->cf.val.get(), m->nnz, a, m->stream));
     if (m->tiled.state == Form::Ready) SMH_TRY(launch_scale_values(m->dtype, m->tiled.val.get(), (size_t)m->tiled.tot, a, m->stream));
@@ -1180,6 +1181,27 @@
     if (!m) return fail(SMH_ERR_INVALID, "NULL handle");
     if (mode < -1 || mode > 0) return fail(SMH_ERR_INVALID, "mode must be -1 (automatic: whenever the values allow) or 0 (never)");
     m->knobs.use_stream_vdict = mode;
+    return recode_stream(m);
+}
+
+int smh_crs_stream_diag(smh_crs *m, int *k_out, int64_t *offsets_out, void *values_out) {
+    if (!m || !k_out) return fail(SMH_ERR_INVALID, "NULL argument");
+    StreamCfg c;
+    SMH_TRY(stream_cfg(m, &c));
+    *k_out = c.diag ? (int)c.diag->k : 0;
+    if (c.diag && offsets_out)
+        for (uint32_t i = 0; i < 8; ++i) offsets_out[i] = i < c.diag->k ? (int64_t)c.diag->offsets[i] : 0;
+    if (c.diag && values_out) {
+        SMH_HIP(hipMemcpyAsync(values_out, c.diag->values.get(), (size_t)c.diag->k * dtype_size(m->dtype), hipMemcpyDeviceToHost, m->stream));
+        SMH_HIP(hipStreamSynchronize(m->stream));
+    }
+    return SMH_OK;
+}
+
+int smh_crs_set_stream_diag(smh_crs *m, int mode) {
+    if (!m) return fail(SMH_ERR_INVALID, "NULL handle");
+    if (mode < -1 || mode > 1) return fail(SMH_ERR_INVALID, "mode must be -1 (automatic), 0 (never) or 1 (wherever the matrix is eligible)");
+    m->knobs.use_stream_diag = mode;
     return recode_stream(m);
 }
 
diff --git a/sparsemat_amd/csrc/crs_forms.hip b/sparsemat_amd/csrc/crs_forms.hip
--- a/sparsemat_amd/csrc/crs_forms.hip
+++ b/sparsemat_amd/csrc/crs_forms.hip
@@ -259,6 +259,8 @@
     if (join) (void)hipEventDestroy(join);
 }
 
+static const bool kStreamDiagAutoF32 = true, kStreamDiagAutoF64 = true;
+
 static int ensure_stream_codes(smh_crs *m) {
     if (m->codes.state != Form::NotTried) return SMH_OK;
     StreamCodes c;
@@ -373,14 +375,35 @@
     m->split = RowSplit();
     m->tiled = Tiled();
     if (what == Changed::Values) m->dict.state = Form::NotTried;
+    if (what == Changed::Values && m->diag.state != Form::NotTried) m->diag.state = Form::NotTried;
     if (what == Changed::Order) {
         m->codes = StreamCodes();
+        m->diag = StreamDiag();
         m->ring.col16.reset();
         drop_ring_col12(m);
         m->ring.c12 = Form::NotTried;
         m->tri[0] = TriSchedule();
         m->tri[1] = TriSchedule();
     }
+}
+
+static int ensure_stream_diag(smh_crs *m) {
+    if (m->diag.state != Form::NotTried) return SMH_OK;
+    StreamDiag &d = m->diag;
+    const size_t n_tiles = (m->n_rows + kStreamRows - 1) / kStreamRows;
+    if (!d.mask8.get()) SMH_TRY(d.mask8.alloc(n_tiles * kStreamRows));
+    if (!d.dstage.get()) SMH_TRY(d.dstage.alloc(n_tiles * 8));
+    if (!d.values.get()) SMH_TRY(d.values.alloc(8 * dtype_size(m->dtype)));
+    uint32_t k = 0;
+    SMH_TRY(stream_diag_build(m->dtype, m->d_off, m->d_col, m->d_val, m->n_rows, m->codes.cwin.get(), d.mask8.get(), d.dstage.get(),
+                              d.values.get(), &k, d.offsets, m->stream));
+    d.k = k;
+    d.state = k ? Form::Ready : Form::Refused;
+    if (!k) {
+        d.mask8.reset();
+        d.dstage.reset();
+    }
+    return SMH_OK;
 }
 
 static int stream_rpt(const smh_crs *m) {
@@ -445,6 +468,15 @@
         c->direct = c->code && m->codes.direct;
         c->dict = c->direct && m->codes.vdict ? m->dict.values.get() : nullptr;
         c->dict_high = c->dict && stream_value_dict_high(m->dtype, m->dict.n, m->codes.vdict_xs);
+        const char *dg_env = getenv("SMH_STREAM_DIAG");
+        const int dg_mode = m->knobs.use_stream_diag >= 0 ? m->knobs.use_stream_diag : (dg_env && *dg_env ? (atoi(dg_env) ? 1 : 0) : -1);
+        const bool want_diag = c->dict && (c->xs == 2 || c->xs == 4) &&
+                               (dg_mode == 1 || (dg_mode < 0 && (m->dtype == SMH_F64 ? kStreamDiagAutoF64 : kStreamDiagAutoF32)));
+        if (recode && want_diag && m->diag.state == Form::NotTried) {
+            SMH_HIP(hipDeviceSynchronize());
+            SMH_TRY(ensure_stream_diag(m));
+        }
+        c->diag = want_diag && m->diag.state == Form::Ready ? &m->diag : nullptr;
     }
     return SMH_OK;
 }
diff --git a/sparsemat_amd/csrc/crs_forms.hpp b/sparsemat_amd/csrc/crs_forms.hpp
--- a/sparsemat_amd/csrc/crs_forms.hpp
+++ b/sparsemat_amd/csrc/crs_forms.hpp
@@ -40,6 +40,7 @@
     bool direct = false;
     const void *dict = nullptr;
     bool dict_high = false;
+    const StreamDiag *diag = nullptr;
 };
 int stream_cfg(::smh_crs *m, StreamCfg *c, bool recode = false);
 int recode_stream(::smh_crs *m);
diff --git a/sparsemat_amd/csrc/internal.hpp b/sparsemat_amd/csrc/internal.hpp
--- a/sparsemat_amd/csrc/internal.hpp
+++ b/sparsemat_amd/csrc/internal.hpp
@@ -336,6 +336,11 @@
 int stream_value_dict(int dtype, const void *val, size_t nnz, void *dict_out, uint32_t *count_out, hipStream_t s);
 int launch_stream_value_codes(int dtype, const void *val, size_t nnz, const void *dict, uint32_t n, int xs, uint16_t *code, hipStream_t s);
 uint32_t stream_value_dict_capacity(int xs);
+int stream_diag_build(int dtype, const uint32_t *off, const uint32_t *col, const void *val, size_t n_rows, const uint32_t *cwin,
+                      uint8_t *mask8, uint16_t *dstage, void *values, uint32_t *k_out, long long *offsets_out, hipStream_t s);
+int launch_spmv_stream_xdd(int dtype, const void *x, void *y, size_t n_rows, void *dot_partials, const uint32_t *cwin, const uint8_t *mask8,
+                           const uint16_t *dstage, const void *values, uint32_t k, const void *dot_lhs, hipStream_t s, int xs,
+                           uint64_t tile_begin = 0, uint64_t tile_end = ~uint64_t(0));
 int launch_stream_stage_codes(const uint32_t *off, const uint32_t *col, const uint32_t *win, size_t n_rows, uint32_t elem_bytes,
                               uint16_t *code, hipStream_t s);
 int launch_stream_odd_rows(const uint8_t *len8, size_t n_padded, unsigned long long *d_out, hipStream_t s);
@@ -594,6 +599,14 @@
     uint32_t n = 0;
     DevArray<char> values;
 };
+struct StreamDiag {
+    Form state = Form::NotTried;
+    uint32_t k = 0;
+    long long offsets[8] = {};
+    DevArray<uint8_t> mask8;
+    DevArray<uint16_t> dstage;
+    DevArray<char> values;
+};
 struct ColBlock {
     Form state = Form::NotTried;
     uint32_t shift = 0;
@@ -681,6 +694,7 @@
     int use_stream_xs = -1;
     int use_stream_direct = -1;
     int use_stream_vdict = -1;
+    int use_stream_diag = -1;
     int use_col16 = -1;
     int use_col12 = -1;
 };
@@ -718,6 +732,7 @@
     smh::RingPlan ring;
     smh::StreamCodes codes;
     smh::StreamDict dict;
+    smh::StreamDiag diag;
     smh::ColBlock cb;
     smh::ColFused cf;
     smh::RowSplit split;
diff --git a/sparsemat_amd/csrc/spmv_dispatch.hip b/sparsemat_amd/csrc/spmv_dispatch.hip
--- a/sparsemat_amd/csrc/spmv_dispatch.hip
+++ b/sparsemat_amd/csrc/spmv_dispatch.hip
@@ -102,6 +102,9 @@
     const bool xs_ok = ((m->dtype == SMH_F64 ? x_len + 1 : ((x_len + 3) & ~(size_t)3)) >= (size_t)m->codes.xs_end) &&
                        (reinterpret_cast<uintptr_t>(x) & 15u) == 0;
     if (c.direct) {
+        if (xs_ok && c.xs && c.diag)
+            return launch_spmv_stream_xdd(m->dtype, x, y, m->n_rows, dot_partials, c.cwin, c.diag->mask8.get(), c.diag->dstage.get(),
+                                          c.diag->values.get(), c.diag->k, dot_lhs, s, c.xs, t0, t1);
         if (xs_ok && c.xs)
             return launch_spmv_stream_xd(m->dtype, m->d_val, x, y, m->n_rows, dot_partials, c.code, c.cwin, c.len8, c.tbase, dot_lhs, s,
                                          c.xs, t0, t1, c.dict, c.dict_high);
diff --git a/sparsemat_amd/csrc/spmv_stream_xd.hip b/sparsemat_amd/csrc/spmv_stream_xd.hip
--- a/sparsemat_amd/csrc/spmv_stream_xd.hip
+++ b/sparsemat_amd/csrc/spmv_stream_xd.hip
@@ -30,6 +30,77 @@
 
 constexpr int kXdSlots = 2 * 4 * kBlock;
 static_assert(kStreamCapSmall + 3 <= kXdSlots, "a tile's entries from an aligned start fit two chunks per thread");
+
+template <typename T, int XS>
+struct XdStage {
+    uint32_t xs_tot;
+    T xr[XS][4];
+    uint32_t xpiece[XS][2];
+    __device__ __forceinline__ void request_from(const T *__restrict__ x, const uint32_t *__restrict__ w , uint32_t tid) {
+        const uint32_t wv[8] = {w[0], w[1], w[2], w[3], w[4], w[5], w[6], w[7]};
+        request(x, wv, tid);
+    }
+    __device__ __forceinline__ void request(const T *__restrict__ x, const uint32_t (&w)[8], uint32_t tid) {
+        const uint32_t lane = tid & (kWave - 1), wbase = tid & ~(uint32_t)(kWave - 1);
+        const uint32_t cb0 = w[0], e0 = w[1], cb1 = w[2], e1 = w[3], cb2 = w[4], e2 = w[5], cb3 = w[6], e3 = w[7];
+        const uint32_t al0 = cb0 & ~3u, al1 = cb1 & ~3u, al2 = cb2 & ~3u, al3 = cb3 & ~3u;
+        const uint32_t n0 = e0 > cb0 ? (e0 - al0 + 3u) >> 2 : 0u, n1 = e1 > cb1 ? (e1 - al1 + 3u) >> 2 : 0u;
+        const uint32_t n2 = e2 > cb2 ? (e2 - al2 + 3u) >> 2 : 0u, n3 = e3 > cb3 ? (e3 - al3 + 3u) >> 2 : 0u;
+        const uint32_t p1 = n0, p2 = p1 + n1, p3 = p2 + n2;
+        xs_tot = p3 + n3;
+        const uint32_t d0 = al0 >> 2, d1 = (al1 >> 2) - p1, d2 = (al2 >> 2) - p2, d3 = (al3 >> 2) - p3;
+#pragma unroll
+        for (int u = 0; u < XS; ++u) {
+            xr[u][0] = xr[u][1] = xr[u][2] = xr[u][3] = T(0);
+            if constexpr (sizeof(T) == 4) {
+                const uint32_t j = tid + (uint32_t)u * kBlock;
+                xpiece[u][0] = xpiece[u][1] = 0;
+                if (j < xs_tot) {
+                    uint32_t d = d0;
+                    d = j >= p1 ? d1 : d;
+                    d = j >= p2 ? d2 : d;
+                    d = j >= p3 ? d3 : d;
+                    const xd_f4 a = *reinterpret_cast<const xd_f4 *>(x + 4ull * (uint64_t)(j + d));
+                    xr[u][0] = a.x; xr[u][1] = a.y; xr[u][2] = a.z; xr[u][3] = a.w;
+                }
+            } else {
+#pragma unroll
+                for (int h = 0; h < 2; ++h) {
+                    const uint32_t pi = 2u * ((uint32_t)u * kBlock + wbase) + (uint32_t)h * kWave + lane;
+                    const uint32_t j = pi >> 1;
+                    xpiece[u][h] = pi;
+                    if (j < xs_tot) {
+                        uint32_t d = d0;
+                        d = j >= p1 ? d1 : d;
+                        d = j >= p2 ? d2 : d;
+                        d = j >= p3 ? d3 : d;
+                        const xd_d2 a = *reinterpret_cast<const xd_d2 *>(x + 4ull * (uint64_t)(j + d) + 2u * (pi & 1u));
+                        xr[u][2 * h] = a.x; xr[u][2 * h + 1] = a.y;
+                    }
+                }
+            }
+        }
+    }
+    __device__ __forceinline__ void put(T *__restrict__ s_xs, uint32_t tid) const {
+#pragma unroll
+        for (int u = 0; u < XS; ++u) {
+            if constexpr (sizeof(T) == 4) {
+                const uint32_t j = tid + (uint32_t)u * kBlock;
+                if (j < xs_tot) {
+                    xd_f4 a; a.x = xr[u][0]; a.y = xr[u][1]; a.z = xr[u][2]; a.w = xr[u][3];
+                    *reinterpret_cast<xd_f4 *>(&s_xs[4u * j]) = a;
+                }
+            } else {
+#pragma unroll
+                for (int h = 0; h < 2; ++h)
+                    if ((xpiece[u][h] >> 1) < xs_tot) {
+                        xd_d2 a; a.x = xr[u][2 * h]; a.y = xr[u][2 * h + 1];
+                        *reinterpret_cast<xd_d2 *>(&s_xs[2u * xpiece[u][h]]) = a;
+                    }
+            }
+        }
+    }
+};
 
 template <typename T, int XS> struct XdBits {
     static constexpr uint32_t kLow = sizeof(T) == 8 ? 3u : 2u;
@@ -64,48 +135,9 @@
     const uint32_t my_len = len8[r0 + tid];
     T dl = T(0);
     if constexpr (DOT) dl = r0 + tid < n_rows ? dot_lhs[r0 + tid] : T(0);
-    const uint32_t *w = cwin + 8 * tile;
-    const uint32_t cb0 = w[0], e0 = w[1], cb1 = w[2], e1 = w[3], cb2 = w[4], e2 = w[5], cb3 = w[6], e3 = w[7];
-    const uint32_t al0 = cb0 & ~3u, al1 = cb1 & ~3u, al2 = cb2 & ~3u, al3 = cb3 & ~3u;
-    const uint32_t n0 = e0 > cb0 ? (e0 - al0 + 3u) >> 2 : 0u, n1 = e1 > cb1 ? (e1 - al1 + 3u) >> 2 : 0u;
-    const uint32_t n2 = e2 > cb2 ? (e2 - al2 + 3u) >> 2 : 0u, n3 = e3 > cb3 ? (e3 - al3 + 3u) >> 2 : 0u;
-    const uint32_t p1 = n0, p2 = p1 + n1, p3 = p2 + n2, xs_tot = p3 + n3;
-    const uint32_t d0 = al0 >> 2, d1 = (al1 >> 2) - p1, d2 = (al2 >> 2) - p2, d3 = (al3 >> 2) - p3;
+    XdStage<T, XS> st;
+    st.request_from(x, cwin + 8 * tile, tid);
     const uint32_t wbase = tid & ~(uint32_t)(kWave - 1);
-    T xr[XS][4];
-    uint32_t xpiece[XS][2];
-#pragma unroll
-    for (int u = 0; u < XS; ++u) {
-        xr[u][0] = xr[u][1] = xr[u][2] = xr[u][3] = T(0);
-        if constexpr (sizeof(T) == 4) {
-            const uint32_t j = tid + (uint32_t)u * kBlock;
-            xpiece[u][0] = xpiece[u][1] = 0;
-            if (j < xs_tot) {
-                uint32_t d = d0;
-                d = j >= p1 ? d1 : d;
-                d = j >= p2 ? d2 : d;
-                d = j >= p3 ? d3 : d;
-                const T *g = x + 4ull * (uint64_t)(j + d);
-                const xd_f4 a = *reinterpret_cast<const xd_f4 *>(g);
-                xr[u][0] = a.x; xr[u][1] = a.y; xr[u][2] = a.z; xr[u][3] = a.w;
-            }
-        } else {
-#pragma unroll
-            for (int h = 0; h < 2; ++h) {
-                const uint32_t pi = 2u * ((uint32_t)u * kBlock + wbase) + (uint32_t)h * kWave + lane;
-                const uint32_t j = pi >> 1;
-                xpiece[u][h] = pi;
-                if (j < xs_tot) {
-                    uint32_t d = d0;
-                    d = j >= p1 ? d1 : d;
-                    d = j >= p2 ? d2 : d;
-                    d = j >= p3 ? d3 : d;
-                    const xd_d2 a = *reinterpret_cast<const xd_d2 *>(x + 4ull * (uint64_t)(j + d) + 2u * (pi & 1u));
-                    xr[u][2 * h] = a.x; xr[u][2 * h + 1] = a.y;
-                }
-            }
-        }
-    }
     const uint32_t pa = k0 & ~3u, hi = k1 - pa;
     const __amdgpu_buffer_rsrc_t rc = __builtin_amdgcn_make_buffer_rsrc((void *)(scode + pa), 0, (int)(((hi + 3u) & ~3u) * 2u), kXdRsrc);
     const __amdgpu_buffer_rsrc_t rv = __builtin_amdgcn_make_buffer_rsrc((void *)(val + pa), 0, (int)(hi * (uint32_t)sizeof(T)), kXdRsrc);
@@ -137,23 +169,7 @@
     }
     const uint32_t incl = xd_wave_scan(my_len);
     if (lane == kWave - 1) s_wtot[wave] = incl;
-#pragma unroll
-    for (int u = 0; u < XS; ++u) {
-        if constexpr (sizeof(T) == 4) {
-            const uint32_t j = tid + (uint32_t)u * kBlock;
-            if (j < xs_tot) {
-                xd_f4 a; a.x = xr[u][0]; a.y = xr[u][1]; a.z = xr[u][2]; a.w = xr[u][3];
-                *reinterpret_cast<xd_f4 *>(&s_xs[4u * j]) = a;
-            }
-        } else {
-#pragma unroll
-            for (int h = 0; h < 2; ++h)
-                if ((xpiece[u][h] >> 1) < xs_tot) {
-                    xd_d2 a; a.x = xr[u][2 * h]; a.y = xr[u][2 * h + 1];
-                    *reinterpret_cast<xd_d2 *>(&s_xs[2u * xpiece[u][h]]) = a;
-                }
-        }
-    }
+    st.put(s_xs, tid);
     if constexpr (VD) {
         if (tid < 32u) s_dict[tid] = dict_v;
     }
@@ -216,11 +232,10 @@
 
 template <typename T, int XS>
 struct XdTileRegs {
-    uint32_t k0, pa, my_len, xs_tot;
+    uint32_t k0, pa, my_len;
     uint64_t r0, tile;
     T dl;
-    T xr[XS][4];
-    uint32_t xpiece[XS][2];
+    XdStage<T, XS> st;
     xd_u2 cw[2];
     uint32_t epos[2][2];
 };
@@ -256,45 +271,7 @@
         R.my_len = len8[R.r0 + tid];
         R.dl = T(0);
         if constexpr (DOT) R.dl = R.r0 + tid < n_rows ? dot_lhs[R.r0 + tid] : T(0);
-        const uint32_t *w = cwin + 8 * R.tile;
-        const uint32_t cb0 = w[0], e0 = w[1], cb1 = w[2], e1 = w[3], cb2 = w[4], e2 = w[5], cb3 = w[6], e3 = w[7];
-        const uint32_t al0 = cb0 & ~3u, al1 = cb1 & ~3u, al2 = cb2 & ~3u, al3 = cb3 & ~3u;
-        const uint32_t n0 = e0 > cb0 ? (e0 - al0 + 3u) >> 2 : 0u, n1 = e1 > cb1 ? (e1 - al1 + 3u) >> 2 : 0u;
-        const uint32_t n2 = e2 > cb2 ? (e2 - al2 + 3u) >> 2 : 0u, n3 = e3 > cb3 ? (e3 - al3 + 3u) >> 2 : 0u;
-        const uint32_t p1 = n0, p2 = p1 + n1, p3 = p2 + n2;
-        R.xs_tot = p3 + n3;
-        const uint32_t d0 = al0 >> 2, d1 = (al1 >> 2) - p1, d2 = (al2 >> 2) - p2, d3 = (al3 >> 2) - p3;
-#pragma unroll
-        for (int u = 0; u < XS; ++u) {
-            R.xr[u][0] = R.xr[u][1] = R.xr[u][2] = R.xr[u][3] = T(0);
-            if constexpr (sizeof(T) == 4) {
-                const uint32_t j = tid + (uint32_t)u * kBlock;
-                R.xpiece[u][0] = R.xpiece[u][1] = 0;
-                if (j < R.xs_tot) {
-                    uint32_t d = d0;
-                    d = j >= p1 ? d1 : d;
-                    d = j >= p2 ? d2 : d;
-                    d = j >= p3 ? d3 : d;
-                    const xd_f4 a = *reinterpret_cast<const xd_f4 *>(x + 4ull * (uint64_t)(j + d));
-                    R.xr[u][0] = a.x; R.xr[u][1] = a.y; R.xr[u][2] = a.z; R.xr[u][3] = a.w;
-                }
-            } else {
-#pragma unroll
-                for (int h = 0; h < 2; ++h) {
-                    const uint32_t pi = 2u * ((uint32_t)u * kBlock + wbase) + (uint32_t)h * kWave + lane;
-                    const uint32_t j = pi >> 1;
-                    R.xpiece[u][h] = pi;
-                    if (j < R.xs_tot) {
-                        uint32_t d = d0;
-                        d = j >= p1 ? d1 : d;
-                        d = j >= p2 ? d2 : d;
-                        d = j >= p3 ? d3 : d;
-                        const xd_d2 a = *reinterpret_cast<const xd_d2 *>(x + 4ull * (uint64_t)(j + d) + 2u * (pi & 1u));
-                        R.xr[u][2 * h] = a.x; R.xr[u][2 * h + 1] = a.y;
-                    }
-                }
-            }
-        }
+        R.st.request_from(x, cwin + 8 * R.tile, tid);
         const uint32_t pa = k0 & ~3u, hi = k1 - pa;
         R.pa = pa;
         const __amdgpu_buffer_rsrc_t rc = __builtin_amdgcn_make_buffer_rsrc((void *)(scode + pa), 0, (int)(((hi + 3u) & ~3u) * 2u), kXdRsrc);
@@ -323,23 +300,7 @@
     auto tile_body = [&](XdTileRegs<T, XS> &R, XdTileRegs<T, XS> &N, uint64_t t_next, uint32_t par, bool first) {
         const uint32_t incl = xd_wave_scan(R.my_len);
         if (lane == kWave - 1) s_wtot[par][wave] = incl;
-#pragma unroll
-        for (int u = 0; u < XS; ++u) {
-            if constexpr (sizeof(T) == 4) {
-                const uint32_t j = tid + (uint32_t)u * kBlock;
-                if (j < R.xs_tot) {
-                    xd_f4 a; a.x = R.xr[u][0]; a.y = R.xr[u][1]; a.z = R.xr[u][2]; a.w = R.xr[u][3];
-                    *reinterpret_cast<xd_f4 *>(&s_xs[4u * j]) = a;
-                }
-            } else {
-#pragma unroll
-                for (int h = 0; h < 2; ++h)
-                    if ((R.xpiece[u][h] >> 1) < R.xs_tot) {
-                        xd_d2 a; a.x = R.xr[u][2 * h]; a.y = R.xr[u][2 * h + 1];
-                        *reinterpret_cast<xd_d2 *>(&s_xs[2u * R.xpiece[u][h]]) = a;
-                    }
-            }
-        }
+        R.st.put(s_xs, tid);
         __syncthreads();
         if constexpr (DOT) {
             if (!first) fold_dot(par ^ 1u, R.tile - 1);
@@ -522,6 +483,326 @@
 #pragma unroll
     for (int o = kWave / 2; o > 0; o >>= 1) c += (uint32_t)__shfl_down((int)c, o, kWave);
     if ((threadIdx.x & (kWave - 1)) == 0 && c) atomicAdd(out, (unsigned long long)c);
+}
+
+constexpr uint32_t kXddNone = 0x7FFFu;
+
+struct XddScal {
+    uint32_t w[8], ds[4];
+};
+template <typename T, int XS>
+struct XddTile {
+    uint64_t r0, tile;
+    uint32_t mask, ds[4];
+    T dl;
+    XdStage<T, XS> st;
+};
+
+__device__ __forceinline__ void xdd_scal(XddScal &S, const uint32_t *__restrict__ cwin, const uint32_t *__restrict__ dstage, uint64_t tile) {
+#pragma unroll
+    for (int i = 0; i < 8; ++i) S.w[i] = cwin[8 * tile + i];
+#pragma unroll
+    for (int i = 0; i < 4; ++i) S.ds[i] = dstage[4 * tile + i];
+}
+template <typename T, bool DOT, int XS>
+__device__ __forceinline__ void xdd_request(XddTile<T, XS> &R, const XddScal &S, uint64_t tile, const T *__restrict__ x, const uint8_t *__restrict__ mask8,
+                                            const T *__restrict__ dot_lhs, uint64_t n_rows, uint32_t tid) {
+    R.tile = tile;
+    R.r0 = tile * (uint64_t)kStreamRows;
+    R.mask = mask8[R.r0 + tid];
+    R.dl = T(0);
+    if constexpr (DOT) R.dl = R.r0 + tid < n_rows ? dot_lhs[R.r0 + tid] : T(0);
+    R.st.request(x, S.w, tid);
+#pragma unroll
+    for (int i = 0; i < 4; ++i) R.ds[i] = S.ds[i];
+}
+__device__ __forceinline__ float xdd_mul(float a, float b) { float r; asm("v_mul_f32 %0, %1, %2" : "=v"(r) : "v"(a), "v"(b)); return r; }
+__device__ __forceinline__ double xdd_mul(double a, double b) { double r; asm("v_mul_f64 %0, %1, %2" : "=v"(r) : "v"(a), "v"(b)); return r; }
+__device__ __forceinline__ float xdd_add(float a, float b) { float r; asm("v_add_f32 %0, %1, %2" : "=v"(r) : "v"(a), "v"(b)); return r; }
+__device__ __forceinline__ double xdd_add(double a, double b) { double r; asm("v_add_f64 %0, %1, %2" : "=v"(r) : "v"(a), "v"(b)); return r; }
+template <typename T> __device__ __forceinline__ void xdd_values(T (&v)[8], const T *__restrict__ vtab) {
+#pragma unroll
+    for (int k = 0; k < 8; ++k) v[k] = vtab[k];
+}
+template <typename T, int XS>
+__device__ __forceinline__ T xdd_row_sum(const T *s_xs, const uint32_t (&ds)[4], uint32_t mask, uint32_t tid, uint32_t K, const T (&v)[8]) {
+    constexpr int kLast = XS * kBlock * 4 - 1;
+    T q[8];
+#pragma unroll
+    for (int k = 0; k < 8; ++k) {
+        q[k] = T(0);
+        if ((uint32_t)k < K) {
+            int i = (int)(int16_t)(uint16_t)(ds[k >> 1] >> (16 * (k & 1))) + (int)tid;
+            i = i < 0 ? 0 : i;
+            i = i > kLast ? kLast : i;
+            q[k] = s_xs[i];
+        }
+    }
+    T acc = T(0);
+#pragma unroll
+    for (int k = 0; k < 8; ++k) {
+        if ((uint32_t)k < K) {
+            const T s = xdd_add(acc, xdd_mul(q[k], v[k]));
+            acc = (mask >> k) & 1u ? s : acc;
+        }
+    }
+    return acc;
+}
+
+template <typename T, bool DOT, int XS>
+__global__ void __launch_bounds__(kBlock)
+k_spmv_stream_xdd(const T *__restrict__ x, T *__restrict__ y, uint64_t n_rows, uint64_t n_tiles, T *__restrict__ dot_partials,
+                  const uint32_t *__restrict__ cwin, const uint8_t *__restrict__ mask8, const uint32_t *__restrict__ dstage,
+                  const T *__restrict__ vtab, uint32_t K, const T *__restrict__ dot_lhs, uint64_t tile0) {
+    constexpr int kXsCap = XS * kBlock * 4;
+    __shared__ __attribute__((aligned(16))) T s_xs[kXsCap];
+    const uint64_t q8 = n_tiles >> 3, rm = n_tiles & 7, xcd = blockIdx.x & 7, idx = blockIdx.x >> 3;
+    const uint64_t tile = tile0 + (xcd < rm ? xcd * (q8 + 1) : rm * (q8 + 1) + (xcd - rm) * q8) + idx;
+    const uint32_t tid = threadIdx.x, lane = tid & (kWave - 1);
+    const uint32_t wave = (uint32_t)__builtin_amdgcn_readfirstlane((int)(tid / kWave));
+    XddScal S;
+    xdd_scal(S, cwin, dstage, tile);
+    XddTile<T, XS> R;
+    xdd_request<T, DOT, XS>(R, S, tile, x, mask8, dot_lhs, n_rows, tid);
+    T v[8];
+    xdd_values(v, vtab);
+    R.st.put(s_xs, tid);
+    __syncthreads();
+    const T acc = xdd_row_sum<T, XS>(s_xs, R.ds, R.mask, tid, K, v);
+    const uint64_t r = R.r0 + tid;
+    if (r < n_rows && (!DOT || y)) __builtin_nontemporal_store(acc, &y[r]);
+    if constexpr (DOT) {
+        __shared__ T s_red[kBlock / kWave];
+        T d = T(0);
+        if (r < n_rows) d += R.dl * acc;
+        d = wave_sum_to_lane63(d);
+        if (lane == kWave - 1) s_red[wave] = d;
+        __syncthreads();
+        if (tid == 0) {
+            T t = T(0);
+#pragma unroll
+            for (int ww = 0; ww < kBlock / kWave; ++ww) t += s_red[ww];
+            dot_partials[tile] = t;
+        }
+    }
+}
+
+template <typename T, bool DOT, int XS>
+__global__ void __launch_bounds__(kBlock)
+k_spmv_stream_xddp(const T *__restrict__ x, T *__restrict__ y, uint64_t n_rows, uint64_t n_tiles, T *__restrict__ dot_partials,
+                   const uint32_t *__restrict__ cwin, const uint8_t *__restrict__ mask8, const uint32_t *__restrict__ dstage,
+                   const T *__restrict__ vtab, uint32_t K, const T *__restrict__ dot_lhs, uint64_t tile0) {
+    constexpr int kXsCap = XS * kBlock * 4;
+    __shared__ __attribute__((aligned(16))) T s_xs[2][kXsCap];
+    __shared__ T s_red[2][kBlock / kWave];
+    const uint32_t tid = threadIdx.x, lane = tid & (kWave - 1);
+    const uint32_t wave = (uint32_t)__builtin_amdgcn_readfirstlane((int)(tid / kWave));
+    const uint64_t q8 = n_tiles >> 3, rm = n_tiles & 7, xcd = blockIdx.x & 7, wgx = gridDim.x >> 3, j_wg = blockIdx.x >> 3;
+    const uint64_t xcd_first = xcd < rm ? xcd * (q8 + 1) : rm * (q8 + 1) + (xcd - rm) * q8, xcd_count = q8 + (xcd < rm ? 1u : 0u);
+    const uint64_t per = (xcd_count + wgx - 1) / wgx;
+    const uint64_t t_begin = xcd_first + j_wg * per;
+    const uint64_t t_end = t_begin + per < xcd_first + xcd_count ? t_begin + per : xcd_first + xcd_count;
+    if (t_begin >= t_end) return;
+    const uint64_t t_last = t_end - 1;
+    T v[8];
+    xdd_values(v, vtab);
+    auto fold_dot = [&](uint32_t par, uint64_t tile) {
+        if (tid == 0) {
+            T t = T(0);
+#pragma unroll
+            for (int ww = 0; ww < kBlock / kWave; ++ww) t += s_red[par][ww];
+            dot_partials[tile] = t;
+        }
+    };
+    XddScal S;
+    auto tile_body = [&](XddTile<T, XS> &R, XddTile<T, XS> &N, uint64_t t, uint32_t par, bool first) {
+        R.st.put(s_xs[par], tid);
+        __syncthreads();
+        if constexpr (DOT) {
+            if (!first) fold_dot(par ^ 1u, R.tile - 1);
+        }
+        xdd_request<T, DOT, XS>(N, S, tile0 + (t + 1 < t_end ? t + 1 : t_last), x, mask8, dot_lhs, n_rows, tid);
+        xdd_scal(S, cwin, dstage, tile0 + (t + 2 < t_end ? t + 2 : t_last));
+        const T acc = xdd_row_sum<T, XS>(s_xs[par], R.ds, R.mask, tid, K, v);
+        const uint64_t r = R.r0 + tid;
+        if (r < n_rows && (!DOT || y)) __builtin_nontemporal_store(acc, &y[r]);
+        if constexpr (DOT) {
+            T d = T(0);
+            if (r < n_rows) d += R.dl * acc;
+            d = wave_sum_to_lane63(d);
+            if (lane == kWave - 1) s_red[par][wave] = d;
+        }
+    };
+    XddTile<T, XS> A, B;
+    xdd_scal(S, cwin, dstage, tile0 + t_begin);
+    xdd_request<T, DOT, XS>(A, S, tile0 + t_begin, x, mask8, dot_lhs, n_rows, tid);
+    xdd_scal(S, cwin, dstage, tile0 + (t_begin + 1 < t_end ? t_begin + 1 : t_last));
+    uint32_t last_par = 0;
+    for (uint64_t t = t_begin;;) {
+        tile_body(A, B, t, 0u, t == t_begin);
+        last_par = 0;
+        if (++t >= t_end) break;
+        tile_body(B, A, t, 1u, false);
+        last_par = 1;
+        if (++t >= t_end) break;
+    }
+    if constexpr (DOT) {
+        __syncthreads();
+        fold_dot(last_par, tile0 + t_last);
+    }
+}
+
+constexpr unsigned long long kXddNoOffset = 0x8000000000000000ull;
+
+template <typename U>
+__device__ __forceinline__ bool xd_tab_insert8(U *tab, U pat, U empty) {
+    for (uint32_t i = 0; i < 8; ++i) {
+        const U seen = tab[i];
+        if (seen == pat) return true;
+        if (seen == empty) {
+            const U old = atomicCAS(tab + i, empty, pat);
+            if (old == empty || old == pat) return true;
+        }
+    }
+    return false;
+}
+
+__global__ void __launch_bounds__(kBlock)
+k_diag_collect(const uint32_t *__restrict__ off, const uint32_t *__restrict__ col, uint64_t n_rows, unsigned long long *__restrict__ wg_tables,
+               uint32_t *__restrict__ fail) {
+    __shared__ unsigned long long tab[8];
+    if (threadIdx.x < 8) tab[threadIdx.x] = kXddNoOffset;
+    __syncthreads();
+    for (uint64_t r = (uint64_t)blockIdx.x * kBlock + threadIdx.x; r < n_rows; r += (uint64_t)gridDim.x * kBlock) {
+        if (*(volatile uint32_t *)fail) break;
+        const uint32_t k0 = off[r], k1 = off[r + 1];
+        bool ok = true;
+        uint32_t prev = 0;
+        for (uint32_t k = k0; k < k1 && ok; ++k) {
+            const uint32_t c = col[k];
+            ok = (k == k0 || c > prev) && xd_tab_insert8<unsigned long long>(tab, (unsigned long long)((long long)c - (long long)r), kXddNoOffset);
+            prev = c;
+        }
+        if (!ok) { atomicOr(fail, 1u); break; }
+    }
+    __syncthreads();
+    if (threadIdx.x < 8) wg_tables[(uint64_t)blockIdx.x * 8 + threadIdx.x] = tab[threadIdx.x];
+}
+
+__global__ void __launch_bounds__(kBlock)
+k_diag_merge(const unsigned long long *__restrict__ wg_tables, uint32_t n_tables, long long *__restrict__ out, uint32_t *__restrict__ count,
+             uint32_t *__restrict__ fail) {
+    __shared__ unsigned long long tab[8];
+    __shared__ uint32_t s_fail;
+    if (threadIdx.x < 8) tab[threadIdx.x] = kXddNoOffset;
+    if (threadIdx.x == 0) s_fail = *fail;
+    __syncthreads();
+    if (!s_fail) {
+        for (uint32_t i = threadIdx.x; i < n_tables * 8; i += kBlock) {
+            const unsigned long long pat = wg_tables[i];
+            if (pat != kXddNoOffset && !xd_tab_insert8<unsigned long long>(tab, pat, kXddNoOffset)) s_fail = 1u;
+        }
+    }
+    __syncthreads();
+    if (threadIdx.x == 0) {
+        uint32_t n = 0;
+        long long sorted[8];
+        for (uint32_t i = 0; i < 8; ++i)
+            if (tab[i] != kXddNoOffset) sorted[n++] = (long long)tab[i];
+        for (uint32_t i = 1; i < n; ++i) {
+            const long long d = sorted[i];
+            uint32_t j = i;
+            while (j > 0 && sorted[j - 1] > d) { sorted[j] = sorted[j - 1]; --j; }
+            sorted[j] = d;
+        }
+        for (uint32_t i = 0; i < 8; ++i) out[i] = i < n ? sorted[i] : 0ll;
+        *count = s_fail ? 0u : n;
+        *fail = s_fail;
+    }
+}
+
+template <typename T>
+__global__ void __launch_bounds__(kBlock)
+k_diag_build(const uint32_t *__restrict__ off, const uint32_t *__restrict__ col, const T *__restrict__ val, uint64_t n_rows, uint64_t n_tiles,
+             const uint32_t *__restrict__ win, const long long *__restrict__ offs, uint32_t K, uint8_t *__restrict__ mask8,
+             uint16_t *__restrict__ dstage, typename XdPat<T>::U *__restrict__ vbits, uint32_t *__restrict__ fail) {
+    typedef typename XdPat<T>::U U;
+    __shared__ U s_v[8];
+    __shared__ uint32_t s_q[8];
+    __shared__ long long s_d[8];
+    if (threadIdx.x < 8) { s_v[threadIdx.x] = XdPat<T>::kEmpty; s_q[threadIdx.x] = 0xFFu; s_d[threadIdx.x] = offs[threadIdx.x]; }
+    __syncthreads();
+    const U *bits = reinterpret_cast<const U *>(val);
+    for (uint64_t t = blockIdx.x; t < n_tiles; t += gridDim.x) {
+        const uint32_t *w = win + 8 * t;
+        const uint32_t a0 = w[0], e0 = w[1], a1 = w[2], e1 = w[3], a2 = w[4], e2 = w[5], a3 = w[6], e3 = w[7];
+        const uint32_t al0 = a0 & ~3u, al1 = a1 & ~3u, al2 = a2 & ~3u, al3 = a3 & ~3u;
+        const uint32_t n0 = e0 > a0 ? (e0 - al0 + 3u) >> 2 : 0u, n1 = e1 > a1 ? (e1 - al1 + 3u) >> 2 : 0u;
+        const uint32_t n2 = e2 > a2 ? (e2 - al2 + 3u) >> 2 : 0u;
+        const uint32_t p1 = n0, p2 = p1 + n1, p3 = p2 + n2;
+        const uint64_t r0 = t * (uint64_t)kStreamRows, r = r0 + threadIdx.x;
+        bool ok = true;
+        if (r < n_rows) {
+            uint32_t mask = 0;
+            const uint32_t k0 = off[r], k1 = off[r + 1];
+            for (uint32_t k = k0; k < k1 && ok; ++k) {
+                const uint32_t c = col[k];
+                const long long d = (long long)c - (long long)r;
+                uint32_t kk = 8;
+                for (uint32_t i = 0; i < K; ++i) kk = s_d[i] == d ? i : kk;
+                if (kk >= 8) { ok = false; break; }
+                mask |= 1u << kk;
+                const U pat = bits[k];
+                U seen = s_v[kk];
+                if (seen == XdPat<T>::kEmpty) {
+                    seen = atomicCAS(&s_v[kk], XdPat<T>::kEmpty, pat);
+                    if (seen == XdPat<T>::kEmpty) seen = pat;
+                }
+                ok = ok && seen == pat;
+                const uint32_t q = (uint32_t)(e1 > a1 && c >= a1) + (uint32_t)(e2 > a2 && c >= a2) + (uint32_t)(e3 > a3 && c >= a3);
+                uint32_t qs = s_q[kk];
+                if (qs == 0xFFu) {
+                    qs = atomicCAS(&s_q[kk], 0xFFu, q);
+                    if (qs == 0xFFu) qs = q;
+                }
+                ok = ok && qs == q;
+            }
+            mask8[r] = (uint8_t)mask;
+        }
+        if (!ok) atomicOr(fail, 1u);
+        __syncthreads();
+        if (threadIdx.x < 8) {
+            const uint32_t q = s_q[threadIdx.x];
+            uint32_t pos = kXddNone;
+            if (threadIdx.x < K && q != 0xFFu) {
+                const uint32_t al = q == 3u ? al3 : q == 2u ? al2 : q == 1u ? al1 : al0;
+                const uint32_t pq = q == 3u ? p3 : q == 2u ? p2 : q == 1u ? p1 : 0u;
+                const long long e = 4ll * (long long)pq + ((long long)r0 + s_d[threadIdx.x] - (long long)al);
+                if (e < -(long long)kStreamRows || e >= (long long)kXddNone) atomicOr(fail, 1u);
+                else pos = (uint32_t)(uint16_t)(int16_t)e;
+            }
+            dstage[8 * t + threadIdx.x] = (uint16_t)pos;
+            s_q[threadIdx.x] = 0xFFu;
+        }
+        __syncthreads();
+    }
+    if (threadIdx.x < K && s_v[threadIdx.x] != XdPat<T>::kEmpty) {
+        const U mine = s_v[threadIdx.x];
+        const U old = atomicCAS(vbits + threadIdx.x, XdPat<T>::kEmpty, mine);
+        if (old != XdPat<T>::kEmpty && old != mine) atomicOr(fail, 1u);
+    }
+}
+
+template <typename T, int XS> int xddp_resident(bool dot) {
+    static int res[2] = {0, 0};
+    if (res[0] == 0 || res[1] == 0) {
+        int a = 0, b = 0;
+        if (hipOccupancyMaxActiveBlocksPerMultiprocessor(&a, k_spmv_stream_xddp<T, false, XS>, kBlock, 0) == hipSuccess && a > 0) res[0] = a;
+        if (hipOccupancyMaxActiveBlocksPerMultiprocessor(&b, k_spmv_stream_xddp<T, true, XS>, kBlock, 0) == hipSuccess && b > 0) res[1] = b;
+        (void)hipGetLastError();
+    }
+    const int r = res[dot ? 1 : 0];
+    return r > 0 ? r : 4;
 }
 
 template <typename T, int XS, int VD> int xdp_resident(bool dot) {
@@ -595,6 +876,115 @@
     return SMH_OK;
 }
 
+template <typename T> constexpr bool kXddPersistAuto = false;
+template <typename T>
+int launch_xdd_t(const T *x, T *y, size_t n_rows, T *dot_partials, const uint32_t *cwin, const uint8_t *mask8, const uint32_t *dstage,
+                 const T *vtab, uint32_t K, const T *dot_lhs, hipStream_t s, int xs, uint64_t tile_begin, uint64_t tile_end) {
+    const uint64_t all_tiles = stream_tiles(n_rows, 1);
+    const uint64_t tile0 = tile_begin < all_tiles ? tile_begin : all_tiles, tile1 = tile_end < all_tiles ? tile_end : all_tiles;
+    if (tile1 <= tile0) return SMH_OK;
+    if (xs != 2 && xs != 4) return fail(SMH_ERR_INVALID, "K1s XD-D: the stage of x holds 2 or 4 chunks per thread");
+    const uint64_t n_tiles = tile1 - tile0;
+    const dim3 block(kBlock);
+    const char *pe = getenv("SMH_STREAM_PERSIST"), *we = getenv("SMH_STREAM_PERSIST_WGS");
+    const int persist_env = pe && *pe ? atoi(pe) : -1, per_cu_env = we ? atoi(we) : 0;
+    const bool want_persist = !(sizeof(T) == 8 && xs == 4) && (persist_env >= 0 ? persist_env != 0 : kXddPersistAuto<T>);
+    int cus = 0;
+    if (want_persist) {
+        static int cus_cache[64] = {};
+        int dev = 0;
+        (void)hipGetDevice(&dev);
+        int &c = cus_cache[dev & 63];
+        if (c == 0) {
+            hipDeviceProp_t prop;
+            c = hipGetDeviceProperties(&prop, dev) == hipSuccess && prop.multiProcessorCount > 0 ? prop.multiProcessorCount : 256;
+        }
+        cus = c;
+    }
+#define SMH_XDD(D, P)                                                                                                                \
+    do {                                                                                                                             \
+        if constexpr (!(sizeof(T) == 8 && P == 4)) {                                                                                 \
+            if (want_persist) {                                                                                                      \
+                const int resident = xddp_resident<T, P>(D);                      \
+                uint64_t wgx = (uint64_t)(cus / 8 > 0 ? cus / 8 : 1) * (uint64_t)(per_cu_env > 0 ? per_cu_env : resident);  \
+                if (persist_env >= 0 || n_tiles > 8 * wgx) {                                                                         \
+                    if (wgx > (n_tiles + 7) / 8) wgx = (n_tiles + 7) / 8;                                                            \
+                    if (wgx < 1) wgx = 1;                                                                                            \
+                    hipLaunchKernelGGL((k_spmv_stream_xddp<T, D, P>), dim3((unsigned)(8 * wgx)), block, 0, s, x, y, (uint64_t)n_rows, \
+                                       n_tiles, dot_partials, cwin, mask8, dstage, vtab, K, dot_lhs, tile0);                         \
+                    break;                                                                                                           \
+                }                                                                                                                    \
+            }                                                                                                                        \
+        }                                                                                                                            \
+        hipLaunchKernelGGL((k_spmv_stream_xdd<T, D, P>), dim3((unsigned)n_tiles), block, 0, s, x, y, (uint64_t)n_rows, n_tiles,      \
+                           dot_partials, cwin, mask8, dstage, vtab, K, dot_lhs, tile0);                                              \
+    } while (0)
+    if (xs == 2) { if (dot_partials) SMH_XDD(true, 2); else SMH_XDD(false, 2); }
+    else { if (dot_partials) SMH_XDD(true, 4); else SMH_XDD(false, 4); }
+#undef SMH_XDD
+    SMH_HIP(hipGetLastError());
+    return SMH_OK;
+}
+
+template <typename T>
+int diag_build_t(const uint32_t *off, const uint32_t *col, const T *val, size_t n_rows, const uint32_t *cwin, uint8_t *mask8, uint16_t *dstage,
+                 T *values, uint32_t *k_out, long long *offsets_out, hipStream_t s) {
+    typedef typename XdPat<T>::U U;
+    *k_out = 0;
+    const uint64_t n_tiles = (n_rows + kStreamRows - 1) / kStreamRows;
+    if (n_tiles == 0) return SMH_OK;
+    const unsigned blocks = grid_for(n_rows, 1024);
+    Scratch scr;
+    unsigned long long *tables = nullptr;
+    long long *d_offs = nullptr;
+    uint32_t *flags = nullptr;
+    SMH_TRY(scr.alloc(&tables, (size_t)blocks * 8));
+    SMH_TRY(scr.alloc(&d_offs, 8));
+    SMH_TRY(scr.alloc(&flags, 2));
+    struct { uint32_t fail, k; } h = {1u, 0u};
+    SMH_HIP(hipMemsetAsync(flags, 0, 2 * sizeof(uint32_t), s));
+    hipLaunchKernelGGL(k_diag_collect, dim3(blocks), dim3(kBlock), 0, s, off, col, (uint64_t)n_rows, tables, flags);
+    SMH_HIP(hipGetLastError());
+    hipLaunchKernelGGL(k_diag_merge, dim3(1), dim3(kBlock), 0, s, (const unsigned long long *)tables, (uint32_t)blocks, d_offs, flags + 1, flags);
+    SMH_HIP(hipGetLastError());
+    SMH_HIP(hipMemcpyAsync(&h, flags, sizeof h, hipMemcpyDeviceToHost, s));
+    SMH_HIP(hipMemcpyAsync(offsets_out, d_offs, 8 * sizeof(long long), hipMemcpyDeviceToHost, s));
+    SMH_HIP(hipStreamSynchronize(s));
+    if (h.fail || h.k == 0 || h.k > 8) return SMH_OK;
+    const uint32_t K = h.k;
+    U init[8];
+    for (uint32_t i = 0; i < 8; ++i) init[i] = i < K ? XdPat<T>::kEmpty : (U)0;
+    SMH_HIP(hipMemcpyAsync(values, init, sizeof init, hipMemcpyHostToDevice, s));
+    SMH_HIP(hipMemsetAsync(mask8, 0, n_tiles * kStreamRows, s));
+    hipLaunchKernelGGL(k_diag_build<T>, dim3((unsigned)(n_tiles < kBuildGrid ? n_tiles : kBuildGrid)), dim3(kBlock), 0, s, off, col, val,
+                       (uint64_t)n_rows, n_tiles, cwin, (const long long *)d_offs, K, mask8, dstage, reinterpret_cast<U *>(values), flags);
+    SMH_HIP(hipGetLastError());
+    SMH_HIP(hipMemcpyAsync(&h, flags, sizeof h, hipMemcpyDeviceToHost, s));
+    SMH_HIP(hipStreamSynchronize(s));
+    *k_out = h.fail ? 0u : K;
+    return SMH_OK;
+}
+
+}
+
+int launch_spmv_stream_xdd(int dtype, const void *x, void *y, size_t n_rows, void *dot_partials, const uint32_t *cwin, const uint8_t *mask8,
+                           const uint16_t *dstage, const void *values, uint32_t k, const void *dot_lhs, hipStream_t s, int xs,
+                           uint64_t tile_begin, uint64_t tile_end) {
+    if (n_rows == 0) return SMH_OK;
+    if (dot_partials && !dot_lhs) dot_lhs = x;
+    if (!dot_partials && !y) return fail(SMH_ERR_INVALID, "K1s: no output");
+    const uint32_t *ds = reinterpret_cast<const uint32_t *>(dstage);
+    if (dtype == SMH_F64)
+        return launch_xdd_t<double>((const double *)x, (double *)y, n_rows, (double *)dot_partials, cwin, mask8, ds, (const double *)values, k,
+                                    (const double *)dot_lhs, s, xs, tile_begin, tile_end);
+    return launch_xdd_t<float>((const float *)x, (float *)y, n_rows, (float *)dot_partials, cwin, mask8, ds, (const float *)values, k,
+                               (const float *)dot_lhs, s, xs, tile_begin, tile_end);
+}
+
+int stream_diag_build(int dtype, const uint32_t *off, const uint32_t *col, const void *val, size_t n_rows, const uint32_t *cwin,
+                      uint8_t *mask8, uint16_t *dstage, void *values, uint32_t *k_out, long long *offsets_out, hipStream_t s) {
+    return dtype == SMH_F64 ? diag_build_t<double>(off, col, (const double *)val, n_rows, cwin, mask8, dstage, (double *)values, k_out, offsets_out, s)
+                            : diag_build_t<float>(off, col, (const float *)val, n_rows, cwin, mask8, dstage, (float *)values, k_out, offsets_out, s);
 }
 
 int launch_spmv_stream_xd(int dtype, const void *val, const void *x, void *y, size_t n_rows, void *dot_partials, const uint16_t *scode,
diff --git a/sparsemat_amd/sparsemat_crs.py b/sparsemat_amd/sparsemat_crs.py
--- a/sparsemat_amd/sparsemat_crs.py
+++ b/sparsemat_amd/sparsemat_crs.py
@@ -499,6 +499,16 @@
     def set_stream_value_dict(self, mode):
         check(lib().smh_crs_set_stream_value_dict(self._h, int(mode)))
 
+    def stream_diag(self):
+        k = C.c_int()
+        offs = np.zeros(8, dtype=np.int64)
+        vals = np.zeros(8, dtype=self.dtype)
+        check(lib().smh_crs_stream_diag(self._h, C.byref(k), offs.ctypes.data, vals.ctypes.data))
+        return offs[:k.value].copy(), vals[:k.value].copy()
+
+    def set_stream_diag(self, mode):
+        check(lib().smh_crs_set_stream_diag(self._h, int(mode)))
+
     def stream_layout(self):
         a, b, c, d = C.c_int(), C.c_int(), C.c_int(), C.c_int()
         check(lib().smh_crs_stream_layout(self._h, C.byref(a), C.byref(b), C.byref(c), C.byref(d)))
```

Result: no change. 8271 (-0.0%).
